# nnnagle/vq-vae

Measured on AMD Instinct MI355X. Metric: tiles/sec, higher is better.
Workload: dtype bf16

## Files before the change

include/frl_hip.h:

```cpp
#ifndef FRL_HIP_H
#define FRL_HIP_H

#include <stddef.h>
#include <stdint.h>

#ifdef __cplusplus
extern "C" {
#endif

typedef void* frl_stream_t;

enum { FRL_F32 = 0, FRL_BF16 = 1, FRL_F16 = 2  };
enum { FRL_ACT_NONE = 0, FRL_ACT_RELU = 1, FRL_ACT_SIGMOID = 2 };

int frl_version(void);
const char* frl_last_error(void);
int frl_device_arch(char* buf, int n);
int frl_kernel_timing_enable(int on);
int frl_kernel_timing_report(char* buf, int n);

size_t frl_pack_cache_table_bytes(void);
int frl_pack_cache_create(void* arena, size_t bytes);
int frl_pack_cache_destroy(int handle);
int frl_pack_cache_activate(int handle);
// ... 49 lines not shown
int frl_scalar_fanout_dev(const float* g, const float* coef_host, const float* const* mult_host, int n, float* out, frl_stream_t stream);
int frl_scalar_fanout_guard(const float* g, const float* coef_host, const float* const* mult_host, const float* const* promise_host, int n,
                            float* out, int* flag, frl_stream_t stream);

int frl_encoder2_supported(int C0, int C1, int C2, int G1, int G2, int HW, int dtype);
size_t frl_encoder2_workspace_bytes(int B);
int frl_encoder2_fwd(const void* x, const float* w1, const float* g1, const float* b1, const float* w2, const float* g2, const float* b2,
                     void* z, float* stats, int B, int HW, float eps, void* ws, size_t ws_bytes, frl_stream_t stream);
int frl_encoder2_bwd(const void* x, const void* dz, const float* w1, const float* g1, const float* b1, const float* w2, const float* g2,
                     const float* b2, const float* stats, float* dw1, float* dg1, float* db1, float* dw2, float* dg2, float* db2,
                     int B, int HW, void* ws, size_t ws_bytes, frl_stream_t stream);

int frl_sobel_fwd(const void* x, void* g, int B, int H, int W, int C, int dtype, frl_stream_t stream);
int frl_sobel_bwd(const void* dg, void* dx, int B, int H, int W, int C, int dtype, frl_stream_t stream);
int frl_sobel_bwd_add(const void* dg, void* dx, const void* dx_add, int B, int H, int W, int C, int dtype, frl_stream_t stream);
int frl_edge_smooth_stencil_fwd(const void* x, const void* a_logit, const void* b_logit, void* smoothed, void* residual,
                                void* a_soft, void* b_soft, int B, int H, int W, int C, int R, int coarse_dilation,
                                int dtype, frl_stream_t stream);
int frl_edge_smooth_stencil_bwd(const void* d_smoothed, const void* x, const void* a_soft, const void* b_soft, void* dx,
                                void* da_logit, void* db_logit, const void* dx_add , int B, int H,
                                int W, int C, int R, int coarse_dilation, int dtype, frl_stream_t stream);
int frl_smooth_heads_supported(int C, int hidden, int rank, int dtype);
size_t frl_smooth_heads_workspace_bytes(int64_t npix);
int frl_smooth_heads_fwd(const void* x, const void* feat, const float* wa, const float* ba, const float* wb, const float* bb,
                         void* smoothed, void* residual, int B, int H, int W, int coarse_dilation, void* ws, size_t ws_bytes,
                         frl_stream_t stream);
size_t frl_smooth_heads_bwd_scratch_bytes(int64_t npix);
int frl_smooth_heads_force_gather(int on);
int frl_smooth_heads_bwd(const void* d_smoothed, const void* x, const void* feat, const float* wa, const float* ba, const float* wb,
                         const float* bb, const void* dx_add, void* dx, void* dfeat, float* dwa, float* dba, float* dwb, float* dbb,
                         void* scratch, size_t scratch_bytes, int B, int H, int W, int coarse_dilation, void* ws, size_t ws_bytes,
                         frl_stream_t stream);
int frl_smooth_heads_bwd_masked(const void* d_smoothed, const void* x, const void* feat, const float* wa, const float* ba, const float* wb,
                                const float* bb, const void* dx_add, void* dx, void* dfeat, float* dwa, float* dba, float* dwb, float* dbb,
                                void* scratch, size_t scratch_bytes, int B, int H, int W, int dil, int dfeat_relu, void* ws,
                                size_t ws_bytes, frl_stream_t stream);
int frl_film_fused_supported(int cond_dim, int hidden, int target_dim, int dtype);
size_t frl_film_fused_workspace_bytes(void);
int frl_film_fused_fwd(const void* z_type, const void* h, const float* w1g, const float* b1g, const float* w2g, const float* b2g,
                       const float* w1b, const float* b1b, const float* w2b, const float* b2b, void* z, void* gamma, void* beta, int B,
                       int T, int HW, void* ws, size_t ws_bytes, frl_stream_t stream);
int frl_film_fused_bwd(const void* z_type, const void* h, const void* dz, const float* w1g, const float* b1g, const float* w2g,
                       const float* b2g, const float* w1b, const float* b1b, const float* w2b, const float* b2b, void* dh, float* dw1g,
                       float* db1g, float* dw2g, float* db2g, float* dw1b, float* db1b, float* dw2b, float* db2b, int B, int T, int HW,
                       void* ws, size_t ws_bytes, frl_stream_t stream);
int frl_gate_blend_fwd(const void* smoothed, const void* residual, const void* gate_raw, float min_gate, void* out,
                       void* gate_out, int64_t n, int dtype, frl_stream_t stream);
int frl_gate_blend_bwd(const void* dout, const void* dgate_ext, const void* residual, const void* gate_raw, float min_gate,
                       void* d_residual, void* d_gate_raw, int64_t n, int dtype, frl_stream_t stream);
int frl_gate_blend_bwd_masked(const void* dout, const void* dgate_ext, const void* residual, const void* gate_raw, float min_gate,
                              void* d_residual, void* d_gate_raw, int64_t n, int dtype, int sigmoid_mask, frl_stream_t stream);

int frl_tcn_block_fwd(const void* x, const float* conv_w, const float* conv_b, const float* gn_w, const float* gn_b,
                      const float* gate_w, const float* gate_b, const float* proj_w, const float* proj_b, void* y,
                      int64_t npix, int HW, int T, int Cin, int Cout, int dilation, int G, float eps, int dtype, void* ws,
                      size_t ws_bytes, frl_stream_t stream);
size_t frl_tcn_block_bwd_workspace_bytes(int64_t npix, int Cout);
int frl_tcn_block_bwd(const void* x, const void* dy, const float* conv_w, const float* conv_b, const float* gn_w,
                      const float* gn_b, const float* gate_w, const float* gate_b, const float* proj_w,
                      const float* proj_b, void* dconv, void* dgpre, void* normed, void* dres, float* dgamma, float* dbeta,
                      int64_t npix, int HW, int T, int Cin, int Cout, int dilation, int G, float eps, int dtype, void* ws,
                      size_t ws_bytes, frl_stream_t stream);
int frl_tcn_block_bwd_data(const void* dconv, const void* dres, const float* conv_w, const float* proj_w, void* dx,
                           int64_t npix, int HW, int T, int Cin, int Cout, int dilation, int dtype, void* ws, size_t ws_bytes,
                           frl_stream_t stream);

int frl_tcn_block_bwd_fused_supported(int T, int Cin, int Cout, int G, int has_proj, int dtype);
size_t frl_tcn_block_bwd_fused_workspace_bytes(int64_t npix);
int frl_tcn_block_bwd_fused(const void* x, const void* dy, const float* conv_w, const float* conv_b, const float* gn_w,
                            const float* gn_b, const float* gate_w, const float* gate_b, void* dx, float* d_conv_w,
                            float* d_conv_b, float* d_gn_w, float* d_gn_b, float* d_gate_w, float* d_gate_b, int64_t npix,
                            int HW, int T, int dilation, int G, float eps, void* ws, size_t ws_bytes, frl_stream_t stream);

int frl_defer_begin(void);
int frl_defer_pending(void);
int frl_defer_destinations(void** out, int max);
int frl_defer_flush(frl_stream_t stream);
int frl_defer_abort(void);

int frl_tcn_hot_supported(int T, int Cin, int Cout, int G, int dilation, int has_proj, int dtype);
size_t frl_tcn_hot_fwd_workspace_bytes(void);
size_t frl_tcn_hot_bwd_workspace_bytes(int64_t npix);
int frl_tcn_hot_fwd(const void* x, const void* drop_mask, const float* conv_w, const float* conv_b, const float* gn_w, const float* gn_b,
                    const float* gate_w, const float* gate_b, void* y, int64_t npix, int HW, int dilation, float eps, void* ws,
                    size_t ws_bytes, frl_stream_t stream);
int frl_tcn_hot_bwd_nodx_supported(int64_t npix, int HW);
int frl_tcn_hot_bwd(const void* x, const void* drop_mask, const void* dy, const float* conv_w, const float* conv_b, const float* gn_w,
                    const float* gn_b, const float* gate_w, const float* gate_b, void* dx, float* d_conv_w, float* d_conv_b,
                    float* d_gn_w, float* d_gn_b, float* d_gate_w, float* d_gate_b, int64_t npix, int HW, int dilation,
                    float eps, void* ws, size_t ws_bytes, frl_stream_t stream);
size_t frl_tcn_chain_fwd_workspace_bytes(void);
int frl_tcn_chain_static_tiles(int on);
int frl_tcn_chain_fwd(const void* x, const float* const* conv_w, const float* const* conv_b, const float* const* gn_w,
                      const float* const* gn_b, const float* const* gate_w, const float* const* gate_b, const float* head_w,
                      const float* head_b, void* y1, void* y2, void* y3, void* h, int64_t npix, int HW, int Ch, float eps, void* ws,
                      size_t ws_bytes, frl_stream_t stream);
int frl_tcn_chain_fwd_xt(const void* x, const float* const* conv_w, const float* const* conv_b, const float* const* gn_w,
                         const float* const* gn_b, const float* const* gate_w, const float* const* gate_b, const float* head_w,
                         const float* head_b, void* y1, void* y2, void* y3, void* h, void* xt, int64_t npix, int HW, int Ch, float eps,
                         void* ws, size_t ws_bytes, frl_stream_t stream);
int frl_tcn_hot_bwd_head_supported(int64_t npix, int HW, int Ch);
size_t frl_tcn_hot_bwd_head_workspace_bytes(int64_t npix);
int frl_tcn_hot_bwd_head(const void* x, const void* dh, const float* head_w, int Ch, const float* conv_w, const float* conv_b,
                         const float* gn_w, const float* gn_b, const float* gate_w, const float* gate_b, void* dx, float* d_conv_w,
                         float* d_conv_b, float* d_gn_w, float* d_gn_b, float* d_gate_w, float* d_gate_b, int64_t npix, int HW,
                         int dilation, float eps, void* ws, size_t ws_bytes, frl_stream_t stream);
int frl_tcn_hot_force_generic_tiles(int on);
int frl_tcn_hot_bwd4_share(int variant, int share);

size_t frl_adamw_workspace_bytes(void);
int frl_adamw_clip_step(const void* desc_host, int ntensors, const void* chunks, const int* chunk_tensor, int nchunks, float max_norm,
                        float lr, double beta1, double beta2, float eps, int step, float* norm_out, const float* ok, int* counters,
                        const float* lr_dev, void* ws, size_t ws_bytes, frl_stream_t stream);
int frl_multi_tensor_scale_copy(const void* desc_host, int ntensors, const void* chunks, const int* chunk_tensor, int nchunks, float scale,
                                frl_stream_t stream);

int frl_film_modulate_fwd(const void* h, const void* gamma, const void* beta, void* out, int64_t B, int T, int64_t HW,
                          int C, int dtype, frl_stream_t stream);
int frl_film_modulate_bwd(const void* dout, const void* h, const void* gamma, void* dh, void* dgamma, void* dbeta,
                          int64_t B, int T, int64_t HW, int C, int dtype, frl_stream_t stream);
int frl_mean_time_fwd(const void* tile, void* out, int64_t B, int T, int64_t HWC, int dtype, frl_stream_t stream);
int frl_add(const void* a, const void* b, float scale_b, void* out, int64_t n, int dtype, frl_stream_t stream);

typedef struct FrlNormRec {
  float sub, div, mul, add, lo, hi;
  int flags;
  int pad;
} FrlNormRec;
int frl_normalize_tiles(const void* raw, int raw_dtype, const uint8_t* valid, const void* table, void* out, int out_dtype,
                        uint8_t* mask_out, int64_t rows, int F, frl_stream_t stream);
int frl_normalize_chunk_tiles(const void* chunk, int raw_dtype, int T, int CY, int CX, int F, const int32_t* desc, int ntiles,
                              int tile, const void* table, void* out, int out_dtype, uint8_t* mask_out, frl_stream_t stream);

int frl_host_parallel_copy(void* dst, const void* src, size_t nbytes, int nthreads);

size_t frl_mse_workspace_bytes(void);
int frl_mse_fwd(const void* pred, const void* target, const uint8_t* mask, int64_t P, int C, float* out, int dtype,
                void* ws, size_t ws_bytes, frl_stream_t stream);
int frl_mse_bwd(const void* pred, const void* target, const uint8_t* mask, const float* gscale, const float* stats,
                int64_t P, int C, void* dpred, int dtype, frl_stream_t stream);

int frl_decoder_mse_fused_supported(int Cz, int hidden, int F, int dtype);
size_t frl_decoder_mse_workspace_bytes(int64_t P, int Cz);
int frl_decoder_mse_fwd(const void* z, const float* w1, const float* b1, const float* w2, const float* b2, const void* target,
                        const uint8_t* mask, void* xhat, float* out, int64_t P, int Cz, void* ws, size_t ws_bytes,
                        frl_stream_t stream);
int frl_decoder_mse_bwd(const void* z, const float* w1, const float* b1, const float* w2, const float* b2, const void* target,
                        const uint8_t* mask, const float* gscale, const float* stats, void* dz, float* dw1, float* db1,
                        float* dw2, float* db2, int64_t P, int Cz, void* ws, size_t ws_bytes, frl_stream_t stream);
size_t frl_decoder_mse_onepass_bytes(int64_t P, int Cz);
int frl_decoder_mse_fwd_bwd(const void* z, const float* w1, const float* b1, const float* w2, const float* b2, const void* target,
                            const uint8_t* mask, const float* gscale, float* out, void* dz, void* buf, size_t buf_bytes, void* ctl,
                            int* nslab, int64_t P, int Cz, frl_stream_t stream);
int frl_decoder_mse_reduce(const void* buf, int nslab, float* dw1, float* db1, float* dw2, float* db2, int Cz, frl_stream_t stream);
int frl_decoder_mse_bwd_subgroups(int on);

size_t frl_vq_workspace_bytes(int64_t N, int K, int d);
int frl_vq_assign_fwd(const void* z, const float* E, int64_t N, int K, int d, int32_t* idx_out, void* zq_out,
                      float* stats_out, int32_t* counts_out, int dtype, void* ws, size_t ws_bytes, frl_stream_t stream);
size_t frl_vq_prepared_bytes(int K, int d);
int frl_vq_stream_tiles(int nt);
int frl_vq_prepare(const float* E, int64_t N, int K, int d, int dtype, void* prep, size_t prep_bytes, frl_stream_t stream);
int frl_vq_assign_fwd_prepared(const void* z, const float* E, void* prep , int64_t N, int K, int d,
                               int32_t* idx_out, void* zq_out, float* stats_out, int32_t* counts_out, int dtype, void* ws,
                               size_t ws_bytes, frl_stream_t stream);
int frl_vq_bwd(const void* g_out, const void* z, const void* zq , const float* E, const int32_t* idx, const int32_t* counts,
               const float* gscale, float beta, int64_t N, int K, int d, void* g_z_out, float* g_E_out, float* sums_out,
               int dtype, void* ws, size_t ws_bytes, frl_stream_t stream);
int frl_vq_ema_update(const float* sums, const int32_t* counts, int K, int d, float decay, float eps, float* ema_count,
                      float* ema_sum, float* E, const float* ok, frl_stream_t stream);
int frl_vq_revive_dead_codes(float* E, const int64_t* window_counts, int64_t min_count, const void* z, int64_t N, int K, int d,
                             uint64_t seed, float* m, float* v, int32_t* revived, int dtype, frl_stream_t stream);

int frl_gather_locations_fwd(const void* feat, int64_t sC, int64_t sH, int64_t sW, int C, int H, int W, const int64_t* coords, int64_t N,
                             void* out, int dtype, frl_stream_t stream);
int frl_segment_sum_rows(const float* vals, const int64_t* order, const int64_t* keys_sorted, int64_t M, int D, float* out, int64_t out_stride,
                         int accumulate, frl_stream_t stream);
int frl_infonce_fwd(const float* emb, int D, const int64_t* pairs, const float* weights, const unsigned char* is_pos, int64_t T,
                    const int64_t* seg, int64_t nseg, float temperature, int similarity, float* sims, float* logits, float* loss_a, float* coef,
                    float* loss, frl_stream_t stream);
int frl_infonce_pair_grads(const float* emb, int D, const int64_t* pairs, const float* sims, const float* coef, const float* gscale, int64_t T,
                           int64_t nseg, float temperature, int similarity, float* ga, float* gb, frl_stream_t stream);

size_t frl_vicreg_workspace_bytes(int64_t N, int D);
int frl_vicreg_fwd(const void* x, int64_t N, int D, int dtype, float variance_weight, float covariance_weight, float variance_target,
                   float eps, float* losses, float* cov, float* centre, void* ws, size_t ws_bytes, frl_stream_t stream);
int frl_vicreg_bwd(const void* x, const float* cov, const float* centre, const float* g3, int64_t N, int D, int dtype, float variance_weight,
                   float covariance_weight, float variance_target, float eps, void* dx, frl_stream_t stream);

int frl_soft_nbr_fwd(const float* d_ref, const float* d_learned, const unsigned char* mask, const float* weights, int64_t B, int M,
                     float inv_tau_ref, float inv_tau_learned, int min_valid, float* pairstat, float* coef, float* out2, double* stats,
                     frl_stream_t stream);
int frl_soft_nbr_bwd(const float* coef, const float* pairstat, const float* weights, const float* out2, const float* gup, int64_t B, int M,
                     float* grad, frl_stream_t stream);
int frl_soft_nbr_gathered_fwd(const float* ref, int C, const void* emb, int D, int emb_dtype, const int64_t* ref_rows_a, const int64_t* ref_rows_b,
                              const int64_t* emb_rows_a, const int64_t* emb_rows_b, const int64_t* lengths, const float* weights, int64_t B, int M,
                              int exclude_diagonal, float inv_tau_ref, float inv_tau_learned, int min_valid, float* pairstat, float* out2,
                              double* stats, frl_stream_t stream);
int frl_soft_nbr_gathered_bwd(const float* ref, int C, const void* emb, int D, int emb_dtype, const int64_t* ref_rows_a, const int64_t* ref_rows_b,
                              const int64_t* emb_rows_a, const int64_t* emb_rows_b, const int64_t* lengths, const float* weights, int64_t B, int M,
                              int exclude_diagonal, float inv_tau_ref, float inv_tau_learned, int min_valid, const float* pairstat,
                              const float* out2, const float* gup, float* grad_rows, frl_stream_t stream);

int frl_evt_soft_nbr_fwd(const void* emb, int emb_dtype, int64_t N, int D, const int32_t* idx, const float* S, const float* w, int K,
                         const int32_t* seg, const int32_t* seg_host, int nseg, float inv_tau_ref, float inv_tau_learned, int min_valid_anchors,
                         float* rowstat, float* segout, double* segstat, int32_t* index_flag, frl_stream_t stream);
int frl_evt_soft_nbr_bwd(const void* emb, int emb_dtype, int64_t N, int D, const int32_t* idx, const float* S, const float* w, int K,
                         const int32_t* seg, const int32_t* seg_host, int nseg, float inv_tau_ref, float inv_tau_learned, const float* rowstat,
                         const float* segout, const float* gup, const float* seg_weights, void* grad, frl_stream_t stream);

int frl_decode_codes(const int32_t* idx, const void* table, void* out, int64_t P, int K, int F, int dtype, int32_t* index_flag,
                     frl_stream_t stream);

size_t frl_mutual_knn_max_points(int D);
int frl_mutual_knn(const float* feat, int N, int D, const int32_t* patch_id, const float* coords, float pos_min_spatial, int k,
                   int32_t* knn_idx, uint8_t* mutual, frl_stream_t stream);

#ifdef __cplusplus
}
#endif
#endif
```

vq-vae_amd/csrc/dec_fused.hip:

```cpp
#include "frl_common.hpp"
#include "frl_host.hpp"
#include "frl_pack.hpp"
#include "frl_reduce.hpp"

typedef bf16 TT;
typedef bf16x8 frag8;
#define DF_H 128
#define DF_F 64
#define DF_GRID_MAX 1024

__device__ __forceinline__ bf16x8 tr_frag_p(const TT* tile, int pitch, int pix0, int ch0, int r16) {
  const TT* a0 = tile + (pix0 + (r16 >> 2)) * pitch + ch0 + 4 * (r16 & 3);
  bf16x4 lo = __builtin_amdgcn_ds_read_tr16_b64_v4bf16((bf16x4 __attribute__((address_space(3)))*)(a0));
  bf16x4 hi = __builtin_amdgcn_ds_read_tr16_b64_v4bf16((bf16x4 __attribute__((address_space(3)))*)(a0 + 4 * pitch));
  return bf16x8{lo[0], lo[1], lo[2], lo[3], hi[0], hi[1], hi[2], hi[3]};
}

template <int NF>
__device__ __forceinline__ void tile_put(TT* tile, int pitch, int prow, int kc, const LQTile<TT, NF>& t) {
  bf16x8* p = reinterpret_cast<bf16x8*>(tile + prow * pitch + NF * 8 * kc);
#pragma unroll
  for (int s = 0; s < NF; ++s) p[s] = t.f[s];
}

template <int NFZ>
__device__ __forceinline__ void dec_chain(float (&h)[32], float (&xh)[16], const LQTile<TT, NFZ>& zt, const frag8* __restrict__ w1,
                                          const frag8* __restrict__ w2, const float* __restrict__ b1q, const float* __restrict__ b2q,
                                          LQTile<TT, 4>& ht, int lane) {
  f32x4 hacc[8];
#pragma unroll
  for (int m = 0; m < 8; ++m) {
    hacc[m] = f32x4{0.f, 0.f, 0.f, 0.f};
#pragma unroll
    for (int s = 0; s < NFZ; ++s) hacc[m] = mfma16(w1[(m * NFZ + s) * 64 + lane], zt.f[s], hacc[m]);
  }
#pragma unroll
  for (int j = 0; j < 32; ++j) {
    const float v = hacc[j >> 2][j & 3] + b1q[j];
    h[j] = v > 0.f ? v : 0.f;
    ht.f[j >> 3][j & 7] = (bf16)h[j];
  }
  f32x4 xacc[4];
#pragma unroll
  for (int m = 0; m < 4; ++m) {
    xacc[m] = f32x4{0.f, 0.f, 0.f, 0.f};
#pragma unroll
    for (int s = 0; s < 4; ++s) xacc[m] = mfma16(w2[(m * 4 + s) * 64 + lane], ht.f[s], xacc[m]);
  }
#pragma unroll
  for (int j = 0; j < 16; ++j) xh[j] = xacc[j >> 2][j & 3] + b2q[j];
}

template <int NFZ>
__global__ __launch_bounds__(256, 4) void dec_mse_fwd_kernel(const TT* __restrict__ Z, const frag8* __restrict__ Wpk, const float* __restrict__ b1,
                                                          const float* __restrict__ b2, const TT* __restrict__ TGT,
                                                          const uint8_t* __restrict__ mask, TT* __restrict__ XHAT, int64_t P, int Cz,
                                                          double* __restrict__ partial) {
  extern __shared__ __attribute__((aligned(16))) char smem[];
  frag8* w1 = reinterpret_cast<frag8*>(smem);
  frag8* w2 = w1 + 8 * NFZ * 64;
  float* tb = reinterpret_cast<float*>(w2 + 16 * 64);
  const int tid = threadIdx.x, lane = tid & 63, wave = tid >> 6;
  const int px = lane & 15, kc = lane >> 4;
  copy_frags_lds<TT>(w1, Wpk, (8 * NFZ + 16) * 64, tid, 256);
  for (int i = tid; i < 192; i += 256) tb[i] = i < 128 ? b1[i] : b2[i - 128];
  __syncthreads();
  const float* b1q = tb + 32 * kc;
  const float* b2q = tb + 128 + 16 * kc;
  const bool fastz = (Cz == 32 * NFZ);
  float sq = 0.f, cnt = 0.f;
  const int64_t ntile = (P + 15) >> 4;
  const int64_t tstep = (int64_t)gridDim.x * 4;
  LQTile<TT, NFZ> zt, zn;
  LQTile<TT, 2> tt, tn;
  {
    const int64_t t0 = (int64_t)blockIdx.x * 4 + wave;
    const int64_t r0 = (t0 < ntile ? t0 : 0) * 16 + px;
    const int64_t rc = r0 < P ? r0 : P - 1;
    lq_load<TT, NFZ>(zt, Z, rc, Cz, kc, fastz);
    lq_load<TT, 2>(tt, TGT, rc, DF_F, kc, true);
  }
  for (int64_t tile = (int64_t)blockIdx.x * 4 + wave; tile < ntile; tile += tstep) {
    int64_t row = tile * 16 + px;
    bool valid = row < P;
    if (!valid) row = P - 1;
    if (valid && mask != nullptr) valid = mask[row] != 0;
    {
      const int64_t tnx = tile + tstep < ntile ? tile + tstep : tile;
      const int64_t rn = tnx * 16 + px;
      const int64_t rc = rn < P ? rn : P - 1;
      lq_load<TT, NFZ>(zn, Z, rc, Cz, kc, fastz);
      lq_load<TT, 2>(tn, TGT, rc, DF_F, kc, true);
    }
    float h[32], xh[16];
    LQTile<TT, 4> ht;
    int lw = lane;
    asm volatile("" : "+v"(lw));
    dec_chain<NFZ>(h, xh, zt, w1, w2, b1q, b2q, ht, lw);
    if (valid) {
#pragma unroll
      for (int j = 0; j < 16; ++j) { const float d = xh[j] - (float)tt.f[j >> 3][j & 7]; sq = fmaf(d, d, sq); }
      cnt += 16.f;
    }
    if (XHAT != nullptr && tile * 16 + px < P) {
      bf16x8* xo = reinterpret_cast<bf16x8*>(XHAT + row * DF_F + 16 * kc);
      bf16x8 o0, o1;
#pragma unroll
      for (int j = 0; j < 8; ++j) { o0[j] = (bf16)xh[j]; o1[j] = (bf16)xh[8 + j]; }
      xo[0] = o0;
      xo[1] = o1;
    }
    zt = zn;
    tt = tn;
  }
  double sd = wave_sum_d((double)sq), cd = wave_sum_d((double)cnt);
  __shared__ double red[8];
  if (lane == 0) { red[wave] = sd; red[4 + wave] = cd; }
  __syncthreads();
  if (tid == 0) {
    partial[blockIdx.x * 2 + 0] = red[0] + red[1] + red[2] + red[3];
    partial[blockIdx.x * 2 + 1] = red[4] + red[5] + red[6] + red[7];
  }
}

__global__ __launch_bounds__(256) void dec_mse_finalize_kernel(const double* __restrict__ partial, int n, float* __restrict__ out) {
  __shared__ double rs[256], rc[256];
  double s = 0.0, c = 0.0;
  for (int i = threadIdx.x; i < n; i += 256) { s += partial[2 * i]; c += partial[2 * i + 1]; }
  rs[threadIdx.x] = s; rc[threadIdx.x] = c;
  __syncthreads();
  for (int o = 128; o > 0; o >>= 1) {
    if (threadIdx.x < o) { rs[threadIdx.x] += rs[threadIdx.x + o]; rc[threadIdx.x] += rc[threadIdx.x + o]; }
    __syncthreads();
  }
  if (threadIdx.x == 0) { out[0] = rc[0] > 0.0 ? (float)(rs[0] / rc[0]) : 0.f; out[1] = (float)rc[0]; }
}

__device__ __forceinline__ void df_sg_sync(unsigned* bar, unsigned& gen, int lane) {
  asm volatile("s_waitcnt lgkmcnt(0)" ::: "memory");
  gen += 4u;
  if (lane == 0) __hip_atomic_fetch_add(bar, 1u, __ATOMIC_RELAXED, __HIP_MEMORY_SCOPE_WORKGROUP);
  for (;;) {
    const unsigned seen = (unsigned)__builtin_amdgcn_readfirstlane((int)__hip_atomic_load(bar, __ATOMIC_RELAXED, __HIP_MEMORY_SCOPE_WORKGROUP));
    if ((int)(seen - gen) >= 0) break;
    __builtin_amdgcn_s_sleep(1);
  }
  asm volatile("" ::: "memory");
}
#define DF_SG_SHARE0 19

template <bool LOSS> struct DecLoss {};
template <> struct DecLoss<true> {
  double* partial;
  const float* out;
  float* out_w;
  float nv_host;
};

template <int NFZ, int NW, bool SG = false, bool LOSS = false>
__global__ __launch_bounds__(SG ? 512 : 64 * NW) void dec_mse_bwd_kernel(const TT* __restrict__ Z, const frag8* __restrict__ Wpk, const float* __restrict__ b1,
                                                               const float* __restrict__ b2, const TT* __restrict__ TGT,
                                                               const uint8_t* __restrict__ mask, const float* __restrict__ gscale,
                                                               const float* __restrict__ stats, TT* __restrict__ DZ, int64_t P, int Cz,
                                                               float* __restrict__ slab, const DecLoss<LOSS> la) {
  constexpr int CZP = 32 * NFZ, CB = CZP / 16, R = 16 * NW, NTH = SG ? 512 : 64 * NW;
  constexpr int PX = DF_F + 8, PH = DF_H + 8, PZ = CZP + 8;
  static_assert(!SG || NW == 4, "subgroups are four waves");
  extern __shared__ __attribute__((aligned(16))) char smem[];
  frag8* w1 = reinterpret_cast<frag8*>(smem);
  frag8* w2 = w1 + 8 * NFZ * 64;
  frag8* w2t = w2 + 16 * 64;
  frag8* w1t = w2t + 16 * 64;
  float* tb = reinterpret_cast<float*>(w1t + CB * 4 * 64);
  const int tid = threadIdx.x, lane = tid & 63;
  const int sg = SG ? (tid >> 8) : 0;
  const int wave = SG ? ((tid >> 6) & 3) : (tid >> 6);
  constexpr int TILE_ELEMS = R * (PX + 2 * PH + PZ);
  unsigned* bars = reinterpret_cast<unsigned*>(tb + 192);
  TT* t_dx = reinterpret_cast<TT*>(tb + 192 + (SG ? 32 : 0)) + sg * TILE_ELEMS;
  TT* t_h = t_dx + R * PX;
  TT* t_dh = t_h + R * PH;
  TT* t_z = t_dh + R * PH;
  const int px = lane & 15, kc = lane >> 4, r16 = px;
  const int prow = wave * 16 + px;
  copy_frags_lds<TT>(w1, Wpk, (8 * NFZ + 16 + 16 + CB * 4) * 64, tid, NTH);
  for (int i = tid; i < 192; i += NTH) tb[i] = i < 128 ? b1[i] : b2[i - 128];
  if (SG && tid < 2) bars[16 * tid] = 0u;
  unsigned* bar = bars + 16 * sg;
  unsigned bgen = 0;
  (void)bar; (void)bgen;
  __syncthreads();
  const float* b1q = tb + 32 * kc;
  const float* b2q = tb + 128 + 16 * kc;
  const bool fastz = (Cz == CZP);
  float nv;
  if constexpr (LOSS) nv = la.nv_host >= 0.f ? la.nv_host : la.out[1]; else nv = stats[1];
  float sq = 0.f;
  int nrow = 0;
  (void)sq; (void)nrow;
  const float ksc = nv > 0.f ? (gscale ? gscale[0] : 1.f) * 2.f / nv : 0.f;

  constexpr int W2CB = (NW == 8) ? 4 : 8;
  const int w2row = (NW == 8) ? (wave & 3) : wave;
  const int w2col0 = (NW == 8) ? 4 * (wave >> 2) : 0;
  constexpr int W1RB = (NW == 8) ? 1 : 2;
  f32x4 a2[W2CB], a1[W1RB][CB], ab2, ab1[W1RB];
#pragma unroll
  for (int i = 0; i < W2CB; ++i) a2[i] = f32x4{0.f, 0.f, 0.f, 0.f};
#pragma unroll
  for (int r = 0; r < W1RB; ++r) {
    ab1[r] = f32x4{0.f, 0.f, 0.f, 0.f};
#pragma unroll
    for (int i = 0; i < CB; ++i) a1[r][i] = f32x4{0.f, 0.f, 0.f, 0.f};
  }
  ab2 = f32x4{0.f, 0.f, 0.f, 0.f};
  const bf16 one = (bf16)1.f, zero = (bf16)0.f;
  const bf16x8 ones = (r16 == 0) ? bf16x8{one, one, one, one, one, one, one, one} : bf16x8{zero, zero, zero, zero, zero, zero, zero, zero};

  const int64_t nwt = (P + R - 1) / R;
  int64_t w_first = blockIdx.x, w_end = nwt;
  const int64_t w_step = gridDim.x;
  if (SG) {
    const int64_t n_wg = (int64_t)blockIdx.x < nwt ? (nwt - 1 - blockIdx.x) / w_step + 1 : 0;
    const int64_t n0 = (n_wg * DF_SG_SHARE0 + 16) >> 5;
    w_first = blockIdx.x + (sg ? n0 : 0) * w_step;
    w_end = blockIdx.x + (sg ? n_wg : n0) * w_step;
    if (w_end > nwt) w_end = nwt;
  }
  LQTile<TT, NFZ> zt, z1, z2, zn;
  LQTile<TT, 2> tt, t1, t2, tn;
  auto fetch = [&](LQTile<TT, NFZ>& zz, LQTile<TT, 2>& tg, int64_t w) {
    const int64_t wc = w < nwt ? w : (nwt - 1);
    const int64_t r0 = wc * R + prow;
    const int64_t rc = r0 < P ? r0 : P - 1;
    lq_load<TT, NFZ>(zz, Z, rc, Cz, kc, fastz);
    lq_load<TT, 2>(tg, TGT, rc, DF_F, kc, true);
  };
  fetch(zt, tt, w_first);
  fetch(z1, t1, w_first + w_step);
  fetch(z2, t2, w_first + 2 * w_step);
  for (int64_t wt = w_first; wt < w_end; wt += w_step) {
    int64_t row = wt * R + prow;
    const bool inb = row < P;
    bool valid = inb;
    if (!inb) row = P - 1;
    if (valid && mask != nullptr) valid = mask[row] != 0;
    fetch(zn, tn, wt + 3 * w_step);
    float h[32], xh[16];
    LQTile<TT, 4> ht;
    dec_chain<NFZ>(h, xh, zt, w1, w2, b1q, b2q, ht, lane);
    LQTile<TT, 2> dxt;
    const float kv = valid ? ksc : 0.f;
    if constexpr (LOSS) {
      if (valid) {
#pragma unroll
        for (int j = 0; j < 16; ++j) { const float d = xh[j] - (float)tt.f[j >> 3][j & 7]; sq = fmaf(d, d, sq); }
      }
      nrow += __popcll(__ballot(valid));
    }
#pragma unroll
    for (int j = 0; j < 16; ++j) dxt.f[j >> 3][j & 7] = (bf16)(kv * (xh[j] - (float)tt.f[j >> 3][j & 7]));
    f32x4 dhacc[8];
#pragma unroll
    for (int m = 0; m < 8; ++m) {
      dhacc[m] = f32x4{0.f, 0.f, 0.f, 0.f};
#pragma unroll
      for (int s = 0; s < 2; ++s) dhacc[m] = mfma16(w2t[(m * 2 + s) * 64 + lane], dxt.f[s], dhacc[m]);
    }
    LQTile<TT, 4> dht;
#pragma unroll
    for (int j = 0; j < 32; ++j) dht.f[j >> 3][j & 7] = (bf16)(h[j] > 0.f ? dhacc[j >> 2][j & 3] : 0.f);
    f32x4 dzacc[CB];
#pragma unroll
    for (int m = 0; m < CB; ++m) {
      dzacc[m] = f32x4{0.f, 0.f, 0.f, 0.f};
#pragma unroll
      for (int s = 0; s < 4; ++s) dzacc[m] = mfma16(w1t[(m * 4 + s) * 64 + lane], dht.f[s], dzacc[m]);
    }
    if (inb) {
      constexpr int QZ = 4 * CB;
      TT* dzp = DZ + row * (int64_t)Cz + QZ * kc;
      if (fastz) {
#pragma unroll
        for (int j = 0; j < QZ; j += 8) {
          bf16x8 o;
#pragma unroll
          for (int e = 0; e < 8; ++e) o[e] = (bf16)dzacc[(j + e) >> 2][(j + e) & 3];
          *reinterpret_cast<bf16x8*>(dzp + j) = o;
        }
      } else if ((Cz & 3) == 0) {
#pragma unroll
        for (int j = 0; j < QZ; j += 4)
          if (QZ * kc + j < Cz)
            *reinterpret_cast<bf16x4*>(dzp + j) = bf16x4{(bf16)dzacc[j >> 2][0], (bf16)dzacc[j >> 2][1], (bf16)dzacc[j >> 2][2], (bf16)dzacc[j >> 2][3]};
      } else {
#pragma unroll
        for (int j = 0; j < QZ; ++j)
          if (QZ * kc + j < Cz) dzp[j] = (bf16)dzacc[j >> 2][j & 3];
      }
    }
    if (!inb) {
#pragma unroll
      for (int s = 0; s < 4; ++s) dht.f[s] = bf16x8{zero, zero, zero, zero, zero, zero, zero, zero};
    }
    tile_put<2>(t_dx, PX, prow, kc, dxt);
    tile_put<4>(t_h, PH, prow, kc, ht);
    tile_put<4>(t_dh, PH, prow, kc, dht);
    tile_put<NFZ>(t_z, PZ, prow, kc, zt);
    if constexpr (SG) df_sg_sync(bar, bgen, lane); else __syncthreads();
#pragma unroll
    for (int ks = 0; ks < R / 32; ++ks) {
      const int pix0 = ks * 32 + 8 * kc;
      const bf16x8 af = tr_frag_p(t_dx, PX, pix0, w2row * 16, r16);
#pragma unroll
      for (int i = 0; i < W2CB; ++i) a2[i] = mfma16(af, tr_frag_p(t_h, PH, pix0, (w2col0 + i) * 16, r16), a2[i]);
      if (NW == 4 || (wave >> 2) == 0) ab2 = mfma16(af, ones, ab2);
#pragma unroll
      for (int r = 0; r < W1RB; ++r) {
        const int rb = (NW == 8) ? wave : 2 * wave + r;
        const bf16x8 ah = tr_frag_p(t_dh, PH, pix0, rb * 16, r16);
#pragma unroll
        for (int i = 0; i < CB; ++i) a1[r][i] = mfma16(ah, tr_frag_p(t_z, PZ, pix0, i * 16, r16), a1[r][i]);
        ab1[r] = mfma16(ah, ones, ab1[r]);
      }
    }
    if constexpr (SG) df_sg_sync(bar, bgen, lane); else __syncthreads();
    zt = z1; z1 = z2; z2 = zn;
    tt = t1; t1 = t2; t2 = tn;
  }
  float* my = slab + (int64_t)(SG ? 2 * blockIdx.x + sg : blockIdx.x) * (DF_F * DF_H + DF_H * CZP + DF_F + DF_H);
#pragma unroll
  for (int i = 0; i < W2CB; ++i)
#pragma unroll
    for (int r = 0; r < 4; ++r) my[(w2row * 16 + kc * 4 + r) * DF_H + (w2col0 + i) * 16 + r16] = a2[i][r];
#pragma unroll
  for (int rr = 0; rr < W1RB; ++rr) {
    const int rb = (NW == 8) ? wave : 2 * wave + rr;
#pragma unroll
    for (int i = 0; i < CB; ++i)
#pragma unroll
      for (int r = 0; r < 4; ++r) my[DF_F * DF_H + (rb * 16 + kc * 4 + r) * CZP + i * 16 + r16] = a1[rr][i][r];
    if (r16 == 0) {
#pragma unroll
      for (int r = 0; r < 4; ++r) my[DF_F * DF_H + DF_H * CZP + DF_F + rb * 16 + kc * 4 + r] = ab1[rr][r];
    }
  }
  if (r16 == 0 && (NW == 4 || (wave >> 2) == 0)) {
#pragma unroll
    for (int r = 0; r < 4; ++r) my[DF_F * DF_H + DF_H * CZP + w2row * 16 + kc * 4 + r] = ab2[r];
  }
  if constexpr (LOSS) {
    constexpr int NWV = NTH / 64;
    __shared__ double lred[2 * NWV];
    const double sd = wave_sum_d((double)sq), cd = 16.0 * (double)nrow;
    if (lane == 0) { lred[tid >> 6] = sd; lred[NWV + (tid >> 6)] = cd; }
    __syncthreads();
    if (tid == 0) {
      double s = lred[0], c = lred[NWV];
#pragma unroll
      for (int w = 1; w < NWV; ++w) { s += lred[w]; c += lred[NWV + w]; }
      la.partial[2 * blockIdx.x + 0] = s;
      la.partial[2 * blockIdx.x + 1] = c;
    }
  }
}

__global__ __launch_bounds__(256) void dec_mask_count_kernel(const uint8_t* __restrict__ mask, int64_t P, unsigned* __restrict__ ctl,
                                                             float* __restrict__ out) {
  __shared__ unsigned wg_n;
  const int tid = threadIdx.x;
  if (tid == 0) wg_n = 0u;
  __syncthreads();
  const int64_t gtid = (int64_t)blockIdx.x * 256 + tid, gstep = (int64_t)gridDim.x * 256;
  const int64_t n16 = ((reinterpret_cast<uintptr_t>(mask) & 15) == 0) ? (P >> 4) : 0;
  unsigned n = 0;
  const uint4* m16 = reinterpret_cast<const uint4*>(mask);
  for (int64_t i = gtid; i < n16; i += gstep) {
    const uint4 v = m16[i];
    const unsigned w[4] = {v.x, v.y, v.z, v.w};
#pragma unroll
    for (int k = 0; k < 4; ++k)
      n += __popc((w[k] | ((w[k] & 0x7f7f7f7fu) + 0x7f7f7f7fu)) & 0x80808080u);
  }
  for (int64_t i = n16 * 16 + gtid; i < P; i += gstep) n += mask[i] != 0 ? 1u : 0u;
  if (n) atomicAdd(&wg_n, n);
  __syncthreads();
  if (tid == 0) {
    unsigned long long* total = reinterpret_cast<unsigned long long*>(ctl + 2);
    if (wg_n) __hip_atomic_fetch_add(total, (unsigned long long)wg_n, __ATOMIC_RELAXED, __HIP_MEMORY_SCOPE_AGENT);
    __builtin_amdgcn_fence(__ATOMIC_RELEASE, "agent");
    asm volatile("s_waitcnt vmcnt(0)" ::: "memory");
    const unsigned ticket = __hip_atomic_fetch_add(ctl, 1u, __ATOMIC_RELAXED, __HIP_MEMORY_SCOPE_AGENT);
    if (ticket == gridDim.x - 1) {
      __builtin_amdgcn_fence(__ATOMIC_ACQUIRE, "agent");
      asm volatile("s_waitcnt vmcnt(0)" ::: "memory");
      const unsigned long long t = __hip_atomic_load(total, __ATOMIC_RELAXED, __HIP_MEMORY_SCOPE_AGENT);
      out[1] = (float)((double)t * (double)DF_F);
      __hip_atomic_store(total, 0ull, __ATOMIC_RELAXED, __HIP_MEMORY_SCOPE_AGENT);
      __hip_atomic_store(ctl, 0u, __ATOMIC_RELAXED, __HIP_MEMORY_SCOPE_AGENT);
    }
  }
}

template <int NFZ>
__global__ void dec_pack_kernel(frag8* __restrict__ dst, const float* __restrict__ W1, const float* __restrict__ W2, int Cz, int bwd) {
  constexpr int CZP = 32 * NFZ, CB = CZP / 16;
  const int tid = blockIdx.x * blockDim.x + threadIdx.x, nt = gridDim.x * blockDim.x;
  pack_weights_lds<TT, NFZ>(dst, W1, DF_H, Cz, 8, Cz, 1, tid, nt);
  frag8* p = dst + 8 * NFZ * 64;
  pack_weights_lds<TT, 4>(p, W2, DF_F, DF_H, 4, DF_H, 1, tid, nt);
  if (!bwd) return;
  p += 16 * 64;
  pack_weights_lds<TT, 2>(p, W2, DF_H, DF_F, 8, 1, DF_H, tid, nt);
  p += 16 * 64;
  pack_weights_lds<TT, 4>(p, W1, Cz, DF_H, CB, 1, Cz, tid, nt);
}

template <int NFZ>
static const frag8* dec_packed(const float* w1, const float* w2, int Cz, int bwd, frag8* ws_pk, hipStream_t st) {
  constexpr int CZP = 32 * NFZ, CB = CZP / 16;
  FrlPackJob jobs[4];
  size_t off = 0;
  jobs[0] = frl_pack_job_pw(w1, off, FRL_BF16, NFZ, DF_H, Cz, 8, Cz, 1);
  off += (size_t)8 * NFZ * 64 * sizeof(frag8);
  jobs[1] = frl_pack_job_pw(w2, off, FRL_BF16, 4, DF_F, DF_H, 4, DF_H, 1);
  off += (size_t)16 * 64 * sizeof(frag8);
  int n = 2;
  if (bwd) {
    jobs[2] = frl_pack_job_pw(w2, off, FRL_BF16, 2, DF_H, DF_F, 8, 1, DF_H);
    off += (size_t)16 * 64 * sizeof(frag8);
    jobs[3] = frl_pack_job_pw(w1, off, FRL_BF16, 4, Cz, DF_H, CB, 1, Cz);
    off += (size_t)CB * 4 * 64 * sizeof(frag8);
    n = 4;
  }
  bool hit = false;
  frag8* pk = ws_pk;
  if (void* img = frl_pack_cached(jobs, n, off, &hit)) pk = (frag8*)img;
  if (!hit) FRL_LAUNCH((dec_pack_kernel<NFZ>), dim3(32), dim3(256), 0, st, pk, w1, w2, Cz, bwd);
  return pk;
}


static unsigned df_fwd_grid(int64_t P) { int64_t g = ((P + 15) / 16 + 3) / 4; if (g > DF_GRID_MAX) g = DF_GRID_MAX; return (unsigned)(g < 1 ? 1 : g); }
static unsigned df_bwd_grid(int64_t P, int R) { int64_t g = (P + R - 1) / R; if (g > 256) g = 256; return (unsigned)(g < 1 ? 1 : g); }

template <int NFZ, int NW, bool LOSS = false>
static int launch_dec_bwd(const void* z, const float* w1, const float* b1, const float* w2, const float* b2, const void* tgt,
                          const uint8_t* mask, const float* gscale, const float* stats, void* dz, float* dw1, float* db1, float* dw2,
                          float* db2, int64_t P, int Cz, char* ws, hipStream_t st, DecLoss<LOSS> la = DecLoss<LOSS>{}, int* nslab_out = nullptr) {
  constexpr int CZP = 32 * NFZ, CB = CZP / 16, R = 16 * NW;
  const unsigned grid = df_bwd_grid(P, R);
  const size_t slab_n = (size_t)DF_F * DF_H + DF_H * CZP + DF_F + DF_H;
  const frag8* pk = dec_packed<NFZ>(w1, w2, Cz, 1, reinterpret_cast<frag8*>(ws + ((grid * slab_n * sizeof(float) + 255) / 256) * 256), st);
  const size_t lds = (size_t)(8 * NFZ + 16 + 16 + CB * 4) * 64 * sizeof(frag8) + 192 * sizeof(float) +
                     (size_t)R * ((DF_F + 8) + 2 * (DF_H + 8) + (CZP + 8)) * sizeof(TT);
  auto kern = dec_mse_bwd_kernel<NFZ, NW, false, LOSS>;
  FRL_HIP(hipFuncSetAttribute((const void*)kern, hipFuncAttributeMaxDynamicSharedMemorySize, (int)lds));
  FRL_LAUNCH_AS(LOSS ? "dec_mse_bwd_loss_kernel" : "dec_mse_bwd_kernel", kern, dim3(grid), dim3(64 * NW), lds, st, (const TT*)z, (const frag8*)pk, b1, b2, (const TT*)tgt, mask, gscale, stats, (TT*)dz, P, Cz,
             (float*)ws, la);
  if constexpr (LOSS) {
    FRL_LAUNCH(dec_mse_finalize_kernel, dim3(1), dim3(256), 0, st, (const double*)la.partial, (int)grid, la.out_w);
    *nslab_out = (int)grid;
    return frl_check_launch("decoder_mse_fwd_bwd");
  }
  launch_slab_reduce_deferrable<float, DecEpi>((const float*)ws, (int)grid, (int64_t)slab_n, DecEpi{dw2, dw1, db2, db1, Cz, CZP, DF_F, DF_H}, st);
  return frl_check_launch("decoder_mse_bwd");
}

template <int NFZ, bool LOSS = false>
static int launch_dec_bwd_sg(const void* z, const float* w1, const float* b1, const float* w2, const float* b2, const void* tgt,
                             const uint8_t* mask, const float* gscale, const float* stats, void* dz, float* dw1, float* db1, float* dw2,
                             float* db2, int64_t P, int Cz, char* ws, hipStream_t st, DecLoss<LOSS> la = DecLoss<LOSS>{}, int* nslab_out = nullptr) {
  constexpr int CZP = 32 * NFZ, CB = CZP / 16, R = 64;
  int64_t g = (P + 2 * R - 1) / (2 * R);
  if (g > 256) g = 256;
  if (g < 1) g = 1;
  const unsigned grid = (unsigned)g, nslab = 2 * grid;
  const size_t slab_n = (size_t)DF_F * DF_H + DF_H * CZP + DF_F + DF_H;
  const frag8* pk = dec_packed<NFZ>(w1, w2, Cz, 1, reinterpret_cast<frag8*>(ws + ((nslab * slab_n * sizeof(float) + 255) / 256) * 256), st);
  const size_t lds = (size_t)(8 * NFZ + 16 + 16 + CB * 4) * 64 * sizeof(frag8) + (192 + 32) * sizeof(float) +
                     (size_t)2 * R * ((DF_F + 8) + 2 * (DF_H + 8) + (CZP + 8)) * sizeof(TT);
  auto kern = dec_mse_bwd_kernel<NFZ, 4, true, LOSS>;
  FRL_HIP(hipFuncSetAttribute((const void*)kern, hipFuncAttributeMaxDynamicSharedMemorySize, (int)lds));
  FRL_LAUNCH_AS(LOSS ? "dec_mse_bwd_sg_loss_kernel" : "dec_mse_bwd_sg_kernel", kern, dim3(grid), dim3(512), lds, st, (const TT*)z, (const frag8*)pk, b1, b2, (const TT*)tgt, mask, gscale, stats, (TT*)dz, P,
                Cz, (float*)ws, la);
  if constexpr (LOSS) {
    FRL_LAUNCH(dec_mse_finalize_kernel, dim3(1), dim3(256), 0, st, (const double*)la.partial, (int)grid, la.out_w);
    *nslab_out = (int)nslab;
    return frl_check_launch("decoder_mse_fwd_bwd");
  }
  launch_slab_reduce_deferrable<float, DecEpi>((const float*)ws, (int)nslab, (int64_t)slab_n, DecEpi{dw2, dw1, db2, db1, Cz, CZP, DF_F, DF_H}, st);
  return frl_check_launch("decoder_mse_bwd");
}

static int g_dec_subgroups = 1;

extern "C" {

int frl_decoder_mse_bwd_subgroups(int on) { const int was = g_dec_subgroups; g_dec_subgroups = on ? 1 : 0; return was; }

int frl_decoder_mse_fused_supported(int Cz, int hidden, int F, int dtype) {
  return (dtype == FRL_BF16 && hidden == DF_H && F == DF_F && Cz >= 1 && Cz <= 64) ? 1 : 0;
}

size_t frl_decoder_mse_workspace_bytes(int64_t P, int Cz) {
  const size_t czp = Cz <= 32 ? 32 : 64;
  const size_t slab_n = (size_t)DF_F * DF_H + DF_H * czp + DF_F + DF_H;
  const size_t bwd = 512 * slab_n * sizeof(float) + 256 + (size_t)(8 * 2 + 32 + 16) * 64 * 16;
  const size_t fwd = (size_t)DF_GRID_MAX * 2 * sizeof(double) + 256 + (size_t)(8 * 2 + 16) * 64 * 16;
  (void)P;
  return bwd > fwd ? bwd : fwd;
}

int frl_decoder_mse_fwd(const void* z, const float* w1, const float* b1, const float* w2, const float* b2, const void* target,
                        const uint8_t* mask, void* xhat, float* out, int64_t P, int Cz, void* ws, size_t ws_bytes, hipStream_t stream) {
  if (P <= 0) return frl_fail(-2, "decoder_mse_fwd: empty input");
  if (Cz < 1 || Cz > 64) return frl_fail(-2, "decoder_mse_fwd: latent width must be 1..64");
  if (ws_bytes < frl_decoder_mse_workspace_bytes(P, Cz)) return frl_fail(-4, "decoder_mse_fwd: workspace too small");
  char* w = (char*)ws;
  double* partial = (double*)w;
  frag8* ws_pk = reinterpret_cast<frag8*>(w + (size_t)DF_GRID_MAX * 2 * sizeof(double) + 256);
  const unsigned grid = df_fwd_grid(P);
  if (Cz <= 32) {
    const frag8* pk = dec_packed<1>(w1, w2, Cz, 0, ws_pk, stream);
    const size_t lds = (size_t)(8 + 16) * 64 * sizeof(frag8) + 192 * sizeof(float);
    FRL_LAUNCH((dec_mse_fwd_kernel<1>), dim3(grid), dim3(256), lds, stream, (const TT*)z, (const frag8*)pk, b1, b2, (const TT*)target, mask,
               (TT*)xhat, P, Cz, partial);
  } else {
    const frag8* pk = dec_packed<2>(w1, w2, Cz, 0, ws_pk, stream);
    const size_t lds = (size_t)(16 + 16) * 64 * sizeof(frag8) + 192 * sizeof(float);
    FRL_LAUNCH((dec_mse_fwd_kernel<2>), dim3(grid), dim3(256), lds, stream, (const TT*)z, (const frag8*)pk, b1, b2, (const TT*)target, mask,
               (TT*)xhat, P, Cz, partial);
  }
  FRL_LAUNCH(dec_mse_finalize_kernel, dim3(1), dim3(256), 0, stream, (const double*)partial, (int)grid, out);
  return frl_check_launch("decoder_mse_fwd");
}

int frl_decoder_mse_bwd(const void* z, const float* w1, const float* b1, const float* w2, const float* b2, const void* target,
                        const uint8_t* mask, const float* gscale, const float* stats, void* dz, float* dw1, float* db1, float* dw2,
                        float* db2, int64_t P, int Cz, void* ws, size_t ws_bytes, hipStream_t stream) {
  if (P <= 0) return frl_fail(-2, "decoder_mse_bwd: empty input");
  if (Cz < 1 || Cz > 64) return frl_fail(-2, "decoder_mse_bwd: latent width must be 1..64");
  if (ws_bytes < frl_decoder_mse_workspace_bytes(P, Cz)) return frl_fail(-4, "decoder_mse_bwd: workspace too small");
  if (g_dec_subgroups && P >= 128 && Cz <= 32)
    return launch_dec_bwd_sg<1>(z, w1, b1, w2, b2, target, mask, gscale, stats, dz, dw1, db1, dw2, db2, P, Cz, (char*)ws, stream);
  if (Cz <= 32) return launch_dec_bwd<1, 8>(z, w1, b1, w2, b2, target, mask, gscale, stats, dz, dw1, db1, dw2, db2, P, Cz, (char*)ws, stream);
  return launch_dec_bwd<2, 4>(z, w1, b1, w2, b2, target, mask, gscale, stats, dz, dw1, db1, dw2, db2, P, Cz, (char*)ws, stream);
}

static size_t df_onepass_partial_off(int64_t P, int Cz) { return ((frl_decoder_mse_workspace_bytes(P, Cz) + 255) / 256) * 256; }
size_t frl_decoder_mse_onepass_bytes(int64_t P, int Cz) { return df_onepass_partial_off(P, Cz) + (size_t)256 * 2 * sizeof(double); }

int frl_decoder_mse_fwd_bwd(const void* z, const float* w1, const float* b1, const float* w2, const float* b2, const void* target,
                            const uint8_t* mask, const float* gscale, float* out, void* dz, void* buf, size_t buf_bytes, void* ctl,
                            int* nslab, int64_t P, int Cz, hipStream_t stream) {
  if (P <= 0) return frl_fail(-2, "decoder_mse_fwd_bwd: empty input");
  if (Cz < 1 || Cz > 64) return frl_fail(-2, "decoder_mse_fwd_bwd: latent width must be 1..64");
  if (buf_bytes < frl_decoder_mse_onepass_bytes(P, Cz)) return frl_fail(-4, "decoder_mse_fwd_bwd: buffer too small");
  if (out == nullptr || dz == nullptr || ctl == nullptr || nslab == nullptr) return frl_fail(-2, "decoder_mse_fwd_bwd: null output");
  unsigned* c = (unsigned*)ctl;
  DecLoss<true> la;
  la.partial = reinterpret_cast<double*>((char*)buf + df_onepass_partial_off(P, Cz));
  la.out = out;
  la.out_w = out;
  la.nv_host = (float)((double)P * (double)DF_F);
  if (mask != nullptr) {
    int64_t g = (P + 256 * 64 - 1) / (256 * 64);
    if (g > 128) g = 128;
    FRL_LAUNCH(dec_mask_count_kernel, dim3((unsigned)g), dim3(256), 0, stream, mask, P, c, out);
    la.nv_host = -1.f;
  }
  if (g_dec_subgroups && P >= 128 && Cz <= 32)
    return launch_dec_bwd_sg<1, true>(z, w1, b1, w2, b2, target, mask, gscale, nullptr, dz, nullptr, nullptr, nullptr, nullptr, P, Cz, (char*)buf, stream, la, nslab);
  if (Cz <= 32)
    return launch_dec_bwd<1, 8, true>(z, w1, b1, w2, b2, target, mask, gscale, nullptr, dz, nullptr, nullptr, nullptr, nullptr, P, Cz, (char*)buf, stream, la, nslab);
  return launch_dec_bwd<2, 4, true>(z, w1, b1, w2, b2, target, mask, gscale, nullptr, dz, nullptr, nullptr, nullptr, nullptr, P, Cz, (char*)buf, stream, la, nslab);
}

int frl_decoder_mse_reduce(const void* buf, int nslab, float* dw1, float* db1, float* dw2, float* db2, int Cz, hipStream_t stream) {
  if (Cz < 1 || Cz > 64 || nslab < 1 || nslab > 512) return frl_fail(-2, "decoder_mse_reduce: bad latent width or slab count");
  const int czp = Cz <= 32 ? 32 : 64;
  const size_t slab_n = (size_t)DF_F * DF_H + DF_H * czp + DF_F + DF_H;
  launch_slab_reduce_deferrable<float, DecEpi>((const float*)buf, nslab, (int64_t)slab_n, DecEpi{dw2, dw1, db2, db1, Cz, czp, DF_F, DF_H}, stream);
  return frl_check_launch("decoder_mse_reduce");
}

}
```

vq-vae_amd/csrc/frl_common.hpp:

```cpp
#pragma once
#include <hip/hip_runtime.h>
#include <stdint.h>

typedef __bf16 bf16;
typedef __attribute__((ext_vector_type(8))) __bf16 bf16x8;
typedef __attribute__((ext_vector_type(4))) __bf16 bf16x4;
typedef __attribute__((ext_vector_type(2))) __bf16 bf16x2;
typedef __attribute__((ext_vector_type(4))) float f32x4;
typedef __attribute__((ext_vector_type(2))) float f32x2;

enum { FRL_F32 = 0, FRL_BF16 = 1 };
enum { FRL_ACT_NONE = 0, FRL_ACT_RELU = 1, FRL_ACT_SIGMOID = 2 };

#define FRL_WAVE 64

template <typename T> struct DT;
template <> struct DT<float> {
  typedef float frag_t;
  static constexpr int FE = 1;
  static constexpr int CPAD = 16;
  static constexpr int VEC = 4;
  static constexpr int ID = FRL_F32;
};
template <> struct DT<bf16> {
  typedef bf16x8 frag_t;
  static constexpr int FE = 8;
  static constexpr int CPAD = 32;
  static constexpr int VEC = 8;
  static constexpr int ID = FRL_BF16;
};

__device__ __forceinline__ f32x4 mfma16(const float a, const float b, f32x4 c) {
  return __builtin_amdgcn_mfma_f32_16x16x4f32(a, b, c, 0, 0, 0);
}
__device__ __forceinline__ f32x4 mfma16(const bf16x8 a, const bf16x8 b, f32x4 c) {
  return __builtin_amdgcn_mfma_f32_16x16x32_bf16(a, b, c, 0, 0, 0);
}

__device__ __forceinline__ float to_f32(float v) { return v; }
__device__ __forceinline__ float to_f32(bf16 v) { return (float)v; }
template <typename T> __device__ __forceinline__ T from_f32(float v);
template <> __device__ __forceinline__ float from_f32<float>(float v) { return v; }
template <> __device__ __forceinline__ bf16 from_f32<bf16>(float v) { return (bf16)v; }

__device__ __forceinline__ float act_fwd(float v, int act) {
  if (act == FRL_ACT_RELU) return v > 0.f ? v : 0.f;
  if (act == FRL_ACT_SIGMOID) return 1.f / (1.f + expf(-v));
  return v;
}
__device__ __forceinline__ float sigmoid_fast(float v) {
  return __builtin_amdgcn_rcpf(1.f + __builtin_amdgcn_exp2f(-1.44269504088896f * v));
}
template <typename T> __device__ __forceinline__ float sigmoid_t(float v) {
  if constexpr (sizeof(T) == 2) return sigmoid_fast(v); else return 1.f / (1.f + expf(-v));
}

__device__ __forceinline__ float act_bwd_from_y(float y, int act) {
  if (act == FRL_ACT_RELU) return y > 0.f ? 1.f : 0.f;
  if (act == FRL_ACT_SIGMOID) return y * (1.f - y);
  return 1.f;
}

template <typename T> struct Vec;
template <> struct Vec<float> {
  static constexpr int N = 4;
  __device__ static __forceinline__ void load(const float* p, float* o) {
    f32x4 v = *reinterpret_cast<const f32x4*>(p);
    o[0] = v[0]; o[1] = v[1]; o[2] = v[2]; o[3] = v[3];
  }
  __device__ static __forceinline__ void store(float* p, const float* o) {
    f32x4 v = {o[0], o[1], o[2], o[3]};
    *reinterpret_cast<f32x4*>(p) = v;
  }
};
template <> struct Vec<bf16> {
  static constexpr int N = 8;
  __device__ static __forceinline__ void load(const bf16* p, float* o) {
    bf16x8 v = *reinterpret_cast<const bf16x8*>(p);
#pragma unroll
    for (int i = 0; i < 8; ++i) o[i] = (float)v[i];
  }
  __device__ static __forceinline__ void store(bf16* p, const float* o) {
    bf16x8 v;
#pragma unroll
    for (int i = 0; i < 8; ++i) v[i] = (bf16)o[i];
    *reinterpret_cast<bf16x8*>(p) = v;
  }
};

__device__ __forceinline__ float wave_sum(float v) {
#pragma unroll
  for (int o = 32; o > 0; o >>= 1) v += __shfl_xor(v, o, 64);
  return v;
}
__device__ __forceinline__ double wave_sum_d(double v) {
#pragma unroll
  for (int o = 32; o > 0; o >>= 1) v += __shfl_xor(v, o, 64);
  return v;
}

__device__ __forceinline__ unsigned xcd_remap(unsigned bid, unsigned nwg) {
  const unsigned q = nwg >> 3, r = nwg & 7u, xcd = bid & 7u;
  const unsigned base = xcd < r ? xcd * (q + 1) : r * (q + 1) + (xcd - r) * q;
  return base + (bid >> 3);
}

template <typename T, int NF> struct LQTile { typename DT<T>::frag_t f[NF]; };

template <typename T> __device__ __forceinline__ int lq_channel(int q, int kc, int s, int e) {
  return q * kc + s * DT<T>::FE + e;
}

template <typename T, int NF>
__device__ __forceinline__ void lq_load(LQTile<T, NF>& t, const T* __restrict__ X, int64_t row, int C,
                                        int kc, bool fast) {
  constexpr int FE = DT<T>::FE;
  const int q = NF * FE;
  const T* p = X + row * (int64_t)C + q * kc;
  if (fast) {
    if constexpr (FE == 8) {
#pragma unroll
      for (int s = 0; s < NF; ++s) t.f[s] = *reinterpret_cast<const bf16x8*>(p + 8 * s);
    } else {
      static_assert(NF % 4 == 0, "f32 quarter must be a multiple of 4");
#pragma unroll
      for (int s = 0; s < NF; s += 4) {
        f32x4 v = *reinterpret_cast<const f32x4*>(p + s);
        t.f[s] = v[0]; t.f[s + 1] = v[1]; t.f[s + 2] = v[2]; t.f[s + 3] = v[3];
      }
    }
  } else {
    if constexpr (FE == 8) {
      if ((C & 3) == 0) {
#pragma unroll
        for (int s = 0; s < NF; ++s) {
          bf16x4 lo = bf16x4{(bf16)0.f, (bf16)0.f, (bf16)0.f, (bf16)0.f}, hi = lo;
          const int c = q * kc + 8 * s;
          if (c < C) lo = *reinterpret_cast<const bf16x4*>(p + 8 * s);
          if (c + 4 < C) hi = *reinterpret_cast<const bf16x4*>(p + 8 * s + 4);
          t.f[s] = bf16x8{lo[0], lo[1], lo[2], lo[3], hi[0], hi[1], hi[2], hi[3]};
        }
        return;
      }
    }
#pragma unroll
    for (int s = 0; s < NF; ++s) {
      if constexpr (FE == 8) {
        bf16x8 v;
#pragma unroll
        for (int e = 0; e < 8; ++e) {
          const int c = q * kc + 8 * s + e;
          v[e] = c < C ? p[8 * s + e] : (bf16)0.f;
        }
        t.f[s] = v;
      } else {
        const int c = q * kc + s;
        t.f[s] = c < C ? p[s] : 0.f;
      }
    }
  }
}

template <typename T, int NF>
__device__ __forceinline__ float lq_get(const LQTile<T, NF>& t, int s, int e) {
  if constexpr (DT<T>::FE == 8) return (float)t.f[s][e]; else return t.f[s];
}
template <typename T, int NF>
__device__ __forceinline__ void lq_set(LQTile<T, NF>& t, int s, int e, float v) {
  if constexpr (DT<T>::FE == 8) t.f[s][e] = (bf16)v; else t.f[s] = v;
}

template <typename T, int NF>
__device__ __forceinline__ void pack_weights_lds(typename DT<T>::frag_t* __restrict__ wl,
                                                 const float* __restrict__ W, int Cout, int Cin, int MB,
                                                 int64_t so, int64_t si, int tid, int nthreads) {
  constexpr int FE = DT<T>::FE;
  const int q = NF * FE, qo = 4 * MB;
  const int total = MB * NF * 64;
  for (int i = tid; i < total; i += nthreads) {
    const int lane = i & 63, fs = i >> 6;
    const int s = fs % NF, mb = fs / NF;
    const int r = lane & 15, kc = lane >> 4;
    const int oc = qo * (r >> 2) + 4 * mb + (r & 3);
    if constexpr (FE == 8) {
      bf16x8 v;
#pragma unroll
      for (int e = 0; e < 8; ++e) {
        const int ic = q * kc + 8 * s + e;
        v[e] = (oc < Cout && ic < Cin) ? (bf16)W[oc * so + ic * si] : (bf16)0.f;
      }
      wl[i] = v;
    } else {
      const int ic = q * kc + s;
      wl[i] = (oc < Cout && ic < Cin) ? W[oc * so + ic * si] : 0.f;
    }
  }
// ... 20 lines not shown
```

vq-vae_amd/csrc/vq.hip:

```cpp
#include "frl_common.hpp"
#include "frl_host.hpp"
#include "frl_reduce.hpp"
#include <math.h>
#include <stdlib.h>

#define VQ_IDX_BITS 7
#define VQ_IDX_MASK 127u
#define VQ_MAX_CHUNK 512

struct VqHeader {
  unsigned enmax_bits;
  int namb;
  double sq_fix;
  int done;
  int pad;
};

template <typename T, int NF>
__global__ void vq_prepare_kernel(const float* __restrict__ E, int K, int d, float* __restrict__ en, int kpad,
                                  typename DT<T>::frag_t* __restrict__ pk, int total, int npack_blocks, int* __restrict__ ctl) {
  constexpr int FE = DT<T>::FE;
  constexpr int q = NF * FE;
  if ((int)blockIdx.x >= npack_blocks) {
    const int k = ((int)blockIdx.x - npack_blocks) * blockDim.x + threadIdx.x;
// ... 1276 lines not shown
#pragma unroll
      for (int s = 0; s < NF; ++s) acc = mfma16(pk[(size_t)(mb * NF + s) * 64 + lane], zr.f[s], acc);
#pragma unroll
      for (int r = 0; r < 4; ++r) {
        const int code = mb * 16 + 4 * kc + r;
        const bool hit = valid && acc[r] <= lm && code < K;
        if (__builtin_amdgcn_ballot_w64(hit && p1 >= 0) != 0ull) flush();
        if (hit) { if (p0 < 0) p0 = code; else p1 = code; }
      }
    }
    flush();
#pragma unroll
    for (int off = 16; off <= 32; off <<= 1) {
      const double ob = __shfl_xor(bestd, off, 64);
      const int okk = __shfl_xor(bk, off, 64);
      if (ob < bestd || (ob == bestd && okk < bk)) { bestd = ob; bk = okk; }
    }
    if (kc == 0) { mrg_d[wave][vx] = bestd; mrg_k[wave][vx] = bk; }
    __syncthreads();
    if (wave == 0) {
      bestd = mrg_d[0][vx]; bk = mrg_k[0][vx];
#pragma unroll
      for (int w = 1; w < VQ_FIXT_WAVES; ++w) {
        const double ob = mrg_d[w][vx];
        const int okk = mrg_k[w][vx];
        if (ob < bestd || (ob == bestd && okk < bk)) { bestd = ob; bk = okk; }
      }
      if ((unsigned)bk >= (unsigned)K) bk = 0;
      if (valid) {
        const float* er = E + (int64_t)bk * d + q * kc;
        T* zo = zq_out + row * (int64_t)d + q * kc;
#pragma unroll
        for (int s = 0; s < NF * FE; ++s) {
          if (q * kc + s < d) {
            const float ev = to_f32(from_f32<T>(er[s]));
            zo[s] = from_f32<T>(ev);
            const float df = lq_get<T, NF>(zr, s / FE, s % FE) - ev;
            sq_acc = fmaf(df, df, sq_acc);
          }
        }
        if (kc == 0) { idx_out[row] = bk; atomicAdd(&counts_fix[bk], 1); }
      }
    }
    __syncthreads();
  }
  if (wave == 0) {
    const float ws_ = wave_sum(sq_acc);
    if (lane == 0 && ws_ != 0.f) atomicAdd(&hdr->sq_fix, (double)ws_);
  }
}

__global__ __launch_bounds__(256) void vq_finalize_kernel(const float* __restrict__ partial, int npartial, const VqHeader* __restrict__ hdr,
                                                          const int32_t* __restrict__ counts_acc, int32_t* __restrict__ counts, int K, int64_t N,
                                                          int d, float* __restrict__ stats) {
  __shared__ double red[256];
  double s = 0.0;
  for (int i = threadIdx.x; i < npartial; i += 256) s += (double)partial[i];
  red[threadIdx.x] = s;
  __syncthreads();
  for (int o = 128; o > 0; o >>= 1) { if (threadIdx.x < o) red[threadIdx.x] += red[threadIdx.x + o]; __syncthreads(); }
  const double sq = red[0] + hdr->sq_fix;
  __syncthreads();
  double h = 0.0;
  for (int k = threadIdx.x; k < K; k += 256) {
    const int cnt = counts_acc[k];
    counts[k] = cnt;
    const double p = (double)cnt / (double)N;
    h += p * log(p + 1e-10);
  }
  red[threadIdx.x] = h;
  __syncthreads();
  for (int o = 128; o > 0; o >>= 1) { if (threadIdx.x < o) red[threadIdx.x] += red[threadIdx.x + o]; __syncthreads(); }
  if (threadIdx.x == 0) {
    stats[0] = (float)sq;
    stats[1] = (float)exp(-red[0]);
    stats[2] = (float)hdr->namb;
    stats[3] = (float)(sq / ((double)N * (double)d));
  }
}

template <typename T>
__global__ __launch_bounds__(256) void vq_bwd_kernel(const T* __restrict__ gout, const T* __restrict__ Z,
                                                     const float* __restrict__ E, const int32_t* __restrict__ idx,
                                                     const float* __restrict__ gscale, float cz_base, int64_t N, int K, int d,
                                                     int Kc, int64_t rows_per_wg, T* __restrict__ gz,
                                                     float* __restrict__ slab ) {
  extern __shared__ __attribute__((aligned(16))) char smem[];
  float* acc = reinterpret_cast<float*>(smem);
  const int tid = threadIdx.x;
  const int64_t r0 = (int64_t)blockIdx.x * rows_per_wg;
  int64_t r1 = r0 + rows_per_wg;
  if (r1 > N) r1 = N;
  const float cz = cz_base * (gscale ? gscale[0] : 1.f);
  constexpr int VEC = DT<T>::VEC;
  const bool fast = (d % VEC) == 0;
  const int vpr = (d + VEC - 1) / VEC;
  const int nchunks = (K + Kc - 1) / Kc;
  for (int c = 0; c < nchunks; ++c) {
    const int kbase = c * Kc;
    __syncthreads();
    for (int i = tid; i < Kc * d; i += 256) acc[i] = 0.f;
    __syncthreads();
    const int64_t nvec = (r1 > r0 ? (r1 - r0) : 0) * vpr;
    for (int64_t i = tid; i < nvec; i += 256) {
      const int64_t n = r0 + i / vpr;
      const int c0 = (int)(i % vpr) * VEC;
      const int k = idx[n];
      const bool mine = (k >= kbase && k < kbase + Kc);
      if (c == 0 || mine) {
        float zv[VEC];
        if (fast) Vec<T>::load(Z + n * (int64_t)d + c0, zv);
        else {
#pragma unroll
          for (int e = 0; e < VEC; ++e) zv[e] = (c0 + e < d) ? to_f32(Z[n * (int64_t)d + c0 + e]) : 0.f;
        }
        if (mine) {
#pragma unroll
          for (int e = 0; e < VEC; ++e)
            if (c0 + e < d) atomicAdd(&acc[(k - kbase) * d + c0 + e], zv[e]);
        }
        if (c == 0 && gz != nullptr) {
          float gv[VEC], ov[VEC];
          if (gout != nullptr) {
            if (fast) Vec<T>::load(gout + n * (int64_t)d + c0, gv);
            else {
#pragma unroll
              for (int e = 0; e < VEC; ++e) gv[e] = (c0 + e < d) ? to_f32(gout[n * (int64_t)d + c0 + e]) : 0.f;
            }
          } else {
#pragma unroll
            for (int e = 0; e < VEC; ++e) gv[e] = 0.f;
          }
#pragma unroll
          for (int e = 0; e < VEC; ++e) {
            const float ev = (c0 + e < d) ? to_f32(from_f32<T>(E[(int64_t)k * d + c0 + e])) : 0.f;
            ov[e] = gv[e] + cz * (zv[e] - ev);
          }
          if (fast) Vec<T>::store(gz + n * (int64_t)d + c0, ov);
          else {
#pragma unroll
            for (int e = 0; e < VEC; ++e)
              if (c0 + e < d) gz[n * (int64_t)d + c0 + e] = from_f32<T>(ov[e]);
          }
        }
      }
    }
    __syncthreads();
    const int kn = (K - kbase) < Kc ? (K - kbase) : Kc;
    float* dst = slab + ((int64_t)blockIdx.x * K + kbase) * d;
    for (int i = tid; i < kn * d; i += 256) dst[i] = acc[i];
  }
}

template <int RB, int CB, int NWV>
__global__ __launch_bounds__(64 * NWV) void vq_bwd_mfma_kernel(const bf16* __restrict__ gout, const bf16* __restrict__ Z, const bf16* __restrict__ ZQ,
                                                          const float* __restrict__ E,
                                                          const int32_t* __restrict__ idx, const float* __restrict__ gscale, float cz_base,
                                                          int64_t N, int K, int d, int64_t rows_per_wg, bf16* __restrict__ gz,
                                                          float* __restrict__ slab ) {
  constexpr int DP = CB * 16, PITCH = DP + 8, KC = RB * NWV * 16, NTH = 64 * NWV;
  extern __shared__ __attribute__((aligned(16))) char smem[];
  bf16* zt = reinterpret_cast<bf16*>(smem);
  int* it = reinterpret_cast<int*>(zt + 64 * PITCH);
  const int tid = threadIdx.x, lane = tid & 63, wave = tid >> 6;
  const int r16 = lane & 15, kc = lane >> 4;
  const int64_t r0 = (int64_t)blockIdx.x * rows_per_wg;
  int64_t r1 = r0 + rows_per_wg;
  if (r1 > N) r1 = N;
  const float cz = cz_base * (gscale ? gscale[0] : 1.f);
  const bool fast = (d % 8) == 0;
  const int vpr = DP / 8;
  const bf16 one = (bf16)1.f, zero = (bf16)0.f;
  for (int kbase = 0; kbase < K; kbase += KC) {
    f32x4 acc[RB][CB];
#pragma unroll
    for (int a = 0; a < RB; ++a)
#pragma unroll
      for (int b = 0; b < CB; ++b) acc[a][b] = f32x4{0.f, 0.f, 0.f, 0.f};
    constexpr int NV = (64 * (DP / 8) + NTH - 1) / NTH;
    const bool pre = fast && (ZQ != nullptr || gz == nullptr || kbase != 0);
    const bool want_gz = (kbase == 0 && gz != nullptr);
    bf16x8 rz[NV], rg[NV], rq[NV];
    auto fetch = [&](int64_t p0) {
#pragma unroll
      for (int u = 0; u < NV; ++u) {
        const int i = tid + u * NTH;
        const int row = i / vpr, c0 = (i % vpr) * 8;
        const int64_t n = p0 + row;
        const bool ok = i < 64 * vpr && n < r1 && c0 < d;
        const int64_t off = ok ? n * (int64_t)d + c0 : 0;
        bf16x8 v = *reinterpret_cast<const bf16x8*>(Z + off);
        if (!ok) v = bf16x8{};
        rz[u] = v;
        if (want_gz) {
          rg[u] = gout != nullptr ? *reinterpret_cast<const bf16x8*>(gout + off) : bf16x8{};
          rq[u] = *reinterpret_cast<const bf16x8*>(ZQ + off);
        }
      }
    };
    if (pre && r0 < r1) fetch(r0);
    for (int64_t p0 = r0; p0 < r1; p0 += 64) {
      __syncthreads();
      if (pre) {
#pragma unroll
        for (int u = 0; u < NV; ++u) {
          const int i = tid + u * NTH;
          if (i >= 64 * vpr) continue;
          const int row = i / vpr, c0 = (i % vpr) * 8;
          const int64_t n = p0 + row;
          if (want_gz && n < r1 && c0 < d) {
            float ov[8];
#pragma unroll
            for (int e = 0; e < 8; ++e) ov[e] = (float)rg[u][e] + cz * ((float)rz[u][e] - (float)rq[u][e]);
            Vec<bf16>::store(gz + n * (int64_t)d + c0, ov);
          }
          *reinterpret_cast<bf16x8*>(zt + row * PITCH + c0) = rz[u];
        }
      } else {
      for (int i = tid; i < 64 * vpr; i += NTH) {
        const int row = i / vpr, c0 = (i % vpr) * 8;
        const int64_t n = p0 + row;
        float zv[8];
#pragma unroll
        for (int e = 0; e < 8; ++e) zv[e] = 0.f;
        if (n < r1 && c0 < d) {
          if (fast) Vec<bf16>::load(Z + n * (int64_t)d + c0, zv);
          else {
#pragma unroll
            for (int e = 0; e < 8; ++e) if (c0 + e < d) zv[e] = (float)Z[n * (int64_t)d + c0 + e];
          }
          if (kbase == 0 && gz != nullptr) {
            const int k = idx[n];
            float gv[8], ov[8];
#pragma unroll
            for (int e = 0; e < 8; ++e) gv[e] = 0.f;
            if (gout != nullptr) {
              if (fast) Vec<bf16>::load(gout + n * (int64_t)d + c0, gv);
              else {
#pragma unroll
                for (int e = 0; e < 8; ++e) if (c0 + e < d) gv[e] = (float)gout[n * (int64_t)d + c0 + e];
              }
            }
            float qv[8];
            if (ZQ != nullptr && fast) Vec<bf16>::load(ZQ + n * (int64_t)d + c0, qv);
            else {
#pragma unroll
              for (int e = 0; e < 8; ++e) qv[e] = (c0 + e < d) ? (float)(bf16)E[(int64_t)k * d + c0 + e] : 0.f;
            }
#pragma unroll
            for (int e = 0; e < 8; ++e) ov[e] = gv[e] + cz * (zv[e] - qv[e]);
            if (fast) Vec<bf16>::store(gz + n * (int64_t)d + c0, ov);
            else {
#pragma unroll
              for (int e = 0; e < 8; ++e) if (c0 + e < d) gz[n * (int64_t)d + c0 + e] = (bf16)ov[e];
            }
          }
        }
        Vec<bf16>::store(zt + row * PITCH + c0, zv);
      }
      }
      if (tid < 64) it[tid] = (p0 + tid < r1) ? idx[p0 + tid] - kbase : -1;
      __syncthreads();
      if (pre && p0 + 64 < r1) fetch(p0 + 64);
#pragma unroll
      for (int ks = 0; ks < 2; ++ks) {
        const int pix0 = ks * 32 + 8 * kc;
        int id8[8];
#pragma unroll
        for (int j = 0; j < 8; ++j) id8[j] = it[pix0 + j];
        bf16x8 bfr[CB];
#pragma unroll
        for (int b = 0; b < CB; ++b) {
          const bf16* a0 = zt + (pix0 + (r16 >> 2)) * PITCH + b * 16 + 4 * (r16 & 3);
          bf16x4 lo = __builtin_amdgcn_ds_read_tr16_b64_v4bf16((bf16x4 __attribute__((address_space(3)))*)(a0));
          bf16x4 hi = __builtin_amdgcn_ds_read_tr16_b64_v4bf16((bf16x4 __attribute__((address_space(3)))*)(a0 + 4 * PITCH));
          bfr[b] = bf16x8{lo[0], lo[1], lo[2], lo[3], hi[0], hi[1], hi[2], hi[3]};
        }
#pragma unroll
        for (int a = 0; a < RB; ++a) {
          const int code = (wave * RB + a) * 16 + r16;
          bf16x8 af;
#pragma unroll
          for (int j = 0; j < 8; ++j) af[j] = (id8[j] == code) ? one : zero;
#pragma unroll
          for (int b = 0; b < CB; ++b) acc[a][b] = mfma16(af, bfr[b], acc[a][b]);
        }
      }
    }
    float* dst = slab + (int64_t)blockIdx.x * K * d;
#pragma unroll
    for (int a = 0; a < RB; ++a)
#pragma unroll
      for (int b = 0; b < CB; ++b)
#pragma unroll
        for (int r = 0; r < 4; ++r) {
          const int k = kbase + (wave * RB + a) * 16 + kc * 4 + r, c = b * 16 + r16;
          if (k < K && c < d) dst[(int64_t)k * d + c] = acc[a][b][r];
        }
  }
}


template <typename T>
__global__ void vq_code_reduce_kernel(const float* __restrict__ slab, int nslab, const float* __restrict__ E,
                                      const int32_t* __restrict__ counts, const float* __restrict__ gscale, float ce_base,
                                      int K, int d, float* __restrict__ gE, float* __restrict__ sums_out) {
  const int64_t i = (int64_t)blockIdx.x * blockDim.x + threadIdx.x;
  if (i >= (int64_t)K * d) return;
  float s = 0.f;
  for (int w = 0; w < nslab; ++w) s += slab[(int64_t)w * K * d + i];
  if (sums_out) sums_out[i] = s;
  if (gE) {
    const float ce = ce_base * (gscale ? gscale[1] : 1.f);
    const float ev = to_f32(from_f32<T>(E[i]));
    gE[i] = ce * ((float)counts[i / d] * ev - s);
  }
}


__global__ __launch_bounds__(256) void vq_ema_kernel(const float* __restrict__ sums, const int32_t* __restrict__ counts, int K, int d,
                                                     float decay, float eps, float* __restrict__ ema_count,
                                                     float* __restrict__ ema_sum, float* __restrict__ E, const float* __restrict__ ok) {
  __shared__ double red[256];
  if (ok != nullptr && !(ok[0] > 0.f)) return;
  double s = 0.0;
  for (int k = threadIdx.x; k < K; k += 256) {
    const float nc = decay * ema_count[k] + (1.f - decay) * (float)counts[k];
    ema_count[k] = nc;
    s += (double)nc;
  }
  red[threadIdx.x] = s;
  __syncthreads();
  for (int o = 128; o > 0; o >>= 1) { if (threadIdx.x < o) red[threadIdx.x] += red[threadIdx.x + o]; __syncthreads(); }
  const float n = (float)red[0];
  for (int i = threadIdx.x; i < K * d; i += 256) {
    const int k = i / d;
    const float ms = decay * ema_sum[i] + (1.f - decay) * sums[i];
    ema_sum[i] = ms;
    const float smoothed = (ema_count[k] + eps) / (n + (float)K * eps) * n;
    E[i] = ms / smoothed;
  }
}

static int vq_chunk(int K, int d_pad, size_t esize, int nw) {
  (void)nw;
  const size_t cap = 64 * 1024;
  int kc = VQ_MAX_CHUNK;
  while (kc > 16 && (size_t)kc * d_pad * esize > cap) kc >>= 1;
  const int kpad = (K + 15) / 16 * 16;
  if (kc > kpad) kc = kpad;
  return kc;
}
static int vq_waves(int64_t N, int d) { return (d <= 64 && N >= (int64_t)256 * 8 * 2 * 16) ? 8 : 4; }
static int vq_grid(int64_t N, int d) {
  const int nw = vq_waves(N, d), NT = nw == 8 ? 2 : 4;
  const int64_t nb = (N + nw * NT * 16 - 1) / (nw * NT * 16);
  const int cap = 512;
  return (int)(nb < cap ? (nb < 1 ? 1 : nb) : cap);
}
#define VQ_FIX_WAVES 1024
#define VQ_BWD_WGS 256

struct VqPrep { size_t ctl, en, pack, total; int Kc, kpad, npk; };
template <typename T, int NF>
static VqPrep vq_prep_layout(int64_t N, int K, int d) {
  VqPrep P;
  const int d_pad = NF * DT<T>::FE * 4;
  P.Kc = vq_chunk(K, d_pad, sizeof(T), vq_waves(N, d));
  P.kpad = (K + P.Kc - 1) / P.Kc * P.Kc;
  P.npk = (P.kpad / 16) * NF * 64;
  P.ctl = 0;
  P.en = (sizeof(VqCtl) + (size_t)K * 4 + 255) / 256 * 256;
  P.pack = P.en + ((size_t)P.kpad * 4 + 255) / 256 * 256;
  P.total = P.pack + (size_t)P.npk * sizeof(typename DT<T>::frag_t);
  return P;
}
static size_t vq_prep_bytes_max(int K) {
  return (sizeof(VqCtl) + (size_t)K * 4 + 255) / 256 * 256 + ((size_t)(K + VQ_MAX_CHUNK) * 4 + 255) / 256 * 256 +
         (size_t)((K + 15) / 16 + 64) * 16 * 128 * 4;
}

struct VqLayout { size_t hdr, counts_fix, partial, amb, amb_lim, prep, total; int grid; };
static VqLayout vq_layout(int64_t N, int K, int d) {
  VqLayout L;
  L.grid = vq_grid(N, d);
  size_t o = 0;
  L.hdr = o; o += 256;
  L.counts_fix = o; o += ((size_t)K * 4 + 255) / 256 * 256;
  L.partial = o; o += ((size_t)L.grid * 16 * 4 + 255) / 256 * 256;
  L.amb = o; o += ((size_t)N * 4 + 255) / 256 * 256;
  L.amb_lim = o; o += ((size_t)N * 4 + 255) / 256 * 256;
  L.prep = o; o += vq_prep_bytes_max(K);
  L.total = o;
  return L;
}

template <typename T, int NF>
static int launch_vq_prepare(const float* E, int64_t N, int K, int d, char* prep, hipStream_t st) {
  typedef typename DT<T>::frag_t frag_t;
  const VqPrep P = vq_prep_layout<T, NF>(N, K, d);
  const int npack_blocks = (P.npk + 255) / 256;
  const int kz = P.kpad > 64 ? P.kpad : 64;
  FRL_LAUNCH((vq_prepare_kernel<T, NF>), dim3(npack_blocks + (kz + 255) / 256), dim3(256), 0, st, E, K, d, (float*)(prep + P.en), P.kpad,
// ... 52 lines not shown
                  (float*)(ws + L.partial), (const bf16x8*)pk, (VqCtl*)(prep + P.ctl), counts, stats, (unsigned*)(ws + L.amb),      \
                  (float*)(ws + L.amb_lim));                                                                                       \
  } while (0)
      if (nt == 4) VQ_GOS(4); else if (nt == 2) VQ_GOS(2); else VQ_GOS(1);
#undef VQ_GOS
      return frl_check_launch("vq_assign");
    }
  }
  if (resident) {
    const int nwr = (nw == 8 && NF <= (sizeof(T) == 2 ? 2 : 4)) ? 8 : 4;
    const int batch = nwr * VQ_RES_NT * 16;
    const int64_t nb = (N + batch - 1) / batch;
    const int grid_r = (int)(nb < L.grid ? nb : L.grid);
    size_t lds = (size_t)(Kc / 16) * NF * 64 * sizeof(frag_t) + (size_t)Kc * 4 + (size_t)((K + 1) & ~1) * 4 + (size_t)VQ_FAST_ROWS * 12 +
                 (size_t)2 * batch * 4 + (size_t)nwr * 64 * 4 + 32 * 4 + (size_t)VQ_PZ_CAP * d * sizeof(T);
    const size_t fold = (size_t)2 * nwr * 64 * sizeof(double);
    if (lds < fold) lds = fold;
    if (lds > 160 * 1024) return frl_fail(-3, "vq_assign: LDS budget exceeded");
#define VQ_GO(NW_)                                                                                                                 \
  do {                                                                                                                             \
    auto kern = vq_assign_resident_kernel<T, NF, VQ_RES_NT, NW_>;                                                                          \
    if (lds > 64 * 1024) FRL_HIP(hipFuncSetAttribute((const void*)kern, hipFuncAttributeMaxDynamicSharedMemorySize, (int)lds));    \
    FRL_LAUNCH_AS("vq_assign_kernel", kern, dim3(grid_r), dim3(64 * NW_), lds, st, (const T*)z, E, en, N, K, d, Kc, idx, (T*)zq,   \
                  (float*)(ws + L.partial), pk, (VqCtl*)(prep + P.ctl), counts, stats);                                            \
  } while (0)
    if constexpr (NF <= (sizeof(T) == 2 ? 2 : 4)) {
      if (nwr == 8) VQ_GO(8); else VQ_GO(4);
    } else {
      VQ_GO(4);
    }
#undef VQ_GO
    return frl_check_launch("vq_assign");
  }
  const int Kc2 = Kc >= 32 ? Kc / 2 : Kc;
  const size_t lds = 2 * ((size_t)(Kc2 / 16) * NF * 64 * sizeof(frag_t) + (size_t)Kc2 * 4) + 64 + (K <= 2048 ? (size_t)K * 4 : 0);
  if (((Kc2 / 16) * NF * 64 * sizeof(frag_t)) % 1024 != 0 || (Kc2 & 63) != 0) return frl_fail(-3, "vq_assign: chunk is not a whole number of DMA pieces");
#define VQ_GO(NT_, NW_)                                                                                                            \
  do {                                                                                                                             \
    auto kern = vq_assign_kernel<T, NF, NT_, NW_>;                                                                                 \
    if (lds > 64 * 1024) FRL_HIP(hipFuncSetAttribute((const void*)kern, hipFuncAttributeMaxDynamicSharedMemorySize, (int)lds));    \
    FRL_LAUNCH_AS("vq_assign_kernel", kern, dim3(L.grid), dim3(64 * NW_), lds, st, (const T*)z, E, en, N, K, d, Kc2, idx, (T*)zq,   \
                  (float*)(ws + L.partial), (int32_t*)(ws + L.counts_fix), hdr, (int32_t*)(ws + L.amb), (float*)(ws + L.amb_lim), pk); \
  } while (0)
  if (nw == 8) VQ_GO(2, 8); else VQ_GO(4, 4);
#undef VQ_GO
  FRL_LAUNCH_AS("vq_fixup_tile_kernel", (vq_fixup_tile_kernel<T, NF>), dim3(1024), dim3(64 * VQ_FIXT_WAVES), 0, st, (const T*)z, E, en, pk, K, P.kpad, d,
                (const int32_t*)(ws + L.amb), (const float*)(ws + L.amb_lim), hdr, idx, (T*)zq, (int32_t*)(ws + L.counts_fix));
  FRL_LAUNCH(vq_finalize_kernel, dim3(1), dim3(256), 0, st, (const float*)(ws + L.partial), L.grid * nw, (const VqHeader*)hdr,
             (const int32_t*)(ws + L.counts_fix), counts, K, N, d, stats);
  return frl_check_launch("vq_assign");
}

static int vq_bwd_chunk(int K, int d) {
  int kc = K;
  while ((size_t)kc * d * 4 > 96 * 1024 && kc > 1) kc = (kc + 1) / 2;
  return kc;
}


__device__ __forceinline__ unsigned long long vq_splitmix64(unsigned long long x) {
  x += 0x9E3779B97F4A7C15ull;
  x = (x ^ (x >> 30)) * 0xBF58476D1CE4E5B9ull;
  x = (x ^ (x >> 27)) * 0x94D049BB133111EBull;
  return x ^ (x >> 31);
}
template <typename T>
__global__ __launch_bounds__(64) void vq_revive_kernel(float* __restrict__ E, const long long* __restrict__ window_counts, long long min_count,
                                                       const T* __restrict__ z, long long N, int K, int d, unsigned long long seed,
                                                       float* __restrict__ m, float* __restrict__ v, int* __restrict__ revived) {
  const int k = blockIdx.x;
  if (k >= K || window_counts[k] >= min_count) return;
  const unsigned long long r = vq_splitmix64(seed + (unsigned long long)k) % (unsigned long long)N;
  for (int j = threadIdx.x; j < d; j += 64) {
    E[(size_t)k * d + j] = to_f32(z[(size_t)r * d + j]);
    if (m != nullptr) m[(size_t)k * d + j] = 0.f;
    if (v != nullptr) v[(size_t)k * d + j] = 0.f;
  }
  if (threadIdx.x == 0) atomicAdd(revived, 1);
}

extern "C" {

int frl_vq_stream_tiles(int nt) {
  const int prev = g_vq_stream_tiles;
  g_vq_stream_tiles = nt < 0 ? -1 : nt;
  return prev;
}

size_t frl_vq_workspace_bytes(int64_t N, int K, int d) {
  const VqLayout L = vq_layout(N, K, d);
  const size_t bwd = (size_t)VQ_BWD_WGS * K * d * 4 + (size_t)K * d * 4;
  return L.total > bwd ? L.total : bwd;
}

#define VQ_DISPATCH(dtype, d, CALL)                                              \
  do {                                                                          \
    if ((dtype) == FRL_F32) {                                                   \
      if ((d) <= 16) return CALL(float, 4);                                     \
      if ((d) <= 32) return CALL(float, 8);                                     \
      if ((d) <= 64) return CALL(float, 16);                                    \
      return CALL(float, 32);                                                   \
    } else if ((dtype) == FRL_BF16) {                                           \
      if ((d) <= 32) return CALL(bf16, 1);                                      \
      if ((d) <= 64) return CALL(bf16, 2);                                      \
      return CALL(bf16, 4);                                                     \
    }                                                                           \
    return frl_fail(-2, "vq: bad dtype");                                       \
  } while (0)

size_t frl_vq_prepared_bytes(int K, int d) { return (K > 0 && d > 0 && d <= 128) ? vq_prep_bytes_max(K) : 0; }

int frl_vq_prepare(const float* E, int64_t N, int K, int d, int dtype, void* prep, size_t prep_bytes, hipStream_t stream) {
  if (N <= 0 || K <= 0 || d <= 0) return frl_fail(-2, "vq_prepare: empty input");
  if (d > 128) return frl_fail(-2, "vq_prepare: d > 128 unsupported");
  if (prep == nullptr || prep_bytes < frl_vq_prepared_bytes(K, d)) return frl_fail(-4, "vq_prepare: buffer too small");
#define VQ_CALL_PREP(T_, NF_) launch_vq_prepare<T_, NF_>(E, N, K, d, (char*)prep, stream)
  VQ_DISPATCH(dtype, d, VQ_CALL_PREP);
#undef VQ_CALL_PREP
}

int frl_vq_assign_fwd_prepared(const void* z, const float* E, void* prep, int64_t N, int K, int d, int32_t* idx_out, void* zq_out,
                               float* stats_out, int32_t* counts_out, int dtype, void* ws, size_t ws_bytes, hipStream_t stream) {
  if (N <= 0 || K <= 0 || d <= 0) return frl_fail(-2, "vq_assign: empty input");
  if (d > 128) return frl_fail(-2, "vq_assign: d > 128 unsupported");
  if (ws_bytes < frl_vq_workspace_bytes(N, K, d)) return frl_fail(-4, "vq_assign: workspace too small");
#define VQ_CALL_FWD(T_, NF_) launch_vq<T_, NF_>(z, E, (char*)prep, N, K, d, idx_out, zq_out, stats_out, counts_out, (char*)ws, stream)
  VQ_DISPATCH(dtype, d, VQ_CALL_FWD);
#undef VQ_CALL_FWD
}

int frl_vq_assign_fwd(const void* z, const float* E, int64_t N, int K, int d, int32_t* idx_out, void* zq_out,
                      float* stats_out, int32_t* counts_out, int dtype, void* ws, size_t ws_bytes, hipStream_t stream) {
  return frl_vq_assign_fwd_prepared(z, E, nullptr, N, K, d, idx_out, zq_out, stats_out, counts_out, dtype, ws, ws_bytes, stream);
}

int frl_vq_bwd(const void* g_out, const void* z, const void* zq, const float* E, const int32_t* idx, const int32_t* counts,
               const float* gscale, float beta, int64_t N, int K, int d, void* g_z_out, float* g_E_out,
               float* sums_out, int dtype, void* ws, size_t ws_bytes, hipStream_t stream) {
  if (N <= 0) return frl_fail(-2, "vq_bwd: empty input");
  if (ws_bytes < frl_vq_workspace_bytes(N, K, d)) return frl_fail(-4, "vq_bwd: workspace too small");
  const int Kc = vq_bwd_chunk(K, d);
  const size_t lds = (size_t)Kc * d * 4;
  const int64_t rows = (N + VQ_BWD_WGS - 1) / VQ_BWD_WGS;
  const float cz = beta * 2.f / ((float)N * (float)d), ce = 2.f / ((float)N * (float)d);
  float* slab = (float*)ws;
  if (dtype == FRL_F32) {
    auto kern = vq_bwd_kernel<float>;
    if (lds > 64 * 1024) FRL_HIP(hipFuncSetAttribute((const void*)kern, hipFuncAttributeMaxDynamicSharedMemorySize, (int)lds));
    FRL_LAUNCH_AS("vq_bwd_kernel", kern, dim3(VQ_BWD_WGS), dim3(256), lds, stream, (const float*)g_out, (const float*)z, E, idx, gscale,
                       cz, N, K, d, Kc, rows, (float*)g_z_out, slab);
    launch_slab_reduce_deferrable<float, CodeEpi>((const float*)slab, VQ_BWD_WGS, (int64_t)K * d, CodeEpi{E, counts, gscale, ce, d, 0, g_E_out, sums_out}, stream, sums_out == nullptr);
  } else if (dtype == FRL_BF16) {
    const int64_t rows64 = (rows + 63) / 64 * 64;
    if (d <= 32) {
      FRL_LAUNCH((vq_bwd_mfma_kernel<4, 2, 8>), dim3(VQ_BWD_WGS), dim3(512), (size_t)64 * 40 * 2 + 256, stream, (const bf16*)g_out, (const bf16*)z, (const bf16*)zq, E, idx,
                 gscale, cz, N, K, d, rows64, (bf16*)g_z_out, slab);
    } else if (d <= 64) {
      FRL_LAUNCH((vq_bwd_mfma_kernel<4, 4, 8>), dim3(VQ_BWD_WGS), dim3(512), (size_t)64 * 72 * 2 + 256, stream, (const bf16*)g_out, (const bf16*)z, (const bf16*)zq, E, idx,
                 gscale, cz, N, K, d, rows64, (bf16*)g_z_out, slab);
    } else {
      FRL_LAUNCH((vq_bwd_mfma_kernel<2, 8, 8>), dim3(VQ_BWD_WGS), dim3(512), (size_t)64 * 136 * 2 + 256, stream, (const bf16*)g_out, (const bf16*)z, (const bf16*)zq, E, idx,
                 gscale, cz, N, K, d, rows64, (bf16*)g_z_out, slab);
    }
    launch_slab_reduce_deferrable<float, CodeEpi>((const float*)slab, VQ_BWD_WGS, (int64_t)K * d, CodeEpi{E, counts, gscale, ce, d, 1, g_E_out, sums_out}, stream, sums_out == nullptr);
  } else return frl_fail(-2, "vq_bwd: bad dtype");
  return frl_check_launch("vq_bwd");
}

int frl_vq_ema_update(const float* sums, const int32_t* counts, int K, int d, float decay, float eps, float* ema_count,
                      float* ema_sum, float* E, const float* ok, hipStream_t stream) {
  FRL_LAUNCH(vq_ema_kernel, dim3(1), dim3(256), 0, stream, sums, counts, K, d, decay, eps, ema_count, ema_sum, E, ok);
  return frl_check_launch("vq_ema_update");
}

int frl_vq_revive_dead_codes(float* E, const int64_t* window_counts, int64_t min_count, const void* z, int64_t N, int K, int d,
                             uint64_t seed, float* m, float* v, int32_t* revived, int dtype, hipStream_t stream) {
  if (K <= 0 || d <= 0) return frl_fail(-2, "vq_revive_dead_codes: bad codebook shape");
  if (N <= 0) return frl_fail(-2, "vq_revive_dead_codes: no candidate rows");
  if (dtype == FRL_F32)
    FRL_LAUNCH((vq_revive_kernel<float>), dim3(K), dim3(64), 0, stream, E, (const long long*)window_counts, (long long)min_count,
               (const float*)z, (long long)N, K, d, (unsigned long long)seed, m, v, revived);
  else if (dtype == FRL_BF16)
    FRL_LAUNCH((vq_revive_kernel<bf16>), dim3(K), dim3(64), 0, stream, E, (const long long*)window_counts, (long long)min_count,
               (const bf16*)z, (long long)N, K, d, (unsigned long long)seed, m, v, revived);
  else return frl_fail(-2, "vq_revive_dead_codes: dtype must be FRL_F32 or FRL_BF16");
  return frl_check_launch("vq_revive_dead_codes");
}

}
```

vq-vae_amd/frl_hip/_lib.py:

```python
from __future__ import annotations

import ctypes
import os
from ctypes import c_char_p, c_float, c_int, c_int64, c_size_t, c_void_p

_HERE = os.path.dirname(os.path.abspath(__file__))
LIB_PATH = os.path.join(_HERE, "libfrlhip_%s.so" % os.environ["FRL_HIP_LIB_TAG"] if os.environ.get("FRL_HIP_LIB_TAG") else "libfrlhip.so")

F32, BF16, F16 = 0, 1, 2
ACT_NONE, ACT_RELU, ACT_SIGMOID = 0, 1, 2

_lib = None


class FrlHipError(RuntimeError):
    pass


P, I, L, F, S, D = c_void_p, c_int, c_int64, c_float, c_size_t, ctypes.c_double
SIGNATURES = {
    "frl_version": (c_int, []),
    "frl_last_error": (c_char_p, []),
    "frl_device_arch": (c_int, [c_char_p, I]),
    "frl_kernel_timing_enable": (c_int, [I]),
    "frl_kernel_timing_report": (c_int, [c_char_p, I]),
    "frl_pack_cache_table_bytes": (S, []),
    "frl_pack_cache_create": (c_int, [P, S]),
    "frl_pack_cache_destroy": (c_int, [I]),
    "frl_pack_cache_activate": (c_int, [I]),
    "frl_pack_cache_images": (c_int, [I]),
    "frl_pack_cache_refresh": (c_int, [I, P]),
    "frl_conv_workspace_bytes": (S, [I, I, I]),
    "frl_conv1x1_fwd": (c_int, [P, P, P, P, L, I, I, I, I, P, S, P]),
    "frl_conv1x1_bwd_data": (c_int, [P, P, I, P, P, L, I, I, I, P, S, P]),
    "frl_conv1x1_bwd_data_add": (c_int, [P, P, I, P, P, P, L, I, I, I, P, S, P]),
    "frl_wgrad_set_max_workgroups": (c_int, [I]),
    "frl_conv3x3_wgrad_force_generic": (c_int, [I]),
    "frl_conv3x3_tile32": (c_int, [I]),
    "frl_conv1x1_bwd_weight_workspace_bytes": (S, [L, I, I]),
    "frl_conv1x1_bwd_weight": (c_int, [P, P, I, P, P, P, L, I, I, I, P, S, P]),
    "frl_conv_tap_bwd_weight": (c_int, [P, P, I, P, P, L, L, P, L, I, I, I, I, I, I, P, S, I, P]),
    "frl_vq_workspace_bytes": (S, [L, I, I]),
    "frl_vq_assign_fwd": (c_int, [P, P, L, I, I, P, P, P, P, I, P, S, P]),
    "frl_vq_prepared_bytes": (S, [I, I]),
    "frl_vq_prepare": (c_int, [P, L, I, I, I, P, S, P]),
    "frl_vq_stream_tiles": (c_int, [I]),
    "frl_vq_assign_fwd_prepared": (c_int, [P, P, P, L, I, I, P, P, P, P, I, P, S, P]),
    "frl_vq_bwd": (c_int, [P, P, P, P, P, P, P, F, L, I, I, P, P, P, I, P, S, P]),
    "frl_vq_ema_update": (c_int, [P, P, I, I, F, F, P, P, P, P, P]),
    "frl_vq_revive_dead_codes": (c_int, [P, P, L, P, L, I, I, ctypes.c_uint64, P, P, P, I, P]),
    "frl_groupnorm_fwd": (c_int, [P, P, P, P, P, P, I, I, I, I, F, I, I, P]),
    "frl_groupnorm_bwd_workspace_bytes": (S, [I, I, I]),
    "frl_groupnorm_bwd": (c_int, [P, P, P, P, P, P, P, P, P, I, I, I, I, I, I, P, S, P]),
    "frl_scalar_combine": (c_int, [P, P, I, P, P, P]),
    "frl_scalar_fanout": (c_int, [P, P, I, P, P]),
    "frl_scalar_combine_dev": (c_int, [P, P, P, I, P, P, P]),
    "frl_scalar_combine_aux": (c_int, [P, P, P, P, I, P, P, P, P]),
    "frl_scalar_fanout_dev": (c_int, [P, P, P, I, P, P]),
    "frl_scalar_fanout_guard": (c_int, [P, P, P, P, I, P, P, P]),
    "frl_encoder2_supported": (c_int, [I, I, I, I, I, I, I]),
    "frl_encoder2_workspace_bytes": (S, [I]),
    "frl_encoder2_fwd": (c_int, [P, P, P, P, P, P, P, P, P, I, I, F, P, S, P]),
    "frl_encoder2_bwd": (c_int, [P, P, P, P, P, P, P, P, P, P, P, P, P, P, P, I, I, P, S, P]),
    "frl_decoder_mse_fused_supported": (c_int, [I, I, I, I]),
    "frl_decoder_mse_workspace_bytes": (S, [L, I]),
    "frl_decoder_mse_fwd": (c_int, [P, P, P, P, P, P, P, P, P, L, I, P, S, P]),
    "frl_decoder_mse_bwd": (c_int, [P, P, P, P, P, P, P, P, P, P, P, P, P, P, L, I, P, S, P]),
    "frl_decoder_mse_onepass_bytes": (S, [L, I]),
    "frl_decoder_mse_fwd_bwd": (c_int, [P, P, P, P, P, P, P, P, P, P, P, S, P, P, L, I, P]),
    "frl_decoder_mse_reduce": (c_int, [P, I, P, P, P, P, I, P]),
    "frl_mse_workspace_bytes": (S, []),
    "frl_mse_fwd": (c_int, [P, P, P, L, I, P, I, P, S, P]),
    "frl_mse_bwd": (c_int, [P, P, P, P, P, L, I, P, I, P]),
    "frl_film_modulate_fwd": (c_int, [P, P, P, P, L, I, L, I, I, P]),
    "frl_film_modulate_bwd": (c_int, [P, P, P, P, P, P, L, I, L, I, I, P]),
    "frl_film_fused_supported": (c_int, [I, I, I, I]),
    "frl_film_fused_workspace_bytes": (S, []),
    "frl_film_fused_fwd": (c_int, [P] * 13 + [I, I, I, P, S, P]),
    "frl_film_fused_bwd": (c_int, [P] * 20 + [I, I, I, P, S, P]),
    "frl_gate_blend_fwd": (c_int, [P, P, P, F, P, P, L, I, P]),
    "frl_gate_blend_bwd": (c_int, [P, P, P, P, F, P, P, L, I, P]),
    "frl_mean_time_fwd": (c_int, [P, P, L, I, L, I, P]),
    "frl_add": (c_int, [P, P, F, P, L, I, P]),
    "frl_normalize_tiles": (c_int, [P, I, P, P, P, I, P, L, I, P]),
    "frl_gather_locations_fwd": (c_int, [P, L, L, L, I, I, I, P, L, P, I, P]),
    "frl_segment_sum_rows": (c_int, [P, P, P, L, I, P, L, I, P]),
    "frl_infonce_fwd": (c_int, [P, I, P, P, P, L, P, L, F, I, P, P, P, P, P, P]),
    "frl_infonce_pair_grads": (c_int, [P, I, P, P, P, P, L, L, F, I, P, P, P]),
    "frl_mutual_knn_max_points": (S, [I]),
    "frl_mutual_knn": (c_int, [P, I, I, P, P, F, I, P, P, P]),
    "frl_host_parallel_copy": (c_int, [P, P, S, I]),
    "frl_normalize_chunk_tiles": (c_int, [P, I, I, I, I, I, P, I, I, P, P, I, P, P]),
    "frl_conv3x3_fwd": (c_int, [P, P, P, P, I, I, I, I, I, I, I, P, S, P]),
    "frl_conv3x3_fwd_gate_blend": (c_int, [P, P, P, P, P, P, P, I, I, I, I, I, I, P, S, P]),
    "frl_conv3x3_bwd_data": (c_int, [P, P, I, P, P, I, I, I, I, I, I, P, S, P]),
    "frl_conv3x3_bwd_data_fused": (c_int, [P, P, I, P, P, P, P, P, I, I, I, I, I, I, P, S, P]),
    "frl_conv3x3_bwd_weight_workspace_bytes": (S, [I, I, I, I, I]),
    "frl_conv3x3_bwd_weight": (c_int, [P, P, I, P, P, P, I, I, I, I, I, I, P, S, I, P]),
    "frl_sobel_fwd": (c_int, [P, P, I, I, I, I, I, P]),
    "frl_sobel_bwd": (c_int, [P, P, I, I, I, I, I, P]),
    "frl_sobel_bwd_add": (c_int, [P, P, P, I, I, I, I, I, P]),
    "frl_edge_smooth_stencil_fwd": (c_int, [P, P, P, P, P, P, P, I, I, I, I, I, I, I, P]),
    "frl_edge_smooth_stencil_bwd": (c_int, [P, P, P, P, P, P, P, P, I, I, I, I, I, I, I, P]),
    "frl_smooth_heads_supported": (c_int, [I, I, I, I]),
    "frl_smooth_heads_workspace_bytes": (S, [L]),
    "frl_smooth_heads_bwd_scratch_bytes": (S, [L]),
    "frl_smooth_heads_force_gather": (c_int, [I]),
    "frl_smooth_heads_fwd": (c_int, [P, P, P, P, P, P, P, P, I, I, I, I, P, S, P]),
    "frl_smooth_heads_bwd": (c_int, [P, P, P, P, P, P, P, P, P, P, P, P, P, P, P, S, I, I, I, I, P, S, P]),
    "frl_tcn_block_fwd": (c_int, [P, P, P, P, P, P, P, P, P, P, L, I, I, I, I, I, I, F, I, P, S, P]),
    "frl_tcn_block_bwd_data": (c_int, [P, P, P, P, P, L, I, I, I, I, I, I, P, S, P]),
    "frl_tcn_block_bwd_workspace_bytes": (S, [L, I]),
    "frl_tcn_block_bwd_fused_supported": (c_int, [I, I, I, I, I, I]),
    "frl_tcn_block_bwd_fused_workspace_bytes": (S, [L]),
    "frl_tcn_block_bwd_fused": (c_int, [P, P, P, P, P, P, P, P, P, P, P, P, P, P, P, L, I, I, I, I, F, P, S, P]),
    "frl_adamw_workspace_bytes": (S, []),
    "frl_adamw_clip_step": (c_int, [P, I, P, P, I, F, F, D, D, F, I, P, P, P, P, P, S, P]),
    "frl_multi_tensor_scale_copy": (c_int, [P, I, P, P, I, F, P]),
    "frl_tcn_hot_supported": (c_int, [I, I, I, I, I, I, I]),
    "frl_tcn_hot_fwd_workspace_bytes": (S, []),
    "frl_tcn_hot_bwd_workspace_bytes": (S, [L]),
    "frl_tcn_hot_fwd": (c_int, [P, P, P, P, P, P, P, P, P, L, I, I, F, P, S, P]),
    "frl_tcn_hot_bwd": (c_int, [P, P, P, P, P, P, P, P, P, P, P, P, P, P, P, P, L, I, I, F, P, S, P]),
    "frl_tcn_hot_force_generic_tiles": (c_int, [I]),
    "frl_decoder_mse_bwd_subgroups": (c_int, [I]),
    "frl_tcn_hot_bwd4_share": (c_int, [I, I]),
    "frl_tcn_chain_static_tiles": (c_int, [I]),
    "frl_conv3x3_bwd_data_outmask": (c_int, [P, P, I, P, P, P, I, I, I, I, I, I, I, P, S, P]),
    "frl_gate_blend_bwd_masked": (c_int, [P, P, P, P, F, P, P, L, I, I, P]),
    "frl_smooth_heads_bwd_masked": (c_int, [P, P, P, P, P, P, P, P, P, P, P, P, P, P, P, S, I, I, I, I, I, P, S, P]),
    "frl_tcn_hot_bwd_head_supported": (c_int, [L, I, I]),
    "frl_tcn_hot_bwd_head_workspace_bytes": (S, [L]),
    "frl_tcn_hot_bwd_head": (c_int, [P, P, P, I, P, P, P, P, P, P, P, P, P, P, P, P, P, L, I, I, F, P, S, P]),
    "frl_defer_begin": (c_int, []),
    "frl_defer_pending": (c_int, []),
    "frl_defer_destinations": (c_int, [P, I]),
    "frl_defer_flush": (c_int, [P]),
    "frl_defer_abort": (c_int, []),
    "frl_tcn_hot_bwd_nodx_supported": (c_int, [L, I]),
    "frl_tcn_chain_fwd_workspace_bytes": (S, []),
    "frl_tcn_chain_fwd": (c_int, [P] * 13 + [L, I, I, F, P, S, P]),
    "frl_tcn_chain_fwd_xt": (c_int, [P] * 14 + [L, I, I, F, P, S, P]),
    "frl_tcn_block_bwd": (c_int, [P, P, P, P, P, P, P, P, P, P, P, P, P, P, P, P, L, I, I, I, I, I, I, F, I, P, S, P]),
    "frl_decode_codes": (c_int, [P, P, P, L, I, I, I, P, P]),
    "frl_vicreg_workspace_bytes": (S, [L, I]),
    "frl_vicreg_fwd": (c_int, [P, L, I, I, F, F, F, F, P, P, P, P, S, P]),
    "frl_vicreg_bwd": (c_int, [P, P, P, P, L, I, I, F, F, F, F, P, P]),
    "frl_soft_nbr_fwd": (c_int, [P, P, P, P, L, I, F, F, I, P, P, P, P, P]),
    "frl_soft_nbr_bwd": (c_int, [P, P, P, P, P, L, I, P, P]),
    "frl_soft_nbr_gathered_fwd": (c_int, [P, I, P, I, I, P, P, P, P, P, P, L, I, I, F, F, I, P, P, P, P]),
    "frl_soft_nbr_gathered_bwd": (c_int, [P, I, P, I, I, P, P, P, P, P, P, L, I, I, F, F, I, P, P, P, P, P]),
    "frl_evt_soft_nbr_fwd": (c_int, [P, I, L, I, P, P, P, I, P, P, I, F, F, I, P, P, P, P, P]),
    "frl_evt_soft_nbr_bwd": (c_int, [P, I, L, I, P, P, P, I, P, P, I, F, F, P, P, P, P, P, P]),
}


def load():
    global _lib
    if _lib is not None:
        return _lib
    if not os.path.exists(LIB_PATH):
        raise FrlHipError(
            f"{LIB_PATH} not found: build it with `python vq-vae_amd/build.py` "
            "(hipcc --offload-arch=gfx950). There is no CPU fallback.")
    import torch
    lib = ctypes.CDLL(LIB_PATH)
    for name, (res, args) in SIGNATURES.items():
        fn = getattr(lib, name)
        fn.restype = res
        fn.argtypes = args
    _lib = lib
    return lib


def check(rc: int, what: str = "") -> None:
    if rc != 0:
        msg = load().frl_last_error()
        raise FrlHipError(f"{what} failed with code {rc}: {msg.decode() if msg else ''}")
```

vq-vae_amd/frl_hip/functional.py:

```python
from __future__ import annotations

from typing import Optional

import torch
from torch.autograd import Function
from torch.autograd.function import once_differentiable

from . import ops
from .ops import ACT_NONE, ACT_RELU, ACT_SIGMOID


def _c(t: Optional[torch.Tensor]):
    return None if t is None else (t if t.is_contiguous() else t.contiguous())


def _wanted(ctx, first: int, grads):
    out = []
    for i, g in enumerate(grads):
        if g is not None and not ctx.needs_input_grad[first + i]:
            ops.discard(g)
            g = None
        out.append(g)
    return tuple(out)

# ... 228 lines not shown
        dw_g0, db_g0 = wgrad3(3, dg1, res, y0, a0)
        pre_f = pre and ctx.fused_heads
        if ctx.fused_heads:
            dx, dfeat, dw_a, db_a, dw_b, db_b = ops.smooth_heads_bwd(d_tot, x, feat, w_a, b_a, w_b, b_b, dil, dx_add=dres_tot, dfeat_relu=pre_f)
        else:
            dx, da, db = ops.edge_smooth_bwd(d_tot, x, a_soft, b_soft, rank, dil, dx_add=dres_tot)
            dfeat = ops.conv1x1_bwd_data(db, w_b, None, ACT_NONE, add=ops.conv1x1_bwd_data(da, w_a, None, ACT_NONE))
            dw_a = dw_b = db_a = db_b = None
            if any(wants[1]):
                dw_a, db_a = ops.conv1x1_bwd_weight(da, feat, None, ACT_NONE, want_bias=wants[1][1])
            if any(wants[2]):
                dw_b, db_b = ops.conv1x1_bwd_weight(db, feat, None, ACT_NONE, want_bias=wants[2][1])
        af, yf = (ACT_NONE, None) if pre_f else (ACT_RELU, feat)
        dw_mb, db_mb = wgrad3(0, dfeat, g, yf, af)
        if ctx.needs_input_grad[0]:
            dx = ops.sobel_bwd(ops.conv3x3_bwd_data(dfeat, w_mb, yf, af), add=dx)
        else:
            dx = None
        heads = _wanted(ctx, 3, (None if dw_a is None else dw_a.reshape(w_a.shape), db_a if hb[1] else None,
                                 None if dw_b is None else dw_b.reshape(w_b.shape), db_b if hb[2] else None))
        return (dx, dw_mb, db_mb if hb[0] else None) + heads + (dw_g0, db_g0 if hb[3] else None, dw_g2, db_g2 if hb[4] else None,
                                                                None, None, None)


class TcnBlockFn(Function):

    @staticmethod
    def forward(ctx, x, conv_w, conv_b, gn_w, gn_b, gate_w, gate_b, proj_w, proj_b, dilation, groups, eps, drop_mask=None):
        pw = None if proj_w is None else proj_w.reshape(proj_w.shape[0], proj_w.shape[1])
        y = ops.tcn_block_fwd(x, conv_w, conv_b, gn_w, gn_b, gate_w, gate_b, pw, proj_b, dilation, groups, eps, drop_mask=drop_mask)
        ctx.cfg = (dilation, groups, eps)
        ctx.drop_mask = drop_mask
        ctx.save_for_backward(x, conv_w, conv_b, gn_w, gn_b, gate_w, gate_b, proj_w, proj_b)
        return y

    @staticmethod
    @once_differentiable
    def backward(ctx, dy):
        x, conv_w, conv_b, gn_w, gn_b, gate_w, gate_b, proj_w, proj_b = ctx.saved_tensors
        dilation, groups, eps = ctx.cfg
        pw = None if proj_w is None else proj_w.reshape(proj_w.shape[0], proj_w.shape[1])
        g = ops.tcn_block_bwd(x, _c(dy), conv_w, conv_b, gn_w, gn_b, gate_w, gate_b, pw, proj_b, dilation, groups, eps,
                              drop_mask=ctx.drop_mask, want_dx=ctx.needs_input_grad[0])
        dpw = g["proj_w"].reshape(proj_w.shape) if proj_w is not None else None
        return (g["dx"] if ctx.needs_input_grad[0] else None,) + _wanted(ctx, 1, (g["conv_w"], g["conv_b"], g["gn_w"], g["gn_b"], g["gate_w"],
                                                                                g["gate_b"], dpw, g.get("proj_b"))) + (None, None, None, None)


class TcnChainHeadFn(Function):

    @staticmethod
    def forward(ctx, x, *args):
        params, (head_w, head_b, groups, eps) = args[:18], args[18:22]
        want_xtype = len(args) > 22 and bool(args[22])
        blocks = [tuple(params[6 * i:6 * i + 6]) + (d, groups, False) for i, d in enumerate((1, 2, 4))]
        y1, y2, y3, h, *xt = ops.tcn_chain_fwd(x, blocks, head_w, head_b, eps, want_xtype=want_xtype)
        ctx.cfg = (groups, eps)
        ctx.n_tail = len(args) - 20
        ctx.save_for_backward(x, y1, y2, y3, head_w, *params)
        if want_xtype:
            ctx.mark_non_differentiable(xt[0])
            ctx.set_materialize_grads(False)
            return h, xt[0]
        return h

    @staticmethod
    @once_differentiable
    def backward(ctx, dh, _dxt=None):
        if dh is None:
            return (None,) * (21 + ctx.n_tail)
        x, y1, y2, y3, head_w, *params = ctx.saved_tensors
        groups, eps = ctx.cfg
        dh = _c(dh)
        w2 = head_w.reshape(head_w.shape[0], head_w.shape[1])
        dw_h = db_h = None
        if ctx.needs_input_grad[19] or ctx.needs_input_grad[20]:
            dw_h, db_h = ops.conv1x1_bwd_weight(dh, y3, None, ACT_NONE, want_bias=ctx.needs_input_grad[20])
            dw_h, = _wanted(ctx, 19, (dw_h.reshape(head_w.shape),))
        head_in_kernel = groups == 8 and ops.tcn_block_bwd_head_supported(y2, dh, w2, 4)
        dy = None if head_in_kernel else ops.conv1x1_bwd_data(dh, w2, None, ACT_NONE)
        grads = [None] * 18
        for i, (xin, dil) in reversed(list(enumerate(zip((x, y1, y2), (1, 2, 4))))):
            cw, cb, gw, gb, tw, tb = params[6 * i:6 * i + 6]
            if i == 2 and head_in_kernel:
                g = ops.tcn_block_bwd_head(xin, dh, w2, cw, cb, gw, gb, tw, tb, dil, eps)
            else:
                g = ops.tcn_block_bwd(xin, dy, cw, cb, gw, gb, tw, tb, None, None, dil, groups, eps, want_dx=(i > 0 or ctx.needs_input_grad[0]))
            grads[6 * i:6 * i + 6] = [g["conv_w"], g["conv_b"], g["gn_w"], g["gn_b"], g["gate_w"], g["gate_b"]]
            dy = g["dx"]
        return (dy if ctx.needs_input_grad[0] else None,) + _wanted(ctx, 1, grads) + (dw_h, db_h) + (None,) * ctx.n_tail


class FilmFn(Function):

    @staticmethod
    def forward(ctx, h, gamma, beta):
        ctx.save_for_backward(h, gamma)
        return ops.film_modulate_fwd(h, gamma, beta)

    @staticmethod
    @once_differentiable
    def backward(ctx, dout):
        h, gamma = ctx.saved_tensors
        return ops.film_modulate_bwd(_c(dout), h, gamma)


class FilmFusedFn(Function):

    @staticmethod
    def forward(ctx, h, z_type, *params):
        z, gamma, beta = ops.film_fused_fwd(z_type, h, params)
        ctx.save_for_backward(h, z_type, *params)
        ctx.mark_non_differentiable(gamma, beta)
        return z, gamma, beta

    @staticmethod
    @once_differentiable
    def backward(ctx, dz, _dg, _db):
        h, z_type, *params = ctx.saved_tensors
        dh, grads = ops.film_fused_bwd(z_type, h, _c(dz), params)
        return (dh if ctx.needs_input_grad[0] else None, None) + _wanted(ctx, 2, grads)


class ChannelScaleFn(Function):

    @staticmethod
    def forward(ctx, x, scale):
        b, c = scale.shape
        ctx.save_for_backward(scale)
        zero = torch.zeros_like(scale)
        ctx.zero = zero
        return ops.film_modulate_fwd(x.reshape(b, -1, 1, c), scale.reshape(b, 1, c), zero.reshape(b, 1, c)).reshape(x.shape)

    @staticmethod
    @once_differentiable
    def backward(ctx, dy):
        (scale,) = ctx.saved_tensors
        b, c = scale.shape
        dy = _c(dy)
        return ops.film_modulate_fwd(dy.reshape(b, -1, 1, c), scale.reshape(b, 1, c), ctx.zero.reshape(b, 1, c)).reshape(dy.shape), None


class VQFn(Function):

    @staticmethod
    def forward(ctx, z, codebook, prep=None):
        idx, zq, stats, counts = ops.vq_assign(z, codebook, prep)
        d = z.shape[-1]
        n = z.numel() // d
        ctx.set_materialize_grads(False)
        ctx.save_for_backward(z, codebook, idx, counts, zq)
        st = stats.clone()
        ctx.mark_non_differentiable(idx, counts, stats)
        return zq, st[3], st.narrow(0, 3, 1).reshape(()), st[1], idx, counts, stats

    @staticmethod
    @once_differentiable
    def backward(ctx, g_zq, g_cb, g_cm, g_perp, g_idx, g_counts, g_stats):
        z, codebook, idx, counts, zq = ctx.saved_tensors
        if g_cm is not None and g_cb is not None:
            gs = torch.stack([g_cm.reshape(()).float(), g_cb.reshape(()).float()])
        else:
            gs = torch.zeros(2, dtype=torch.float32, device=z.device)
            if g_cm is not None:
                gs[0] = g_cm
            if g_cb is not None:
                gs[1] = g_cb
        gz, ge, _ = ops.vq_bwd(_c(g_zq), z, codebook, idx, counts, gs, 1.0,
                               want_gz=ctx.needs_input_grad[0], want_ge=ctx.needs_input_grad[1], zq=zq)
        return gz, ge, None


class MseFn(Function):

    @staticmethod
    def forward(ctx, pred, target, mask):
        stats = ops.mse_fwd(pred, target, mask)
        ctx.save_for_backward(pred, target, mask, stats)
        return stats[0].clone()

    @staticmethod
    @once_differentiable
    def backward(ctx, g):
        pred, target, mask, stats = ctx.saved_tensors
        return ops.mse_bwd(pred, target, mask, g.reshape(1).float().contiguous(), stats), None, None


class DecoderMseFn(Function):

    @staticmethod
    def forward(ctx, z, w1, b1, w2, b2, target, mask, want_xhat, onepass=None):
        ctx.set_materialize_grads(False)
        ctx.onepass = onepass
        if onepass is not None:
            stats, dz, slabs = ops.decoder_mse_fwd_bwd(z, w1, b1, w2, b2, target, mask, onepass[0])
            ctx.held = (dz, slabs)
            ctx.save_for_backward(w1, b1, w2, b2)
            return stats.narrow(0, 0, 1).reshape(()), None
        stats, xhat = ops.decoder_mse_fwd(z, w1, b1, w2, b2, target, mask, want_xhat)
        ctx.save_for_backward(z, w1, b1, w2, b2, target, mask, stats)
        if xhat is not None:
            ctx.mark_non_differentiable(xhat)
        return stats.narrow(0, 0, 1).reshape(()), xhat

    @staticmethod
    @once_differentiable
    def backward(ctx, g, g_xhat):
        if ctx.onepass is not None:
            held, ctx.held = ctx.held, None
            if held is None:
                raise RuntimeError("decoder_mse: the gradients of a one-pass loss (grad_scale=) are handed out once; a second backward "
                                   "through it needs the two-kernel path (grad_scale=None)")
            if g is None:
                return (None,) * 9
            grad_scale, state = ctx.onepass
            if not state["guarded"]:
                ops.scalar_fanout(g.reshape(1).float().contiguous(), (1.0,), None, (grad_scale,))
            dz, slabs = held
            w1, b1, w2, b2 = ctx.saved_tensors
            gw = (None,) * 4
            if any(ctx.needs_input_grad[1:5]):
                dw1, db1, dw2, db2 = ops.decoder_mse_reduce(slabs, w1, b1, w2, b2)
                gw = _wanted(ctx, 1, (dw1.reshape(w1.shape), db1, dw2.reshape(w2.shape), db2))
            del held, slabs
            return (dz if ctx.needs_input_grad[0] else None,) + gw + (None, None, None, None)
        z, w1, b1, w2, b2, target, mask, stats = ctx.saved_tensors
        if g is None:
            return (None,) * 9
        dz, dw1, db1, dw2, db2 = ops.decoder_mse_bwd(z, w1, b1, w2, b2, target, mask, g.reshape(1).float().contiguous(), stats)
        return _wanted(ctx, 0, (dz, dw1.reshape(w1.shape), db1, dw2.reshape(w2.shape), db2)) + (None, None, None, None)


def decoder_mse(z, w1, b1, w2, b2, target, mask=None, want_xhat=False, grad_scale=None):
    if mask is not None:
        mask = mask.reshape(-1).to(torch.uint8).contiguous()
    if (grad_scale is not None and not want_xhat and torch.is_grad_enabled()
            and any(torch.is_tensor(t) and t.requires_grad for t in (z, w1, b1, w2, b2))):
        state = {"guarded": False}
        loss, xhat = DecoderMseFn.apply(z, w1, b1, w2, b2, target, mask, False, (grad_scale, state))
        loss._frl_promise = (grad_scale, state)
        return loss, xhat
    return DecoderMseFn.apply(z, w1, b1, w2, b2, target, mask, want_xhat)


def conv1x1(x, w, bias=None, act=ACT_NONE):
    return Conv1x1Fn.apply(x, w, bias, act)


def conv3x3(x, w, bias=None, act=ACT_NONE):
    return Conv3x3Fn.apply(x, w, bias, act)


def encoder2(x, w1, g1, b1, w2, g2, b2, eps=1e-5):
    return Encoder2Fn.apply(x, w1, g1, b1, w2, g2, b2, eps)


def group_norm(x, gamma, beta, groups, eps=1e-5, relu=False):
    return GroupNormFn.apply(x, gamma, beta, groups, eps, relu)


def mse_loss(pred, target, mask=None):
    if mask is not None:
        mask = mask.reshape(-1).to(torch.uint8).contiguous()
    return MseFn.apply(pred, target, mask)
```

vq-vae_amd/frl_hip/models/vqvae.py:

```python
from __future__ import annotations

from typing import Dict, Optional

import torch
import torch.distributed as dist
import torch.nn as nn

from .. import functional as Fh
from .. import ops
from ..losses.variance_covariance import variance_covariance_loss
from .blocks import Conv2DHead
from .representation import RepresentationModel


class VectorQuantizer(nn.Module):

    def __init__(self, codebook_size: int = 256, emb_dim: int = 64, beta: float = 0.25, quantizer: str = "st",
                 ema_decay: float = 0.99, ema_eps: float = 1e-5):
        super().__init__()
        if quantizer not in ("st", "ema"):
            raise ValueError("quantizer must be 'st' or 'ema' (scripts/train_vqvae.py:412)")
        self.codebook_size, self.emb_dim, self.beta = codebook_size, emb_dim, beta
        self.quantizer, self.ema_decay, self.ema_eps = quantizer, ema_decay, ema_eps
        self.codebook = nn.Parameter(torch.empty(codebook_size, emb_dim).uniform_(-1.0 / codebook_size, 1.0 / codebook_size),
                                     requires_grad=(quantizer == "st"))
        if quantizer == "ema":
            self.register_buffer("ema_count", torch.zeros(codebook_size))
            self.register_buffer("ema_sum", self.codebook.detach().clone())
        self.last_counts: Optional[torch.Tensor] = None
        self.last_stats: Optional[torch.Tensor] = None
        self.defer_ema = False
        self._pending_ema = None
        self._prepared = None

    def prepared(self, dtype: torch.dtype, n_rows: int) -> torch.Tensor:
        cb = self.codebook
        key = (cb.data_ptr(), cb._version, dtype)
        if self._prepared is None or self._prepared[0] != key:
            buf = self._prepared[1] if self._prepared is not None else None
            self._prepared = (key, ops.vq_prepare(cb.detach(), n_rows, dtype, out=buf))
        return self._prepared[1]

    def forward(self, z_rows: torch.Tensor, raw_terms: bool = False):
        zq, l_cb, l_cm, perp, idx, counts, stats = Fh.VQFn.apply(z_rows, self.codebook, self.prepared(z_rows.dtype, z_rows.shape[0]))
        self.last_counts = counts
        self.last_stats = stats
        if self.quantizer == "ema":
            vq_loss = Fh.scalar_combine([l_cm], [self.beta])[0]
            if self.training:
                with torch.no_grad():
                    _, _, sums = ops.vq_bwd(None, z_rows.detach(), self.codebook.detach(), idx, counts, None, 0.0,
                                            want_gz=False, want_ge=False, want_sums=True)
                self._pending_ema = (sums, counts)
                if not self.defer_ema:
                    self.apply_ema()
        elif raw_terms:
            vq_loss = ((l_cb, 1.0), (l_cm, float(self.beta)))
        else:
            vq_loss = Fh.scalar_combine([l_cb, l_cm], [1.0, self.beta])[0]
        return zq, vq_loss, perp, idx

    @torch.no_grad()
    def apply_ema(self, ok: Optional[torch.Tensor] = None) -> None:
        if self._pending_ema is None:
            return
        sums, counts = self._pending_ema
        self._pending_ema = None
        if dist.is_available() and dist.is_initialized() and dist.get_world_size() > 1:
            counts = counts.clone()
            dist.all_reduce(sums)
            dist.all_reduce(counts)
        ops.vq_ema_update(sums, counts, self.ema_count, self.ema_sum, self.codebook.data, self.ema_decay, self.ema_eps, ok)
        if self._prepared is not None:
            self._prepared = ((None, None, self._prepared[0][2]), self._prepared[1])
        if self.defer_ema:
            torch.autograd.graph.increment_version(self.codebook)

    def drop_ema(self) -> None:
        self._pending_ema = None


class VQVAE(RepresentationModel):

    def __init__(self, in_features: Optional[int] = None, codebook_size: int = 256, emb_dim: int = 64, beta: float = 0.25,
                 hidden: int = 128, quantizer: str = "st", ema_decay: float = 0.99, ema_eps: float = 1e-5,
                 phase: bool = True, phase_codebook_size: int = 0, lambda_recon: float = 1.0, lambda_vq: float = 1.0,
                 cont_dim: Optional[int] = None, cat_vocab_sizes=None, naip_bands: Optional[int] = None, cat_emb_dim: int = 8,
                 lambda_vcr: float = 0.0, vcr_variance_weight: float = 1.0, vcr_covariance_weight: float = 1.0,
                 vcr_variance_target: float = 1.0, **repr_kwargs):
        if cont_dim is not None:
            if in_features is not None and int(in_features) != int(cont_dim):
                raise ValueError(f"cont_dim ({cont_dim}) and in_features ({in_features}) name the same axis and disagree")
            in_features = int(cont_dim)
        if in_features is None:
            in_features = 64
        if cat_vocab_sizes:
            raise ValueError("cat_vocab_sizes is not empty: categorical inputs are not part of the (time, y, x, feature) tile VQ-VAE "
                             f"(got {sorted(dict(cat_vocab_sizes))}); pass an empty mapping")
        self_legacy = dict(cat_vocab_sizes=dict(cat_vocab_sizes or {}), naip_bands=None if naip_bands is None else int(naip_bands),
                           cat_emb_dim=int(cat_emb_dim))
        repr_kwargs.setdefault("z_type_dim", emb_dim)
        if repr_kwargs["z_type_dim"] != emb_dim:
            raise ValueError("emb_dim must equal z_type_dim (the quantizer acts on z_type)")
        if "type_encoder_channels" not in repr_kwargs and emb_dim != 64:
            repr_kwargs["type_encoder_channels"] = (128, emb_dim)
        super().__init__(type_in_channels=in_features, phase_in_channels=in_features, **repr_kwargs)
        self.in_features, self.phase, self.lambda_recon, self.lambda_vq = in_features, phase, lambda_recon, lambda_vq
        self.cont_dim, self.legacy_inputs = in_features, self_legacy
        if lambda_vcr < 0:
            raise ValueError("lambda_vcr must be >= 0")
        self.lambda_vcr = float(lambda_vcr)
        self.vcr_variance_weight, self.vcr_covariance_weight = float(vcr_variance_weight), float(vcr_covariance_weight)
        self.vcr_variance_target = float(vcr_variance_target)
        self.quant = VectorQuantizer(codebook_size, emb_dim, beta, quantizer, ema_decay, ema_eps)
        self.decoder_type = Conv2DHead(emb_dim, [hidden], in_features)
        if phase:
            self.decoder_phase = Conv2DHead(self.z_phase_dim, [hidden], in_features)
            if phase_codebook_size:
                self.quant_phase = VectorQuantizer(phase_codebook_size, self.z_phase_dim, beta, quantizer, ema_decay, ema_eps)
        self.lambda_vq_dev: Optional[torch.Tensor] = None
        self.codebook_manager = None
        self._manager_takes_rows = False
        self.defer_codebook_hooks = False
        self._pending_manager = None
        self.fused_decoder = True
        self.onepass_decoder = True
        self.chain_xtype = True
        self._grad_scale_dev = {}
        self.concurrent_phase = True
        self._side_stream = None

    def phase_stream(self, device):
        if self._side_stream is None:
            self._side_stream = torch.cuda.Stream(device=device)
        return self._side_stream

    def attach_codebook_manager(self, manager) -> None:
        import inspect
        self.codebook_manager = manager
        upd = getattr(manager, "update", None)
        self._manager_takes_rows = upd is not None and len(inspect.signature(upd).parameters) >= 2

    def _grad_scale(self, device) -> torch.Tensor:
        key = (str(device), float(self.lambda_recon))
        t = self._grad_scale_dev.get(key)
        if t is None:
            t = self._grad_scale_dev[key] = torch.full((1,), float(self.lambda_recon), dtype=torch.float32, device=device)
        return t

    def _vcr_term(self, z: torch.Tensor):
        total, _, _ = variance_covariance_loss(z.reshape(-1, z.shape[-1]), self.vcr_variance_weight, self.vcr_covariance_weight,
                                               self.vcr_variance_target)
        return (total, self.lambda_vcr)

    def _decode_loss(self, dec: Conv2DHead, z: torch.Tensor, target: torch.Tensor, mask, want_recon: bool, onepass: bool = False):
        l0, l2 = dec.layers[0], dec.layers[-1]
        if (len(dec.layers) == 3 and self.fused_decoder
                and ops.decoder_mse_supported(z.shape[-1], l0.out_channels, l2.out_channels, z)):
            w1 = l0.weight.reshape(l0.out_channels, l0.in_channels)
            w2 = l2.weight.reshape(l2.out_channels, l2.in_channels)
            gs = self._grad_scale(z.device) if (onepass and self.onepass_decoder and not want_recon) else None
            return Fh.decoder_mse(z, w1, l0.bias, w2, l2.bias, target, mask, want_recon, grad_scale=gs)
        xhat = dec(z)
        return Fh.mse_loss(xhat, target, mask), xhat

    def _phase_branch(self, tile, z_type_detached, mask, return_recon, onepass: bool = False, h=None) -> Dict[str, torch.Tensor]:
        b, t, hh, ww, f = tile.shape
        out: Dict[str, torch.Tensor] = {}
        z_phase = self.forward_phase_nhwc(tile, z_type_detached, h=h)
        zp_in = z_phase
        terms = []
        if hasattr(self, "quant_phase"):
            zpq, pvq, pperp, pidx = self.quant_phase(z_phase.reshape(-1, z_phase.shape[-1]))
            zp_in = zpq.reshape(z_phase.shape)
            terms.append(self._vq_term(pvq))
            out.update(idx_phase=pidx, vq_loss_phase=pvq, perplexity_phase=pperp)
        if mask is None or mask.dim() == 4:
            pmask = mask
        else:
            pmask = mask.unsqueeze(1).expand(b, t, hh, ww).contiguous()
        l_phase, xhat_phase = self._decode_loss(self.decoder_phase, zp_in, tile, pmask, return_recon, onepass)
        terms.append((l_phase, self.lambda_recon))
        if self.lambda_vcr > 0 and self.training:
            terms.append(self._vcr_term(z_phase))
            out["vcr_loss_phase"] = terms[-1][0].detach()
        out.update(z_phase=z_phase, l_phase=l_phase, loss_terms=terms)
        if xhat_phase is not None:
            out["xhat_phase"] = xhat_phase
        return out

    def forward_tiles(self, tile: torch.Tensor, mask: Optional[torch.Tensor] = None,
                      return_recon: bool = False, differentiable_vq_loss: bool = False) -> Dict[str, torch.Tensor]:
        self._require_gpu(tile)
        tile = self._rows(tile)
        b, t, hh, ww, f = tile.shape
        concurrent = self.phase and self.concurrent_phase and tile.is_cuda
        pre = None
        if self.phase and self.chain_xtype and tile.is_cuda and not differentiable_vq_loss:
            if concurrent:
                main, side = torch.cuda.current_stream(), self.phase_stream(tile.device)
                side.wait_stream(main)
                tile.record_stream(side)
                with torch.cuda.stream(side):
                    pre = self.phase_chain_xtype(tile)
                if pre is not None:
                    main.wait_stream(side)
                    pre[1].record_stream(main)
            else:
                pre = self.phase_chain_xtype(tile)
        if pre is not None:
            h_phase, x_type = pre
        else:
            h_phase = None
            with torch.no_grad():
                x_type = ops.mean_time(tile)
        z_type, gate = self.forward_nhwc(x_type, return_gate=True)
        side = ph = None
        onepass = self.training and not differentiable_vq_loss
        if concurrent:
            main, side = torch.cuda.current_stream(), self.phase_stream(tile.device)
            side.wait_stream(main)
            zt = z_type.detach()
            zt.record_stream(side)
            tile.record_stream(side)
            if mask is not None:
                mask.record_stream(side)
            with torch.cuda.stream(side):
                ph = self._phase_branch(tile, zt, mask, return_recon, onepass, h_phase)
        d = z_type.shape[-1]
        split_vq = self.quant.quantizer != "ema" and z_type.is_cuda and not differentiable_vq_loss
        zq, vq_loss, perp, idx = self.quant(z_type.reshape(-1, d), raw_terms=split_vq)
        vq_parts = vq_loss if split_vq else None
        tmask = mask.amin(dim=1) if (mask is not None and mask.dim() == 4) else mask
        l_type, xhat_type = self._decode_loss(self.decoder_type, zq.reshape(b, hh, ww, d), x_type, tmask, return_recon, onepass)
        out = dict(z_type=z_type, gate=gate, idx=idx, vq_loss=None if split_vq else vq_loss, perplexity=perp, l_type=l_type,
                   vq_stats=self.quant.last_stats)
        if xhat_type is not None:
            out["xhat_type"] = xhat_type
        if split_vq:
            terms = [(l_type, self.lambda_recon)]
            for part, w in vq_parts:
                t = self._vq_term(part)
                terms.append((t[0], t[1] * w) + tuple(t[2:]))
            aux = [0.0] + [w for _, w in vq_parts]
        else:
            terms = [(l_type, self.lambda_recon), self._vq_term(vq_loss)]
            aux = None
        if self.lambda_vcr > 0 and self.training:
            terms.append(self._vcr_term(z_type))
            out["vcr_loss"] = terms[-1][0].detach()
        if self.phase:
            if side is not None:
                main.wait_stream(side)
                for v in ph.values():
                    if torch.is_tensor(v):
                        v.record_stream(main)
            else:
                ph = self._phase_branch(tile, z_type.detach(), mask, return_recon, onepass, h_phase)
            terms += ph.pop("loss_terms")
            out.update(ph)
        res = Fh.scalar_combine([t[0] for t in terms], [float(t[1]) for t in terms], [t[2] if len(t) > 2 else None for t in terms],
                                aux_coefs=None if aux is None else aux + [0.0] * (len(terms) - len(aux)))
        loss, ok = res[0], res[1]
        if aux is not None:
            out["vq_loss"] = res[2]
        out["loss"] = loss
        if ok is not None:
            out["loss_ok"] = ok
        if self.codebook_manager is not None and hasattr(self.codebook_manager, "update") and self.training:
            self._pending_manager = (self.quant.last_counts, z_type.detach().reshape(-1, d))
            if not self.defer_codebook_hooks:
                self.commit_codebook_hooks()
        return out

    @torch.no_grad()
    def encode_tiles(self, tile: torch.Tensor, mask: Optional[torch.Tensor] = None, return_latents: bool = False) -> Dict[str, torch.Tensor]:
        self._require_gpu(tile)
        was_training = self.training
        self.eval()
        try:
            tile = self._rows(tile)
            b, t, hh, ww, f = tile.shape
            z_type = self.forward_nhwc(ops.mean_time(tile))
            d = z_type.shape[-1]
            rows = z_type.reshape(-1, d)
            q = self.quant
            idx, _, stats, counts = ops.vq_assign(rows, q.codebook.detach(), q.prepared(rows.dtype, rows.shape[0]))
            out = dict(idx=idx.reshape(b, hh, ww), counts=counts, perplexity=stats.narrow(0, 1, 1).reshape(()))
            want_phase = self.phase and (hasattr(self, "quant_phase") or return_latents)
            z_phase = self.forward_phase_nhwc(tile, z_type, inference=True) if want_phase else None
            if z_phase is not None and hasattr(self, "quant_phase"):
                qp = self.quant_phase
                prow = z_phase.reshape(-1, z_phase.shape[-1])
                pidx, _, pstats, pcounts = ops.vq_assign(prow, qp.codebook.detach(), qp.prepared(prow.dtype, prow.shape[0]))
                out.update(idx_phase=pidx.reshape(b, t, hh, ww), counts_phase=pcounts, perplexity_phase=pstats.narrow(0, 1, 1).reshape(()))
            if mask is not None:
                m = mask.to(torch.uint8)
                out["valid"] = (m.amin(dim=1) if m.dim() == 4 else m).to(torch.bool)
            if return_latents:
                out["z_type"] = z_type
                if z_phase is not None:
                    out["z_phase"] = z_phase
            return out
        finally:
            self.train(was_training)

    def _code_table(self, q: "VectorQuantizer", dec: Conv2DHead) -> torch.Tensor:
        rows = q.codebook.detach().to(self.compute_dtype).contiguous()
        l0, l2 = dec.layers[0], dec.layers[-1]
        if (len(dec.layers) == 3 and self.fused_decoder
                and ops.decoder_mse_supported(rows.shape[-1], l0.out_channels, l2.out_channels, rows)):
            w1 = l0.weight.detach().reshape(l0.out_channels, l0.in_channels)
            w2 = l2.weight.detach().reshape(l2.out_channels, l2.in_channels)
            target = torch.zeros(rows.shape[0], l2.out_channels, dtype=rows.dtype, device=rows.device)
            return ops.decoder_mse_fwd(rows, w1, l0.bias.detach(), w2, l2.bias.detach(), target, None, want_xhat=True)[1]
        return dec(rows)

    @torch.no_grad()
    def decode_codes(self, idx: Optional[torch.Tensor] = None, idx_phase: Optional[torch.Tensor] = None) -> Dict[str, torch.Tensor]:
        out: Dict[str, torch.Tensor] = {}
        if idx is not None:
            out["xhat_type"] = ops.decode_codes(idx, self._code_table(self.quant, self.decoder_type))
        if idx_phase is not None:
            if not hasattr(self, "quant_phase"):
                raise ValueError("decode_codes: idx_phase given but the model has no phase codebook (phase_codebook_size=0)")
            out["xhat_phase"] = ops.decode_codes(idx_phase, self._code_table(self.quant_phase, self.decoder_phase))
        return out

    @torch.no_grad()
    def init_codebook_from_tiles(self, tile: torch.Tensor, seed: int = 0) -> None:
        self._require_gpu(tile)
        tile = self._rows(tile)
        was_training = self.training
        self.eval()
        try:
            z_type = self.forward_nhwc(ops.mean_time(tile))
            gen = torch.Generator(device="cpu").manual_seed(int(seed))

            def draw(rows: torch.Tensor, q: "VectorQuantizer"):
                rows = rows.reshape(-1, rows.shape[-1]).float()
                if rows.shape[0] < q.codebook_size:
                    raise ValueError(f"init_codebook_from_tiles: {rows.shape[0]} encoder rows for {q.codebook_size} codes")
                pick = torch.randperm(rows.shape[0], generator=gen)[:q.codebook_size].to(rows.device)
                q.codebook.copy_(rows[pick])
                if q.quantizer == "ema":
                    q.ema_sum.copy_(q.codebook)
                    q.ema_count.fill_(1.0)

            draw(z_type, self.quant)
            if hasattr(self, "quant_phase"):
                draw(self.forward_phase_nhwc(tile, z_type), self.quant_phase)
        finally:
            self.train(was_training)

    def _vq_term(self, vq_loss):
        if self.lambda_vq_dev is not None and vq_loss.is_cuda:
            return (vq_loss, 1.0, self.lambda_vq_dev)
        return (vq_loss, self.lambda_vq)

    def _quantizers(self):
        return [q for q in (getattr(self, "quant", None), getattr(self, "quant_phase", None)) if q is not None]

    def set_defer_codebook_hooks(self, on: bool) -> None:
        self.defer_codebook_hooks = bool(on)
        for qz in self._quantizers():
            qz.defer_ema = bool(on)

    def commit_codebook_hooks(self, ok: Optional[torch.Tensor] = None) -> None:
        for qz in self._quantizers():
            if qz.quantizer == "ema":
                qz.apply_ema(ok)
        pend, self._pending_manager = self._pending_manager, None
        if pend is not None and self.codebook_manager is not None:
            counts, rows = pend
            if self._manager_takes_rows:
                if ok is not None:
                    self.codebook_manager.update(counts, rows, ok=ok)
                else:
                    self.codebook_manager.update(counts, rows)
            else:
                self.codebook_manager.update(counts if ok is None else counts * (ok > 0).to(counts.dtype))

    def drop_codebook_hooks(self) -> None:
        self._pending_manager = None
        for qz in self._quantizers():
            qz.drop_ema()

# ... 6 lines not shown
```

vq-vae_amd/frl_hip/ops.py:

```python
from __future__ import annotations

import ctypes
from typing import Optional, Tuple

import torch

from . import _lib
from ._lib import ACT_NONE, ACT_RELU, ACT_SIGMOID, BF16, F32, check

_WS = {}

_TIMING = {"on": False, "events": {}}


def set_timing(on: bool) -> None:
    _TIMING["on"] = bool(on)
    _TIMING["events"] = {}


def timing_summary():
    torch.cuda.synchronize()
    return {k: (len(v), sum(a.elapsed_time(b) for a, b in v)) for k, v in _TIMING["events"].items()}


# ... 912 lines not shown
    ws = workspace(lib.frl_tcn_chain_fwd_workspace_bytes(), x.device)
    ys = [torch.empty_like(x) for _ in range(3)] if keep_intermediates else [None] * 3
    h = torch.empty(x.shape[:-1] + (ch,), dtype=x.dtype, device=x.device)
    if torch.is_tensor(want_xtype):
        xt, want_xtype = want_xtype, True
        if xt.dtype != x.dtype or xt.device != x.device or not xt.is_contiguous() or xt.numel() < b * hw * c:
            raise ValueError("tcn_chain_fwd: the x_type buffer must be contiguous, of x's dtype and device, with >= B*HW*C elements")
    else:
        xt = torch.empty((b,) + tuple(x.shape[2:]), dtype=x.dtype, device=x.device) if want_xtype else None
    arr = ctypes.c_void_p * 3
    cols = [arr(*[_f32(blk[i] if i != 4 else blk[i].reshape(c, c), "tcn parameter").data_ptr() for blk in blocks]) for i in range(6)]
    check(lib.frl_tcn_chain_fwd_xt(_p(x), *[ctypes.cast(a, ctypes.c_void_p) for a in cols], _p(_f32(head_w.reshape(ch, c), "head_w")),
                                   _p(_f32(head_b, "head_b")), _p(ys[0]), _p(ys[1]), _p(ys[2]), _p(h), _p(xt), b * hw, hw, ch, float(eps),
                                   _p(ws), ws.numel(), _stream()), "frl_tcn_chain_fwd_xt")
    return (ys[0], ys[1], ys[2], h, xt) if want_xtype else (ys[0], ys[1], ys[2], h)


@_timed("tcn_block_bwd")
def tcn_block_bwd_head_supported(x, dh, head_w, dilation: int) -> bool:
    b, t, cin = x.shape[0], x.shape[1], x.shape[-1]
    hw = x.numel() // (b * t * cin)
    lib = _lib.load()
    return bool(fusion_enabled("headbwd") and dilation == 4 and x.dtype == torch.bfloat16 and dh.dtype == torch.bfloat16 and
                lib.frl_tcn_hot_supported(t, cin, cin, 8, dilation, 0, _dt(x)) and
                lib.frl_tcn_hot_bwd_head_supported(b * hw, hw, int(head_w.shape[0])))


@_timed("tcn_block_bwd")
def tcn_block_bwd_head(x, dh, head_w, conv_w, conv_b, gn_w, gn_b, gate_w, gate_b, dilation: int, eps: float = 1e-5):
    b, t, cin = x.shape[0], x.shape[1], x.shape[-1]
    cout = conv_w.shape[0]
    hw = x.numel() // (b * t * cin)
    npix = b * hw
    ch = int(head_w.shape[0])
    _chk_rows(dh, ch, "tcn_block_bwd_head.dh")
    lib = _lib.load()
    dx = torch.empty_like(x)
    g = {k: grad_empty(v.shape, x.device) for k, v in
         dict(conv_w=conv_w, conv_b=conv_b, gn_w=gn_w, gn_b=gn_b, gate_w=gate_w, gate_b=gate_b).items()}
    ws = workspace(lib.frl_tcn_hot_bwd_head_workspace_bytes(npix), x.device)
    with span("tcn_block_bwd.main"):
        check(lib.frl_tcn_hot_bwd_head(_p(x), _p(dh), _p(_f32(head_w.reshape(ch, cin), "head_w")), ch, _p(conv_w), _p(conv_b), _p(gn_w), _p(gn_b),
                                       _p(gate_w.reshape(cout, cout)), _p(gate_b), _p(dx), _p(g["conv_w"]), _p(g["conv_b"]), _p(g["gn_w"]),
                                       _p(g["gn_b"]), _p(g["gate_w"]), _p(g["gate_b"]), npix, hw, dilation, float(eps), _p(ws), ws.numel(),
                                       _stream()), "frl_tcn_hot_bwd_head")
    g["dx"] = dx
    return g


def tcn_block_bwd(x, dy, conv_w, conv_b, gn_w, gn_b, gate_w, gate_b, proj_w, proj_b, dilation: int, groups: int,
                  eps: float = 1e-5, allow_fused: bool = True, allow_hot: bool = True, drop_mask=None, want_dx: bool = True):
    b, t, cin = x.shape[0], x.shape[1], x.shape[-1]
    cout = conv_w.shape[0]
    hw = x.numel() // (b * t * cin)
    npix = b * hw
    lib = _lib.load()
    dev = x.device
    hot = bool(allow_fused and allow_hot and lib.frl_tcn_hot_supported(t, cin, cout, groups, dilation, int(proj_w is not None), _dt(x)))
    _check_drop_mask(drop_mask, x, hot)
    if hot:
        skip_dx = (not want_dx) and drop_mask is None and bool(lib.frl_tcn_hot_bwd_nodx_supported(npix, hw))
        dx = None if skip_dx else torch.empty_like(x)
        g = {k: grad_empty(v.shape, x.device) for k, v in
             dict(conv_w=conv_w, conv_b=conv_b, gn_w=gn_w, gn_b=gn_b, gate_w=gate_w, gate_b=gate_b).items()}
        ws = workspace(lib.frl_tcn_hot_bwd_workspace_bytes(npix), dev)
        with span("tcn_block_bwd.main"):
            check(lib.frl_tcn_hot_bwd(_p(x), _p(drop_mask), _p(dy), _p(conv_w), _p(conv_b), _p(gn_w), _p(gn_b), _p(gate_w.reshape(cout, cout)), _p(gate_b),
                                      _p(dx), _p(g["conv_w"]), _p(g["conv_b"]), _p(g["gn_w"]), _p(g["gn_b"]), _p(g["gate_w"]),
                                      _p(g["gate_b"]), npix, hw, dilation, float(eps), _p(ws), ws.numel(), _stream()), "frl_tcn_hot_bwd")
        g["dx"] = dx
        return g
    if allow_fused and lib.frl_tcn_block_bwd_fused_supported(t, cin, cout, groups, int(proj_w is not None), _dt(x)):
        dx = torch.empty_like(x)
        g = {k: grad_empty(v.shape, x.device) for k, v in
             dict(conv_w=conv_w, conv_b=conv_b, gn_w=gn_w, gn_b=gn_b, gate_w=gate_w, gate_b=gate_b).items()}
        ws = workspace(lib.frl_tcn_block_bwd_fused_workspace_bytes(npix), dev)
        with span("tcn_block_bwd.main"):
            check(lib.frl_tcn_block_bwd_fused(_p(x), _p(dy), _p(conv_w), _p(conv_b), _p(gn_w), _p(gn_b),
                                              _p(gate_w.reshape(cout, cout)), _p(gate_b), _p(dx), _p(g["conv_w"]), _p(g["conv_b"]),
                                              _p(g["gn_w"]), _p(g["gn_b"]), _p(g["gate_w"]), _p(g["gate_b"]), npix, hw, t, dilation,
                                              groups, float(eps), _p(ws), ws.numel(), _stream()), "frl_tcn_block_bwd_fused")
        g["dx"] = dx
        return g
    oshape = x.shape[:-1] + (cout,)
    dconv = torch.empty(oshape, dtype=x.dtype, device=dev)
    dgpre, normed, dres = torch.empty_like(dconv), torch.empty_like(dconv), torch.empty_like(dconv)
    dgam, dbet = grad_empty((cout,), dev), grad_empty((cout,), dev)
    gate_w2 = gate_w.reshape(cout, cout)
    ws = workspace(lib.frl_tcn_block_bwd_workspace_bytes(npix, cout), dev)
    with span("tcn_block_bwd.main"):
        check(lib.frl_tcn_block_bwd(_p(x), _p(dy), _p(conv_w), _p(conv_b), _p(gn_w), _p(gn_b), _p(gate_w2), _p(gate_b), _p(proj_w),
                                    _p(proj_b), _p(dconv), _p(dgpre), _p(normed), _p(dres), _p(dgam), _p(dbet), npix, hw, t, cin,
                                    cout, dilation, groups, float(eps), _dt(x), _p(ws), ws.numel(), _stream()), "frl_tcn_block_bwd")
    dx = torch.empty_like(x)
    ws1 = workspace(lib.frl_conv_workspace_bytes(max(cin, cout), max(cin, cout), 6), dev)
    check(lib.frl_tcn_block_bwd_data(_p(dconv), _p(dres), _p(conv_w), _p(proj_w), _p(dx), npix, hw, t, cin, cout, dilation,
                                     _dt(x), _p(ws1), ws1.numel(), _stream()), "frl_tcn_block_bwd_data")
    p = b * t * hw
    dw, dcb = grad_empty((cout, cin, 3), dev), grad_empty((cout,), dev)
    ws2 = workspace(lib.frl_conv1x1_bwd_weight_workspace_bytes(p, max(cin, cout), cout), dev)
    for k in range(3):
        check(lib.frl_conv_tap_bwd_weight(_p(dconv), None, 0, _p(x), ctypes.c_void_p(dw.data_ptr() + 4 * k), cin * 3, 3,
                                          _p(dcb) if k == 1 else None, p, cin, cout, hw, t, (k - 1) * dilation, _dt(x),
                                          _p(ws2), ws2.numel(), 0, _stream()), "frl_conv_tap_bwd_weight")
    dgw, dgb = _conv1x1_bwd_weight_impl(dgpre, normed)
    out = dict(dx=dx, conv_w=dw, conv_b=dcb, gn_w=dgam, gn_b=dbet, gate_w=dgw.reshape(gate_w.shape), gate_b=dgb)
    if proj_w is not None:
        dpw, dpb = _conv1x1_bwd_weight_impl(dres, x)
        out.update(proj_w=dpw.reshape(proj_w.shape), proj_b=dpb)
    return out


def decoder_mse_supported(cz: int, hidden: int, features: int, t: torch.Tensor) -> bool:
    return bool(_lib.load().frl_decoder_mse_fused_supported(cz, hidden, features, _dt(t)))


@_timed("decoder_mse_fwd")
def decoder_mse_fwd(z, w1, b1, w2, b2, target, mask=None, want_xhat: bool = False):
    cz = z.shape[-1]
    p = z.numel() // cz
    lib = _lib.load()
    ws = workspace(lib.frl_decoder_mse_workspace_bytes(p, cz), z.device)
    out = torch.empty(2, dtype=torch.float32, device=z.device)
    xhat = torch.empty_like(target) if want_xhat else None
    check(lib.frl_decoder_mse_fwd(_p(z), _p(w1), _p(b1), _p(w2), _p(b2), _p(target), _p(mask), _p(xhat), _p(out), p, cz, _p(ws),
                                  ws.numel(), _stream()), "frl_decoder_mse_fwd")
    return out, xhat


@_timed("decoder_mse_bwd")
def decoder_mse_bwd(z, w1, b1, w2, b2, target, mask, gscale, stats):
    cz = z.shape[-1]
    p = z.numel() // cz
    lib = _lib.load()
    ws = workspace(lib.frl_decoder_mse_workspace_bytes(p, cz), z.device)
    dz = torch.empty_like(z)
    dw1, db1, dw2, db2 = (grad_empty(t.shape, z.device) for t in (w1, b1, w2, b2))
    check(lib.frl_decoder_mse_bwd(_p(z), _p(w1), _p(b1), _p(w2), _p(b2), _p(target), _p(mask), _p(gscale), _p(stats), _p(dz), _p(dw1),
                                  _p(db1), _p(dw2), _p(db2), p, cz, _p(ws), ws.numel(), _stream()), "frl_decoder_mse_bwd")
    return dz, dw1, db1, dw2, db2


_DEC_CTL = {}


def _dec_ctl(device) -> torch.Tensor:
    key = (str(device), torch.cuda.current_stream().cuda_stream)
    c = _DEC_CTL.get(key)
    if c is None:
        c = _DEC_CTL[key] = torch.zeros(4, dtype=torch.int32, device=device)
    return c


@_timed("decoder_mse_fwd_bwd")
def decoder_mse_fwd_bwd(z, w1, b1, w2, b2, target, mask, grad_scale):
    cz = z.shape[-1]
    p = z.numel() // cz
    lib = _lib.load()
    if grad_scale is not None and (grad_scale.dtype != torch.float32 or grad_scale.numel() != 1 or grad_scale.device != z.device):
        raise ValueError("decoder_mse_fwd_bwd: grad_scale is a float32 scalar on the input's device")
    buf = torch.empty(lib.frl_decoder_mse_onepass_bytes(p, cz), dtype=torch.uint8, device=z.device)
    out = torch.empty(2, dtype=torch.float32, device=z.device)
    dz = torch.empty_like(z)
    nslab = ctypes.c_int(0)
    check(lib.frl_decoder_mse_fwd_bwd(_p(z), _p(w1), _p(b1), _p(w2), _p(b2), _p(target), _p(mask), _p(grad_scale), _p(out), _p(dz), _p(buf),
                                      buf.numel(), _p(_dec_ctl(z.device)), ctypes.cast(ctypes.byref(nslab), ctypes.c_void_p), p, cz, _stream()),
          "frl_decoder_mse_fwd_bwd")
    return out, dz, (buf, int(nslab.value))


@_timed("decoder_mse_reduce")
def decoder_mse_reduce(slabs, w1, b1, w2, b2):
    buf, nslab = slabs
    cz = w1.shape[-1]
    if _DEFER["on"]:
        _DEFER["keep"].append(buf)
    dw1, db1, dw2, db2 = (grad_empty(t.shape, buf.device) for t in (w1, b1, w2, b2))
    check(_lib.load().frl_decoder_mse_reduce(_p(buf), nslab, _p(dw1), _p(db1), _p(dw2), _p(db2), cz, _stream()), "frl_decoder_mse_reduce")
    return dw1, db1, dw2, db2


def _index_flag(device) -> torch.Tensor:
    device = torch.device(device)
    flag = _INDEX_FLAG.get(device)
    if flag is None:
        flag = _INDEX_FLAG[device] = torch.zeros(1, dtype=torch.int32, device=device)
    return flag


@_timed("decode_codes")
def decode_codes(idx: torch.Tensor, table: torch.Tensor) -> torch.Tensor:
    import os
    if table.dim() != 2:
        raise ValueError(f"decode_codes: table must be [K, F], got {tuple(table.shape)}")
    k, f = table.shape
    _chk_rows(table, f, "decode_codes.table")
    if not idx.is_cuda or idx.device != table.device:
        raise _lib.FrlHipError("decode_codes: idx must live on the table's GPU (no CPU fallback)")
    if idx.dtype == torch.int64:
        idx = idx.clamp(-k - 1, k).to(torch.int32)
    elif idx.dtype != torch.int32:
        raise TypeError(f"decode_codes: idx must be int32 or int64, got {idx.dtype}")
    idx = idx.contiguous()
    out = torch.empty(tuple(idx.shape) + (f,), dtype=table.dtype, device=table.device)
    p = idx.numel()
    if p == 0:
        return out
    check_now = os.environ.get("FRL_HIP_CHECK_INDICES", "0") == "1"
    flag = torch.zeros(1, dtype=torch.int32, device=table.device) if check_now else _index_flag(table.device)
    check(_lib.load().frl_decode_codes(_p(idx), _p(table), _p(out), p, k, f, _dt(table), _p(flag), _stream()), "frl_decode_codes")
    if check_now:
        _index_flag(table.device).bitwise_or_(flag)
        if bool(flag.item()):
            raise IndexError(f"decode_codes: code index out of range for {k} codes")
    return out


@_timed("gather_locations")
def gather_locations(feature: torch.Tensor, coords: torch.Tensor) -> torch.Tensor:
    if not feature.is_cuda:
        raise _lib.FrlHipError("gather_locations: tensor must live on the GPU (no CPU fallback)")
    c, h, w = feature.shape
    if coords.dtype != torch.int64 or not coords.is_contiguous() or coords.device != feature.device:
        raise ValueError("gather_locations: coords must be a contiguous int64 [N, 2] tensor on the feature's device")
    n = coords.shape[0]
    out = torch.empty(n, c, dtype=feature.dtype, device=feature.device)
    sc, sh, sw = feature.stride()
    check(_lib.load().frl_gather_locations_fwd(_p(feature), sc, sh, sw, c, h, w, _p(coords), n, _p(out), _dt(feature), _stream()),
          "frl_gather_locations_fwd")
    return out


@_timed("segment_sum_rows")
def segment_sum_rows(vals: torch.Tensor, order: Optional[torch.Tensor], keys_sorted: torch.Tensor, out: torch.Tensor, accumulate: bool = False):
    m, d = vals.shape
    if vals.dtype != torch.float32 or not vals.is_contiguous() or out.dtype != torch.float32 or not out.is_contiguous() or out.shape[-1] != d:
        raise ValueError("segment_sum_rows: vals [M, D] and out [.., D] must be contiguous float32")
    for t in (order, keys_sorted):
        if t is not None and (t.dtype != torch.int64 or not t.is_contiguous() or t.numel() != m):
            raise ValueError("segment_sum_rows: order / keys must be contiguous int64 [M]")
    check(_lib.load().frl_segment_sum_rows(_p(vals), _p(order), _p(keys_sorted), m, d, _p(out), d, int(accumulate), _stream()),
          "frl_segment_sum_rows")
    return out


@_timed("infonce_fwd")
def infonce_fwd(emb, pairs, weights, is_pos, seg, temperature: float, sim: int, want_coef: bool = True):
    t, d = pairs.shape[0], emb.shape[1]
    sims = torch.empty(t, dtype=torch.float32, device=emb.device)
    logits = torch.empty_like(sims)
    nseg = seg.numel() - 1
    loss_a = torch.empty(nseg, dtype=torch.float32, device=emb.device)
    coef = torch.empty_like(sims) if want_coef else None
    loss = torch.empty(1, dtype=torch.float32, device=emb.device)
    check(_lib.load().frl_infonce_fwd(_p(emb), d, _p(pairs), _p(weights), _p(is_pos), t, _p(seg), nseg, float(temperature), int(sim),
                                      _p(sims), _p(logits), _p(loss_a), _p(coef), _p(loss), _stream()), "frl_infonce_fwd")
    return loss, sims, coef


@_timed("infonce_bwd")
def infonce_pair_grads(emb, pairs, sims, coef, gscale, nseg: int, temperature: float, sim: int):
    t, d = pairs.shape[0], emb.shape[1]
    ga = torch.empty(t, d, dtype=torch.float32, device=emb.device)
    gb = torch.empty_like(ga)
    check(_lib.load().frl_infonce_pair_grads(_p(emb), d, _p(pairs), _p(sims), _p(coef), _p(gscale), t, nseg, float(temperature), int(sim),
                                             _p(ga), _p(gb), _stream()), "frl_infonce_pair_grads")
    return ga, gb


def _chk_vicreg(x: torch.Tensor, name: str):
    if not x.is_cuda:
        raise _lib.FrlHipError(f"{name}: tensor must live on the GPU (no CPU fallback)")
    if x.dim() != 2 or not x.is_contiguous() or x.shape[0] < 2 or not (1 <= x.shape[1] <= 128):
        raise ValueError(f"{name}: expected contiguous rows [N >= 2, 1 <= D <= 128], got {tuple(x.shape)} stride {x.stride()}")


@_timed("vicreg_fwd")
def vicreg_fwd(x: torch.Tensor, variance_weight: float = 1.0, covariance_weight: float = 1.0, variance_target: float = 1.0,
               eps: float = 1e-4, want_grad: bool = True):
    _chk_vicreg(x, "vicreg_fwd")
    n, d = x.shape
    losses = torch.empty(3, dtype=torch.float32, device=x.device)
    cov = torch.empty(d, d, dtype=torch.float32, device=x.device) if want_grad else None
    centre = torch.empty(2, d, dtype=torch.float32, device=x.device) if want_grad else None
    lib = _lib.load()
    ws = workspace(lib.frl_vicreg_workspace_bytes(n, d), x.device)
    check(lib.frl_vicreg_fwd(_p(x), n, d, _dt(x), float(variance_weight), float(covariance_weight), float(variance_target), float(eps),
                             _p(losses), _p(cov), _p(centre), _p(ws), ws.numel(), _stream()), "frl_vicreg_fwd")
    return losses, cov, centre


@_timed("vicreg_bwd")
def vicreg_bwd(x: torch.Tensor, cov: torch.Tensor, centre: torch.Tensor, g3: torch.Tensor, variance_weight: float = 1.0,
               covariance_weight: float = 1.0, variance_target: float = 1.0, eps: float = 1e-4) -> torch.Tensor:
    _chk_vicreg(x, "vicreg_bwd")
    n, d = x.shape
    for t, shape, name in ((cov, (d, d), "cov"), (centre, (2, d), "centre"), (g3, (3,), "g3")):
        if t.dtype != torch.float32 or tuple(t.shape) != shape or not t.is_contiguous() or t.device != x.device:
            raise ValueError(f"vicreg_bwd: {name} must be a contiguous float32 {shape} tensor on the device of x")
    dx = torch.empty_like(x)
    check(_lib.load().frl_vicreg_bwd(_p(x), _p(cov), _p(centre), _p(g3), n, d, _dt(x), float(variance_weight), float(covariance_weight),
                                     float(variance_target), float(eps), _p(dx), _stream()), "frl_vicreg_bwd")
    return dx


SOFT_NBR_MAX_M, SOFT_NBR_MAX_WIDTH = 32, 256


def _chk_soft_nbr(name: str, tau_ref: float, tau_learned: float, min_valid_per_row: int):
    if int(min_valid_per_row) < 2:
        raise ValueError(f"min_valid_per_row must be >= 2, got {min_valid_per_row}")
    if not (tau_ref > 0 and tau_learned > 0):
        raise ValueError(f"{name}: temperatures must be positive, got tau_ref={tau_ref} tau_learned={tau_learned}")


def _soft_nbr_weights(weights: Optional[torch.Tensor], b: int, device, name: str):
    if weights is None:
# ... 168 lines not shown
```

Baseline: 111,800.

## Fold VQ commitment gradient into fused one-pass decoder MSE backward kernel

Computes the quantizer's straight-through/commitment term cz*(z_pre - zq) directly inside the one-pass decoder backward epilogue when writing dz, so the VQ backward kernel no longer has to read g_out/z/zq and write g_z. Adds a GZ template flag to the VQ backward MFMA kernel so it can run in a sums-only mode without the gz pass. It also reworks the autograd plumbing so VQFn exposes a decoder-facing zq output and a fold context, and the model enables the fold by default. In exchange it adds an extra z_pre load per row in the decoder kernel and more complex Python autograd coordination.

```diff
diff --git a/include/frl_hip.h b/include/frl_hip.h
--- a/include/frl_hip.h
+++ b/include/frl_hip.h
@@ -225,6 +225,10 @@
 int frl_decoder_mse_fwd_bwd(const void* z, const float* w1, const float* b1, const float* w2, const float* b2, const void* target,
                             const uint8_t* mask, const float* gscale, float* out, void* dz, void* buf, size_t buf_bytes, void* ctl,
                             int* nslab, int64_t P, int Cz, frl_stream_t stream);
+int frl_decoder_mse_vq_supported(int Cz, int hidden, int F, int dtype);
+int frl_decoder_mse_fwd_bwd_vq(const void* z, const float* w1, const float* b1, const float* w2, const float* b2, const void* target,
+                               const uint8_t* mask, const float* gscale, float* out, void* dz, void* buf, size_t buf_bytes, void* ctl,
+                               int* nslab, int64_t P, int Cz, const void* z_pre, const float* vq_gscale, float beta, frl_stream_t stream);
 int frl_decoder_mse_reduce(const void* buf, int nslab, float* dw1, float* db1, float* dw2, float* db2, int Cz, frl_stream_t stream);
 int frl_decoder_mse_bwd_subgroups(int on);
 
diff --git a/vq-vae_amd/csrc/dec_fused.hip b/vq-vae_amd/csrc/dec_fused.hip
--- a/vq-vae_amd/csrc/dec_fused.hip
+++ b/vq-vae_amd/csrc/dec_fused.hip
@@ -157,13 +157,21 @@
   float nv_host;
 };
 
-template <int NFZ, int NW, bool SG = false, bool LOSS = false>
+template <bool VQ> struct DecVq {};
+template <> struct DecVq<true> {
+  const TT* zpre;
+  const float* gscale;
+  float cz_base;
+};
+
+template <int NFZ, int NW, bool SG = false, bool LOSS = false, bool VQ = false>
 __global__ __launch_bounds__(SG ? 512 : 64 * NW) void dec_mse_bwd_kernel(const TT* __restrict__ Z, const frag8* __restrict__ Wpk, const float* __restrict__ b1,
                                                                const float* __restrict__ b2, const TT* __restrict__ TGT,
                                                                const uint8_t* __restrict__ mask, const float* __restrict__ gscale,
                                                                const float* __restrict__ stats, TT* __restrict__ DZ, int64_t P, int Cz,
-                                                               float* __restrict__ slab, const DecLoss<LOSS> la) {
+                                                               float* __restrict__ slab, const DecLoss<LOSS> la, const DecVq<VQ> vq = DecVq<VQ>{}) {
   constexpr int CZP = 32 * NFZ, CB = CZP / 16, R = 16 * NW, NTH = SG ? 512 : 64 * NW;
+  static_assert(!VQ || (NFZ == 2 && LOSS), "the quantizer fold rides on the 64-channel one-pass kernel");
   constexpr int PX = DF_F + 8, PH = DF_H + 8, PZ = CZP + 8;
   static_assert(!SG || NW == 4, "subgroups are four waves");
   extern __shared__ __attribute__((aligned(16))) char smem[];
@@ -199,6 +207,9 @@
   int nrow = 0;
   (void)sq; (void)nrow;
   const float ksc = nv > 0.f ? (gscale ? gscale[0] : 1.f) * 2.f / nv : 0.f;
+  float cz = 0.f;
+  if constexpr (VQ) cz = vq.cz_base * (vq.gscale ? vq.gscale[0] : 1.f);
+  (void)cz;
 
   constexpr int W2CB = (NW == 8) ? 4 : 8;
   const int w2row = (NW == 8) ? (wave & 3) : wave;
@@ -246,6 +257,8 @@
     if (!inb) row = P - 1;
     if (valid && mask != nullptr) valid = mask[row] != 0;
     fetch(zn, tn, wt + 3 * w_step);
+    LQTile<TT, 2> zp;
+    if constexpr (VQ) lq_load<TT, 2>(zp, vq.zpre, row, CZP, kc, true);
     float h[32], xh[16];
     LQTile<TT, 4> ht;
     dec_chain<NFZ>(h, xh, zt, w1, w2, b1q, b2q, ht, lane);
@@ -286,6 +299,10 @@
           bf16x8 o;
 #pragma unroll
           for (int e = 0; e < 8; ++e) o[e] = (bf16)dzacc[(j + e) >> 2][(j + e) & 3];
+          if constexpr (VQ) {
+#pragma unroll
+            for (int e = 0; e < 8; ++e) o[e] = (bf16)vq_gz_combine((float)o[e], cz, (float)zp.f[j >> 3][e], (float)zt.f[j >> 3][e]);
+          }
           *reinterpret_cast<bf16x8*>(dzp + j) = o;
         }
       } else if ((Cz & 3) == 0) {
@@ -444,20 +461,21 @@
 static unsigned df_fwd_grid(int64_t P) { int64_t g = ((P + 15) / 16 + 3) / 4; if (g > DF_GRID_MAX) g = DF_GRID_MAX; return (unsigned)(g < 1 ? 1 : g); }
 static unsigned df_bwd_grid(int64_t P, int R) { int64_t g = (P + R - 1) / R; if (g > 256) g = 256; return (unsigned)(g < 1 ? 1 : g); }
 
-template <int NFZ, int NW, bool LOSS = false>
+template <int NFZ, int NW, bool LOSS = false, bool VQ = false>
 static int launch_dec_bwd(const void* z, const float* w1, const float* b1, const float* w2, const float* b2, const void* tgt,
                           const uint8_t* mask, const float* gscale, const float* stats, void* dz, float* dw1, float* db1, float* dw2,
-                          float* db2, int64_t P, int Cz, char* ws, hipStream_t st, DecLoss<LOSS> la = DecLoss<LOSS>{}, int* nslab_out = nullptr) {
+                          float* db2, int64_t P, int Cz, char* ws, hipStream_t st, DecLoss<LOSS> la = DecLoss<LOSS>{}, int* nslab_out = nullptr,
+                          DecVq<VQ> vq = DecVq<VQ>{}) {
   constexpr int CZP = 32 * NFZ, CB = CZP / 16, R = 16 * NW;
   const unsigned grid = df_bwd_grid(P, R);
   const size_t slab_n = (size_t)DF_F * DF_H + DF_H * CZP + DF_F + DF_H;
   const frag8* pk = dec_packed<NFZ>(w1, w2, Cz, 1, reinterpret_cast<frag8*>(ws + ((grid * slab_n * sizeof(float) + 255) / 256) * 256), st);
   const size_t lds = (size_t)(8 * NFZ + 16 + 16 + CB * 4) * 64 * sizeof(frag8) + 192 * sizeof(float) +
                      (size_t)R * ((DF_F + 8) + 2 * (DF_H + 8) + (CZP + 8)) * sizeof(TT);
-  auto kern = dec_mse_bwd_kernel<NFZ, NW, false, LOSS>;
+  auto kern = dec_mse_bwd_kernel<NFZ, NW, false, LOSS, VQ>;
   FRL_HIP(hipFuncSetAttribute((const void*)kern, hipFuncAttributeMaxDynamicSharedMemorySize, (int)lds));
-  FRL_LAUNCH_AS(LOSS ? "dec_mse_bwd_loss_kernel" : "dec_mse_bwd_kernel", kern, dim3(grid), dim3(64 * NW), lds, st, (const TT*)z, (const frag8*)pk, b1, b2, (const TT*)tgt, mask, gscale, stats, (TT*)dz, P, Cz,
-             (float*)ws, la);
+  FRL_LAUNCH_AS(VQ ? "dec_mse_bwd_loss_vq_kernel" : LOSS ? "dec_mse_bwd_loss_kernel" : "dec_mse_bwd_kernel", kern, dim3(grid), dim3(64 * NW), lds, st, (const TT*)z, (const frag8*)pk, b1, b2, (const TT*)tgt, mask, gscale, stats, (TT*)dz, P, Cz,
+             (float*)ws, la, vq);
   if constexpr (LOSS) {
     FRL_LAUNCH(dec_mse_finalize_kernel, dim3(1), dim3(256), 0, st, (const double*)la.partial, (int)grid, la.out_w);
     *nslab_out = (int)grid;
@@ -483,7 +501,7 @@
   auto kern = dec_mse_bwd_kernel<NFZ, 4, true, LOSS>;
   FRL_HIP(hipFuncSetAttribute((const void*)kern, hipFuncAttributeMaxDynamicSharedMemorySize, (int)lds));
   FRL_LAUNCH_AS(LOSS ? "dec_mse_bwd_sg_loss_kernel" : "dec_mse_bwd_sg_kernel", kern, dim3(grid), dim3(512), lds, st, (const TT*)z, (const frag8*)pk, b1, b2, (const TT*)tgt, mask, gscale, stats, (TT*)dz, P,
-                Cz, (float*)ws, la);
+                Cz, (float*)ws, la, DecVq<false>{});
   if constexpr (LOSS) {
     FRL_LAUNCH(dec_mse_finalize_kernel, dim3(1), dim3(256), 0, st, (const double*)la.partial, (int)grid, la.out_w);
     *nslab_out = (int)nslab;
@@ -551,10 +569,25 @@
 static size_t df_onepass_partial_off(int64_t P, int Cz) { return ((frl_decoder_mse_workspace_bytes(P, Cz) + 255) / 256) * 256; }
 size_t frl_decoder_mse_onepass_bytes(int64_t P, int Cz) { return df_onepass_partial_off(P, Cz) + (size_t)256 * 2 * sizeof(double); }
 
+int frl_decoder_mse_fwd_bwd_vq(const void* z, const float* w1, const float* b1, const float* w2, const float* b2, const void* target,
+                               const uint8_t* mask, const float* gscale, float* out, void* dz, void* buf, size_t buf_bytes, void* ctl,
+                               int* nslab, int64_t P, int Cz, const void* z_pre, const float* vq_gscale, float beta, hipStream_t stream);
 int frl_decoder_mse_fwd_bwd(const void* z, const float* w1, const float* b1, const float* w2, const float* b2, const void* target,
                             const uint8_t* mask, const float* gscale, float* out, void* dz, void* buf, size_t buf_bytes, void* ctl,
                             int* nslab, int64_t P, int Cz, hipStream_t stream) {
+  return frl_decoder_mse_fwd_bwd_vq(z, w1, b1, w2, b2, target, mask, gscale, out, dz, buf, buf_bytes, ctl, nslab, P, Cz, nullptr, nullptr, 0.f,
+                                    stream);
+}
+
+int frl_decoder_mse_vq_supported(int Cz, int hidden, int F, int dtype) {
+  return (dtype == FRL_BF16 && hidden == DF_H && F == DF_F && Cz == 64) ? 1 : 0;
+}
+
+int frl_decoder_mse_fwd_bwd_vq(const void* z, const float* w1, const float* b1, const float* w2, const float* b2, const void* target,
+                               const uint8_t* mask, const float* gscale, float* out, void* dz, void* buf, size_t buf_bytes, void* ctl,
+                               int* nslab, int64_t P, int Cz, const void* z_pre, const float* vq_gscale, float beta, hipStream_t stream) {
   if (P <= 0) return frl_fail(-2, "decoder_mse_fwd_bwd: empty input");
+  if (z_pre != nullptr && Cz != 64) return frl_fail(-2, "decoder_mse_fwd_bwd_vq: the quantizer fold needs 64-channel latents");
   if (Cz < 1 || Cz > 64) return frl_fail(-2, "decoder_mse_fwd_bwd: latent width must be 1..64");
   if (buf_bytes < frl_decoder_mse_onepass_bytes(P, Cz)) return frl_fail(-4, "decoder_mse_fwd_bwd: buffer too small");
   if (out == nullptr || dz == nullptr || ctl == nullptr || nslab == nullptr) return frl_fail(-2, "decoder_mse_fwd_bwd: null output");
@@ -574,6 +607,13 @@
     return launch_dec_bwd_sg<1, true>(z, w1, b1, w2, b2, target, mask, gscale, nullptr, dz, nullptr, nullptr, nullptr, nullptr, P, Cz, (char*)buf, stream, la, nslab);
   if (Cz <= 32)
     return launch_dec_bwd<1, 8, true>(z, w1, b1, w2, b2, target, mask, gscale, nullptr, dz, nullptr, nullptr, nullptr, nullptr, P, Cz, (char*)buf, stream, la, nslab);
+  if (z_pre != nullptr) {
+    DecVq<true> vq;
+    vq.zpre = (const TT*)z_pre;
+    vq.gscale = vq_gscale;
+    vq.cz_base = beta * 2.f / ((float)P * (float)Cz);
+    return launch_dec_bwd<2, 4, true, true>(z, w1, b1, w2, b2, target, mask, gscale, nullptr, dz, nullptr, nullptr, nullptr, nullptr, P, Cz, (char*)buf, stream, la, nslab, vq);
+  }
   return launch_dec_bwd<2, 4, true>(z, w1, b1, w2, b2, target, mask, gscale, nullptr, dz, nullptr, nullptr, nullptr, nullptr, P, Cz, (char*)buf, stream, la, nslab);
 }
 
diff --git a/vq-vae_amd/csrc/frl_common.hpp b/vq-vae_amd/csrc/frl_common.hpp
--- a/vq-vae_amd/csrc/frl_common.hpp
+++ b/vq-vae_amd/csrc/frl_common.hpp
@@ -42,6 +42,8 @@
 template <typename T> __device__ __forceinline__ T from_f32(float v);
 template <> __device__ __forceinline__ float from_f32<float>(float v) { return v; }
 template <> __device__ __forceinline__ bf16 from_f32<bf16>(float v) { return (bf16)v; }
+
+__device__ __forceinline__ float vq_gz_combine(float g, float cz, float z, float q) { return fmaf(cz, z - q, g); }
 
 __device__ __forceinline__ float act_fwd(float v, int act) {
   if (act == FRL_ACT_RELU) return v > 0.f ? v : 0.f;
diff --git a/vq-vae_amd/csrc/vq.hip b/vq-vae_amd/csrc/vq.hip
--- a/vq-vae_amd/csrc/vq.hip
+++ b/vq-vae_amd/csrc/vq.hip
@@ -1452,7 +1452,7 @@
   }
 }
 
-template <int RB, int CB, int NWV>
+template <int RB, int CB, int NWV, bool GZ = true>
 __global__ __launch_bounds__(64 * NWV) void vq_bwd_mfma_kernel(const bf16* __restrict__ gout, const bf16* __restrict__ Z, const bf16* __restrict__ ZQ,
                                                           const float* __restrict__ E,
                                                           const int32_t* __restrict__ idx, const float* __restrict__ gscale, float cz_base,
@@ -1479,7 +1479,7 @@
       for (int b = 0; b < CB; ++b) acc[a][b] = f32x4{0.f, 0.f, 0.f, 0.f};
     constexpr int NV = (64 * (DP / 8) + NTH - 1) / NTH;
     const bool pre = fast && (ZQ != nullptr || gz == nullptr || kbase != 0);
-    const bool want_gz = (kbase == 0 && gz != nullptr);
+    const bool want_gz = GZ && (kbase == 0 && gz != nullptr);
     bf16x8 rz[NV], rg[NV], rq[NV];
     auto fetch = [&](int64_t p0) {
 #pragma unroll
@@ -1511,7 +1511,7 @@
           if (want_gz && n < r1 && c0 < d) {
             float ov[8];
 #pragma unroll
-            for (int e = 0; e < 8; ++e) ov[e] = (float)rg[u][e] + cz * ((float)rz[u][e] - (float)rq[u][e]);
+            for (int e = 0; e < 8; ++e) ov[e] = vq_gz_combine((float)rg[u][e], cz, (float)rz[u][e], (float)rq[u][e]);
             Vec<bf16>::store(gz + n * (int64_t)d + c0, ov);
           }
           *reinterpret_cast<bf16x8*>(zt + row * PITCH + c0) = rz[u];
@@ -1529,7 +1529,7 @@
 #pragma unroll
             for (int e = 0; e < 8; ++e) if (c0 + e < d) zv[e] = (float)Z[n * (int64_t)d + c0 + e];
           }
-          if (kbase == 0 && gz != nullptr) {
+          if (GZ && kbase == 0 && gz != nullptr) {
             const int k = idx[n];
             float gv[8], ov[8];
 #pragma unroll
@@ -1548,7 +1548,7 @@
               for (int e = 0; e < 8; ++e) qv[e] = (c0 + e < d) ? (float)(bf16)E[(int64_t)k * d + c0 + e] : 0.f;
             }
 #pragma unroll
-            for (int e = 0; e < 8; ++e) ov[e] = gv[e] + cz * (zv[e] - qv[e]);
+            for (int e = 0; e < 8; ++e) ov[e] = vq_gz_combine(gv[e], cz, zv[e], qv[e]);
             if (fast) Vec<bf16>::store(gz + n * (int64_t)d + c0, ov);
             else {
 #pragma unroll
@@ -1907,16 +1907,18 @@
     launch_slab_reduce_deferrable<float, CodeEpi>((const float*)slab, VQ_BWD_WGS, (int64_t)K * d, CodeEpi{E, counts, gscale, ce, d, 0, g_E_out, sums_out}, stream, sums_out == nullptr);
   } else if (dtype == FRL_BF16) {
     const int64_t rows64 = (rows + 63) / 64 * 64;
+#define VQ_BWD_MFMA(RB_, CB_, PITCH_, GZ_)                                                                                                    \
+  FRL_LAUNCH_AS(GZ_ ? "vq_bwd_mfma_kernel" : "vq_bwd_mfma_sums_kernel", (vq_bwd_mfma_kernel<RB_, CB_, 8, GZ_>), dim3(VQ_BWD_WGS), dim3(512),   \
+                (size_t)64 * PITCH_ * 2 + 256, stream, (const bf16*)g_out, (const bf16*)z, (const bf16*)zq, E, idx, gscale, cz, N, K, d, rows64, \
+                (bf16*)g_z_out, slab)
     if (d <= 32) {
-      FRL_LAUNCH((vq_bwd_mfma_kernel<4, 2, 8>), dim3(VQ_BWD_WGS), dim3(512), (size_t)64 * 40 * 2 + 256, stream, (const bf16*)g_out, (const bf16*)z, (const bf16*)zq, E, idx,
-                 gscale, cz, N, K, d, rows64, (bf16*)g_z_out, slab);
+      if (g_z_out != nullptr) VQ_BWD_MFMA(4, 2, 40, true); else VQ_BWD_MFMA(4, 2, 40, false);
     } else if (d <= 64) {
-      FRL_LAUNCH((vq_bwd_mfma_kernel<4, 4, 8>), dim3(VQ_BWD_WGS), dim3(512), (size_t)64 * 72 * 2 + 256, stream, (const bf16*)g_out, (const bf16*)z, (const bf16*)zq, E, idx,
-                 gscale, cz, N, K, d, rows64, (bf16*)g_z_out, slab);
+      if (g_z_out != nullptr) VQ_BWD_MFMA(4, 4, 72, true); else VQ_BWD_MFMA(4, 4, 72, false);
     } else {
-      FRL_LAUNCH((vq_bwd_mfma_kernel<2, 8, 8>), dim3(VQ_BWD_WGS), dim3(512), (size_t)64 * 136 * 2 + 256, stream, (const bf16*)g_out, (const bf16*)z, (const bf16*)zq, E, idx,
-                 gscale, cz, N, K, d, rows64, (bf16*)g_z_out, slab);
-    }
+      if (g_z_out != nullptr) VQ_BWD_MFMA(2, 8, 136, true); else VQ_BWD_MFMA(2, 8, 136, false);
+    }
+#undef VQ_BWD_MFMA
     launch_slab_reduce_deferrable<float, CodeEpi>((const float*)slab, VQ_BWD_WGS, (int64_t)K * d, CodeEpi{E, counts, gscale, ce, d, 1, g_E_out, sums_out}, stream, sums_out == nullptr);
   } else return frl_fail(-2, "vq_bwd: bad dtype");
   return frl_check_launch("vq_bwd");
diff --git a/vq-vae_amd/frl_hip/_lib.py b/vq-vae_amd/frl_hip/_lib.py
--- a/vq-vae_amd/frl_hip/_lib.py
+++ b/vq-vae_amd/frl_hip/_lib.py
@@ -68,6 +68,8 @@
     "frl_decoder_mse_bwd": (c_int, [P, P, P, P, P, P, P, P, P, P, P, P, P, P, L, I, P, S, P]),
     "frl_decoder_mse_onepass_bytes": (S, [L, I]),
     "frl_decoder_mse_fwd_bwd": (c_int, [P, P, P, P, P, P, P, P, P, P, P, S, P, P, L, I, P]),
+    "frl_decoder_mse_vq_supported": (c_int, [I, I, I, I]),
+    "frl_decoder_mse_fwd_bwd_vq": (c_int, [P, P, P, P, P, P, P, P, P, P, P, S, P, P, L, I, P, P, F, P]),
     "frl_decoder_mse_reduce": (c_int, [P, I, P, P, P, P, I, P]),
     "frl_mse_workspace_bytes": (S, []),
     "frl_mse_fwd": (c_int, [P, P, P, L, I, P, I, P, S, P]),
diff --git a/vq-vae_amd/frl_hip/functional.py b/vq-vae_amd/frl_hip/functional.py
--- a/vq-vae_amd/frl_hip/functional.py
+++ b/vq-vae_amd/frl_hip/functional.py
@@ -404,12 +404,13 @@
         ctx.save_for_backward(z, codebook, idx, counts, zq)
         st = stats.clone()
         ctx.mark_non_differentiable(idx, counts, stats)
-        return zq, st[3], st.narrow(0, 3, 1).reshape(()), st[1], idx, counts, stats
-
-    @staticmethod
-    @once_differentiable
-    def backward(ctx, g_zq, g_cb, g_cm, g_perp, g_idx, g_counts, g_stats):
+        return zq, st[3], st.narrow(0, 3, 1).reshape(()), st[1], idx, counts, stats, zq.detach()
+
+    @staticmethod
+    @once_differentiable
+    def backward(ctx, g_zq, g_cb, g_cm, g_perp, g_idx, g_counts, g_stats, g_dec=None):
         z, codebook, idx, counts, zq = ctx.saved_tensors
+        fold = getattr(ctx, "fold", None)
         if g_cm is not None and g_cb is not None:
             gs = torch.stack([g_cm.reshape(()).float(), g_cb.reshape(()).float()])
         else:
@@ -418,6 +419,18 @@
                 gs[0] = g_cm
             if g_cb is not None:
                 gs[1] = g_cb
+        if fold is not None and g_dec is not None and not fold["state"]["guarded"]:
+            gc = g_cm if g_cm is not None else torch.zeros((), dtype=torch.float32, device=z.device)
+            ops.scalar_fanout(gc.reshape(1).float().contiguous(), (1.0,), None, (fold["gscale"].narrow(0, 0, 1),))
+        if fold is not None and g_dec is not None and g_zq is None:
+            ge = None
+            if ctx.needs_input_grad[1]:
+                _, ge, _ = ops.vq_bwd(None, z, codebook, idx, counts, gs, 1.0, want_gz=False, want_ge=True, zq=zq)
+            return (g_dec if ctx.needs_input_grad[0] else None), ge, None
+        if g_dec is not None:
+            if fold is not None:
+                g_dec = fold["plain_dz"]()
+            g_zq = g_dec if g_zq is None else g_zq + g_dec.reshape(g_zq.shape)
         gz, ge, _ = ops.vq_bwd(_c(g_zq), z, codebook, idx, counts, gs, 1.0,
                                want_gz=ctx.needs_input_grad[0], want_ge=ctx.needs_input_grad[1], zq=zq)
         return gz, ge, None
@@ -441,11 +454,16 @@
 class DecoderMseFn(Function):
 
     @staticmethod
-    def forward(ctx, z, w1, b1, w2, b2, target, mask, want_xhat, onepass=None):
+    def forward(ctx, z, w1, b1, w2, b2, target, mask, want_xhat, onepass=None, fold=None):
         ctx.set_materialize_grads(False)
         ctx.onepass = onepass
         if onepass is not None:
-            stats, dz, slabs = ops.decoder_mse_fwd_bwd(z, w1, b1, w2, b2, target, mask, onepass[0])
+            vq = None
+            if fold is not None:
+                vq = (fold["z_pre"], fold["gscale"], 1.0)
+                zd = z.detach()
+                fold["plain_dz"] = lambda: ops.decoder_mse_fwd_bwd(zd, w1, b1, w2, b2, target, mask, onepass[0])[1]
+            stats, dz, slabs = ops.decoder_mse_fwd_bwd(z, w1, b1, w2, b2, target, mask, onepass[0], vq=vq)
             ctx.held = (dz, slabs)
             ctx.save_for_backward(w1, b1, w2, b2)
             return stats.narrow(0, 0, 1).reshape(()), None
@@ -464,7 +482,7 @@
                 raise RuntimeError("decoder_mse: the gradients of a one-pass loss (grad_scale=) are handed out once; a second backward "
                                    "through it needs the two-kernel path (grad_scale=None)")
             if g is None:
-                return (None,) * 9
+                return (None,) * 10
             grad_scale, state = ctx.onepass
             if not state["guarded"]:
                 ops.scalar_fanout(g.reshape(1).float().contiguous(), (1.0,), None, (grad_scale,))
@@ -475,22 +493,31 @@
                 dw1, db1, dw2, db2 = ops.decoder_mse_reduce(slabs, w1, b1, w2, b2)
                 gw = _wanted(ctx, 1, (dw1.reshape(w1.shape), db1, dw2.reshape(w2.shape), db2))
             del held, slabs
-            return (dz if ctx.needs_input_grad[0] else None,) + gw + (None, None, None, None)
+            return (dz if ctx.needs_input_grad[0] else None,) + gw + (None, None, None, None, None)
         z, w1, b1, w2, b2, target, mask, stats = ctx.saved_tensors
         if g is None:
-            return (None,) * 9
+            return (None,) * 10
         dz, dw1, db1, dw2, db2 = ops.decoder_mse_bwd(z, w1, b1, w2, b2, target, mask, g.reshape(1).float().contiguous(), stats)
-        return _wanted(ctx, 0, (dz, dw1.reshape(w1.shape), db1, dw2.reshape(w2.shape), db2)) + (None, None, None, None)
-
-
-def decoder_mse(z, w1, b1, w2, b2, target, mask=None, want_xhat=False, grad_scale=None):
+        return _wanted(ctx, 0, (dz, dw1.reshape(w1.shape), db1, dw2.reshape(w2.shape), db2)) + (None, None, None, None, None)
+
+
+def decoder_mse(z, w1, b1, w2, b2, target, mask=None, want_xhat=False, grad_scale=None, vq_fold=None):
     if mask is not None:
         mask = mask.reshape(-1).to(torch.uint8).contiguous()
     if (grad_scale is not None and not want_xhat and torch.is_grad_enabled()
             and any(torch.is_tensor(t) and t.requires_grad for t in (z, w1, b1, w2, b2))):
         state = {"guarded": False}
-        loss, xhat = DecoderMseFn.apply(z, w1, b1, w2, b2, target, mask, False, (grad_scale, state))
+        fold = None
+        if (vq_fold is not None and z.requires_grad and vq_fold[0].requires_grad and isinstance(z.grad_fn, VQFn._backward_cls)
+                and ops.decoder_mse_vq_supported(z.shape[-1], w1.shape[0], w2.shape[0], z)):
+            z_pre, l_cb, l_cm, gscale = vq_fold
+            fold = {"z_pre": _c(z_pre.detach().reshape(-1, z_pre.shape[-1])), "gscale": gscale, "state": {"guarded": False}}
+        loss, xhat = DecoderMseFn.apply(z, w1, b1, w2, b2, target, mask, False, (grad_scale, state), fold)
         loss._frl_promise = (grad_scale, state)
+        if fold is not None:
+            z.grad_fn.fold = fold
+            l_cm._frl_promise = (gscale.narrow(0, 0, 1), fold["state"])
+            l_cb._frl_promise = (gscale.narrow(0, 1, 1), fold["state"])
         return loss, xhat
     return DecoderMseFn.apply(z, w1, b1, w2, b2, target, mask, want_xhat)
 
diff --git a/vq-vae_amd/frl_hip/models/vqvae.py b/vq-vae_amd/frl_hip/models/vqvae.py
--- a/vq-vae_amd/frl_hip/models/vqvae.py
+++ b/vq-vae_amd/frl_hip/models/vqvae.py
@@ -41,8 +41,8 @@
             self._prepared = (key, ops.vq_prepare(cb.detach(), n_rows, dtype, out=buf))
         return self._prepared[1]
 
-    def forward(self, z_rows: torch.Tensor, raw_terms: bool = False):
-        zq, l_cb, l_cm, perp, idx, counts, stats = Fh.VQFn.apply(z_rows, self.codebook, self.prepared(z_rows.dtype, z_rows.shape[0]))
+    def forward(self, z_rows: torch.Tensor, raw_terms: bool = False, decoder_output: bool = False):
+        zq, l_cb, l_cm, perp, idx, counts, stats, zq_dec = Fh.VQFn.apply(z_rows, self.codebook, self.prepared(z_rows.dtype, z_rows.shape[0]))
         self.last_counts = counts
         self.last_stats = stats
         if self.quantizer == "ema":
@@ -58,6 +58,8 @@
             vq_loss = ((l_cb, 1.0), (l_cm, float(self.beta)))
         else:
             vq_loss = Fh.scalar_combine([l_cb, l_cm], [1.0, self.beta])[0]
+        if decoder_output:
+            return zq, vq_loss, perp, idx, zq_dec
         return zq, vq_loss, perp, idx
 
     @torch.no_grad()
@@ -126,6 +128,7 @@
         self.fused_decoder = True
         self.onepass_decoder = True
         self.chain_xtype = True
+        self.fold_vq_grad = True
         self._grad_scale_dev = {}
         self.concurrent_phase = True
         self._side_stream = None
@@ -148,19 +151,29 @@
             t = self._grad_scale_dev[key] = torch.full((1,), float(self.lambda_recon), dtype=torch.float32, device=device)
         return t
 
+    def _vq_grad_scale(self, device) -> torch.Tensor:
+        lam = 1.0 if self.lambda_vq_dev is not None else self.lambda_vq
+        key = (str(device), "vq", float(lam * float(self.quant.beta)), float(lam * 1.0))
+        t = self._grad_scale_dev.get(key)
+        if t is None:
+            t = self._grad_scale_dev[key] = torch.tensor(key[2:], dtype=torch.float32, device=device)
+        return t * self.lambda_vq_dev if self.lambda_vq_dev is not None else t
+
     def _vcr_term(self, z: torch.Tensor):
         total, _, _ = variance_covariance_loss(z.reshape(-1, z.shape[-1]), self.vcr_variance_weight, self.vcr_covariance_weight,
                                                self.vcr_variance_target)
         return (total, self.lambda_vcr)
 
-    def _decode_loss(self, dec: Conv2DHead, z: torch.Tensor, target: torch.Tensor, mask, want_recon: bool, onepass: bool = False):
+    def _decode_loss(self, dec: Conv2DHead, z: torch.Tensor, target: torch.Tensor, mask, want_recon: bool, onepass: bool = False,
+                     vq_fold=None):
         l0, l2 = dec.layers[0], dec.layers[-1]
         if (len(dec.layers) == 3 and self.fused_decoder
                 and ops.decoder_mse_supported(z.shape[-1], l0.out_channels, l2.out_channels, z)):
             w1 = l0.weight.reshape(l0.out_channels, l0.in_channels)
             w2 = l2.weight.reshape(l2.out_channels, l2.in_channels)
             gs = self._grad_scale(z.device) if (onepass and self.onepass_decoder and not want_recon) else None
-            return Fh.decoder_mse(z, w1, l0.bias, w2, l2.bias, target, mask, want_recon, grad_scale=gs)
+            return Fh.decoder_mse(z, w1, l0.bias, w2, l2.bias, target, mask, want_recon, grad_scale=gs,
+                                  vq_fold=vq_fold if gs is not None else None)
         xhat = dec(z)
         return Fh.mse_loss(xhat, target, mask), xhat
 
@@ -229,10 +242,17 @@
                 ph = self._phase_branch(tile, zt, mask, return_recon, onepass, h_phase)
         d = z_type.shape[-1]
         split_vq = self.quant.quantizer != "ema" and z_type.is_cuda and not differentiable_vq_loss
-        zq, vq_loss, perp, idx = self.quant(z_type.reshape(-1, d), raw_terms=split_vq)
+        dt = self.decoder_type
+        fold = (self.fold_vq_grad and split_vq and onepass and self.onepass_decoder and not return_recon and torch.is_grad_enabled()
+                and z_type.requires_grad and self.fused_decoder and len(dt.layers) == 3
+                and ops.decoder_mse_vq_supported(d, dt.layers[0].out_channels, dt.layers[-1].out_channels, z_type))
+        z_rows = z_type.reshape(-1, d)
+        zq, vq_loss, perp, idx, zq_dec = self.quant(z_rows, raw_terms=split_vq, decoder_output=True)
         vq_parts = vq_loss if split_vq else None
         tmask = mask.amin(dim=1) if (mask is not None and mask.dim() == 4) else mask
-        l_type, xhat_type = self._decode_loss(self.decoder_type, zq.reshape(b, hh, ww, d), x_type, tmask, return_recon, onepass)
+        vq_fold = (z_rows, vq_parts[0][0], vq_parts[1][0], self._vq_grad_scale(z_type.device)) if fold else None
+        l_type, xhat_type = self._decode_loss(self.decoder_type, zq_dec if fold else zq.reshape(b, hh, ww, d), x_type, tmask, return_recon,
+                                              onepass, vq_fold)
         out = dict(z_type=z_type, gate=gate, idx=idx, vq_loss=None if split_vq else vq_loss, perplexity=perp, l_type=l_type,
                    vq_stats=self.quant.last_stats)
         if xhat_type is not None:
diff --git a/vq-vae_amd/frl_hip/ops.py b/vq-vae_amd/frl_hip/ops.py
--- a/vq-vae_amd/frl_hip/ops.py
+++ b/vq-vae_amd/frl_hip/ops.py
@@ -1088,17 +1088,36 @@
     return c
 
 
+def decoder_mse_vq_supported(cz: int, hidden: int, features: int, t: torch.Tensor) -> bool:
+    return bool(_lib.load().frl_decoder_mse_vq_supported(cz, hidden, features, _dt(t)))
+
+
 @_timed("decoder_mse_fwd_bwd")
-def decoder_mse_fwd_bwd(z, w1, b1, w2, b2, target, mask, grad_scale):
+def decoder_mse_fwd_bwd(z, w1, b1, w2, b2, target, mask, grad_scale, vq=None):
     cz = z.shape[-1]
     p = z.numel() // cz
     lib = _lib.load()
     if grad_scale is not None and (grad_scale.dtype != torch.float32 or grad_scale.numel() != 1 or grad_scale.device != z.device):
         raise ValueError("decoder_mse_fwd_bwd: grad_scale is a float32 scalar on the input's device")
+    z_pre = vq_gs = None
+    beta = 0.0
+    if vq is not None:
+        z_pre, vq_gs, beta = vq
+        if not decoder_mse_vq_supported(cz, w1.shape[0], w2.shape[0], z):
+            raise ValueError("decoder_mse_fwd_bwd: the quantizer fold needs bfloat16 rows of 64 channels")
+        if z_pre.dtype != z.dtype or z_pre.device != z.device or z_pre.numel() != z.numel() or not z_pre.is_contiguous():
+            raise ValueError("decoder_mse_fwd_bwd: z_pre must match z (contiguous rows, same dtype and device)")
+        if vq_gs is not None and (vq_gs.dtype != torch.float32 or vq_gs.numel() != 2 or vq_gs.device != z.device or not vq_gs.is_contiguous()):
+            raise ValueError("decoder_mse_fwd_bwd: the quantizer's gscale is a float32 [2] tensor on the input's device")
     buf = torch.empty(lib.frl_decoder_mse_onepass_bytes(p, cz), dtype=torch.uint8, device=z.device)
     out = torch.empty(2, dtype=torch.float32, device=z.device)
     dz = torch.empty_like(z)
     nslab = ctypes.c_int(0)
+    if vq is not None:
+        check(lib.frl_decoder_mse_fwd_bwd_vq(_p(z), _p(w1), _p(b1), _p(w2), _p(b2), _p(target), _p(mask), _p(grad_scale), _p(out), _p(dz), _p(buf),
+                                             buf.numel(), _p(_dec_ctl(z.device)), ctypes.cast(ctypes.byref(nslab), ctypes.c_void_p), p, cz,
+                                             _p(z_pre), _p(vq_gs), float(beta), _stream()), "frl_decoder_mse_fwd_bwd_vq")
+        return out, dz, (buf, int(nslab.value))
     check(lib.frl_decoder_mse_fwd_bwd(_p(z), _p(w1), _p(b1), _p(w2), _p(b2), _p(target), _p(mask), _p(grad_scale), _p(out), _p(dz), _p(buf),
                                       buf.numel(), _p(_dec_ctl(z.device)), ctypes.cast(ctypes.byref(nslab), ctypes.c_void_p), p, cz, _stream()),
           "frl_decoder_mse_fwd_bwd")
```

Result: no change. 112,000, median of 5 (+0.2%).
